# PytorchConnectomics/pytorch_connectomics

Hardware: AMD Instinct MI355X
Metric: voxels/s (train + sliding-window infer), MedNeXt-S 112^3 bf16 (higher is better)
Workload: dtype bf16; 1 GPU; Lucchi++ sliding-window inference (configs[1]): MedNeXt-S k3, 165x1024x768 volume, roi 112^3, overlap 0.5, bump blending, sw_batch_size 8, random-init weights; step = one whole-volume EagerSlidingWindowEngine call (TTA off); value = window-voxels/s; sw_batch_size=8, window_pipeline_streams=3

## Files before the change

include/pytc_hip.h:

```cpp
#ifndef PYTC_HIP_H
#define PYTC_HIP_H

#include <stdint.h>

#ifdef __cplusplus
extern "C" {
#endif

#define PYTC_ABI_VERSION 12

#define PYTC_OK 0
#define PYTC_ERR_INVALID 1
#define PYTC_ERR_HIP 2
#define PYTC_ERR_UNSUPPORTED 3

#define PYTC_F32 0
#define PYTC_BF16 1

#define PYTC_VIEW_FLIP_Z 1
#define PYTC_VIEW_FLIP_Y 2
#define PYTC_VIEW_FLIP_X 4
#define PYTC_VIEW_SWAP_YX 8
#define PYTC_VIEW_SWAP_ZY 16
#define PYTC_VIEW_SWAP_ZX 32

#define PYTC_PAD_CONSTANT 0
#define PYTC_PAD_REFLECT 1
#define PYTC_PAD_REPLICATE 2
#define PYTC_PAD_CIRCULAR 3

#define PYTC_BLEND_PRODUCT 0
#define PYTC_BLEND_MIN 1

#define PYTC_ACT_NONE 0
#define PYTC_ACT_SIGMOID 1
#define PYTC_ACT_TANH 2
#define PYTC_ACT_GELU 3

#define PYTC_RES_NONE 0
#define PYTC_RES_ADD 1
#define PYTC_RES_UPSAMPLE 2
#define PYTC_RES_GELU_BWD 3
#define PYTC_RES_NORM_BWD 4

int pytc_abi_version(void);
const char* pytc_last_error(void);
int pytc_device_info(int device, int* cu_count, int* lds_bytes_per_cu, char* arch, int arch_len);
int pytc_set_tuning(const char* key, int value);


int pytc_gather_windows(const float* vol, int C, int Z, int Y, int X, const int32_t* starts, int B,
                        int rz, int ry, int rx, int view, int pad_mode, float cval, void* out,
                        int out_dtype, void* stream);

int pytc_blend_accumulate(const void* pred, int pred_dtype, int B, const int32_t* starts, int rz,
                          int ry, int rx, int C, int view, const float* wz, const float* wy,
                          const float* wx, int combine, float floor_w, const int32_t* border ,
                          float* value, float* weight, int Z, int Y, int X, void* stream);

int pytc_blend_accumulate_mapped(const void* pred, int pred_dtype, int B, const int32_t* starts, int rz, int ry,
                                 int rx, int C, int view, const float* wz, const float* wy, const float* wx,
                                 int combine, float floor_w, const int32_t* border, const int32_t* chan_src,
                                 const int32_t* chan_shift, float* value, float* weight, int Z, int Y, int X,
                                 void* stream);
int pytc_blend_weight_shifted(int B, const int32_t* starts, int rz, int ry, int rx, const float* wz, const float* wy,
                              const float* wx, int combine, float floor_w, const int32_t* border,
                              const int32_t* shift, float* weight, int Z, int Y, int X, void* stream);
int pytc_normalize_covered(float* value, const float* weight, int64_t n, void* stream);
int pytc_ensemble_update_masked(float* stat, float* count, const float* x, const float* cover, int64_t n, int mode,
                                void* stream);
int pytc_ensemble_finalize_masked(const float* stat, const float* count, float* out, int64_t n, int mode, void* stream);

int pytc_blend_finalize(float* value, const float* weight, int C, int64_t nvox, float clamp,
                        int act, void* stream);

#define PYTC_ACT_SOFTMAX 4
int pytc_channel_activation(float* value, int C, int64_t nvox, int channels_last, int c0, int c1, int act,
                            float scale, void* stream);

int pytc_ensemble_update(float* acc, const float* x, int64_t n, int mode, int count, void* stream);

#define PYTC_ST_U8 0
#define PYTC_ST_I8 1
#define PYTC_ST_U16 2
#define PYTC_ST_I16 3
#define PYTC_ST_I32 4
#define PYTC_ST_F16 5
#define PYTC_ST_F32 6
int pytc_scale_cast(const float* x, void* y, int64_t n, float scale, int target, void* stream);


#define PYTC_RAW_U8 0
#define PYTC_RAW_I8 1
#define PYTC_RAW_U16 2
#define PYTC_RAW_I16 3
#define PYTC_RAW_U32 4
#define PYTC_RAW_I32 5
#define PYTC_RAW_F32 6
#define PYTC_RAW_F64 7
int pytc_resample_region(const void* raw, int raw_dtype, const int64_t* strides_czyx, int C, const int32_t* tab_i0,
                         const int32_t* tab_i1, const float* tab_f, const int32_t* dims_zyx, float* out, void* stream);

#define PYTC_NORM_NONE 0
#define PYTC_NORM_ZSCORE 1
#define PYTC_NORM_MINMAX 2
#define PYTC_NORM_DIVIDE 3
int64_t pytc_window_normalize_ws_elems(int B, int64_t n);
int pytc_window_normalize(float* x, int B, int64_t n, int mode, int binarize, float threshold, float divide, const float* clip,
                          double* workspace, void* stream);


int pytc_dwconv3d_stat_slots(int N, int D, int H, int W, int C, int K, int stride, int dtype,
                             int transposed);

int pytc_dwconv3d_kernel_variant(int N, int D, int H, int W, int C, int K, int stride, int dtype, int transposed);

int pytc_dwconv3d_fwd(const void* x, void* y, const float* w, const float* bias, float* stats,
                      int N, int D, int H, int W, int C, int K, int stride, int dtype,
                      void* stream);

int pytc_dwconv3d_fwd_wide(const void* x, void* y, const float* w, const float* bias, float* stats, int N, int D, int H,
                           int W, int C, int K, int stride, int dtype, void* stream);

int pytc_dwconv3d_res_supported(int D, int H, int W, int C, int K, int stride, int dtype);

int pytc_dwmix_supported(int D, int H, int W, int C, int C_hid, int C_out, int dtype);
int pytc_dwmix_fwd(const void* x, const float* taps, const float* dw_bias, const void* w2n, const float* b2n, const void* w3_f16,
                   const float* b3, int residual, void* y, const void* head_w, const float* head_b, float* head_y, int n_head, int N,
                   int D, int H, int W, int C, int C_hid, int C_out, int dtype, void* stream);
int pytc_dwconv3d_fwd_res(const void* x, const void* res, void* y, const float* w, const float* bias, int N, int D, int H,
                          int W, int C, int K, int stride, int dtype, void* stream);

int pytc_dwconvT3d_fwd(const void* x, void* y, const float* w, const float* bias, float* stats,
                       int N, int D, int H, int W, int C, int K, int dtype, void* stream);

int pytc_groupnorm_finalize(const float* stats, int slots, float count, const float* gamma,
                            const float* beta, float eps, float* ab, int N, int C, void* stream);


int64_t pytc_pw_packed_elems(int C_out, int C_in, int dtype);
int pytc_pw_pack_weight(const float* w, int C_out, int C_in, int transposed, void* packed,
                        int dtype, void* stream);

typedef struct {
  const void* x;
  const void* w_packed;
  const float* bias;
  const float* ab;
  const void* res;
  void* y;
  int N;
  int64_t rows_per_sample;
  int C_in, C_out;
  int in_dtype, out_dtype, w_dtype;
  int act;
  int res_mode;
  int gather;
  int Di, Hi, Wi;
  const void* res_low;
  const float* res_bias;
  int pre_act;
  int w_paired;
} pytc_pw_args;

int pytc_pw_conv_fwd(const pytc_pw_args* a, void* stream);
int pytc_pw_conv_paired_supported(const pytc_pw_args* a);
int pytc_pw_conv_rowmajor_supported(const pytc_pw_args* a);

typedef struct {
  const void* t;
  const float* ab;
  const void* w2_packed;
  const float* b2;
  const void* w3_packed;
  const float* b3;
  const void* res;
  const void* res_low;
  const float* res_bias;
  void* y;
  int N;
  int64_t rows_per_sample;
  int C_in, C_hid, C_out;
  int res_mode;
  int Di, Hi, Wi;
  int w3_format;
  int per_sample;
} pytc_mlp_args;
#define PYTC_W3_BF16 0
#define PYTC_W3_F16 1

int pytc_pw_gemm_supported(int C_in, int C_out);
int pytc_pw_gemm_fwd(const void* x, const void* w, const float* bias, const float* ab, void* y, int N, int64_t rows_per_sample,
                     int C_in, int C_out, int in_f16, int gelu_out, const void* res, const void* res_low, const float* res_bias,
                     int res_mode, int Di, int Hi, int Wi, void* stream);
int pytc_pw_mlp_supported(int C_in, int C_hid, int C_out);
int pytc_pw_pack_weight_paired(const float* w, int C_out, int C_in, int transposed, void* packed_bf16,
                               void* stream);
int pytc_pack_multi(const int64_t* table_dev, int n_items, int64_t total_elems, void* stream);
int pytc_pw_pack_weight_paired_f16(const float* w, int C_out, int C_in, int transposed, void* packed_f16,
                                   void* stream);
int pytc_pw_mlp_fwd(const pytc_mlp_args* a, void* stream);

int pytc_pw_mlp_lds_supported(int C_in, int C_hid, int C_out);
int pytc_pw_mlp_lds_fwd(const pytc_mlp_args* a, void* stream);
int pytc_pw_mlp_dma_applies(const pytc_mlp_args* a, int ignore_res_mode);
int pytc_pw_mlp_proj_supported(int C_in, int C_hid, int C_out, int C_proj);
int pytc_pw_mlp_proj_fwd(const pytc_mlp_args* a, const void* proj_w, const float* proj_b, void* z, int store_y, void* stream);
int pytc_pw_mlp_chunk_supported(int C_in, int C_hid, int C_out);
int pytc_pw_mlp_chunk_fwd(const pytc_mlp_args* a, void* stream);
int pytc_groupnorm_fold_mlp(const float* stats, int slots, float count, const float* gamma, const float* beta, float eps,
                            const float* w2, const float* b2, void* w2n, float* b2n, float* ab_out, int N, int C, int C_hid,
                            void* stream);
int pytc_pw_mlp_train_fwd(const pytc_mlp_args* a, void* hidden_pre, void* stream);
int pytc_pw_mlp_train_fwd_nostore(const pytc_mlp_args* a, void* stream);
int pytc_pw_mlp_bwd(const pytc_mlp_args* a, const void* hidden_pre, void* d_hidden, void* stream);
int pytc_pw_mlp_up_supported(int C_in, int C_hid, int C_out);
int pytc_pw_mlp_up_fwd(const pytc_mlp_args* a, const float* taps, const float* dw_bias, void* stream);
int pytc_pw_mlp_head_supported(int C_in, int C_hid, int C_out);
int pytc_pw_mlp_stemres_fwd(const pytc_mlp_args* a, const float* stem_x, const float* stem_w, const float* stem_b,
                            void* stream);
int pytc_stem_dwconv3d_stat_slots(int D, int H, int W);
int pytc_stem_dwconv3d_supported(int C_in, int C, int K);
int pytc_stem_dwconv3d_mfma_image_bytes(void);
int pytc_stem_dwconv3d_pack_mfma(const float* wx, const float* wb, const float* cst, void* image, void* stream);
int pytc_stem_dwconv3d_fwd(const float* x, const float* wx, const float* wb, const float* cst, const void* mfma_image, void* y,
                           float* stats, int N, int D, int H, int W, int C, void* stream);
int pytc_pw_mlp_head_fwd(const pytc_mlp_args* a, const void* head_w, const float* head_b, float* head_y, int n_head,
                         int store_y, void* stream);


#define PYTC_ACT_RELU 5
#define PYTC_ACT_LEAKY 6
#define PYTC_ACT_ELU 7

typedef struct {
  const void* x;
  const void* w_packed;
  const float* bias;
  const float* ab;
  const void* res;
  void* y;
  int N, D, H, W, C_in, C_out;
  int kd, kh, kw;
  int act_in;
  float act_param;
  int res_mode;
  int dtype;
} pytc_conv3d_args;

int64_t pytc_conv3d_packed_elems(int C_out, int C_in, int kd, int kh, int kw, int dtype);
int pytc_conv3d_pack_weight(const float* w, int C_out, int C_in, int kd, int kh, int kw, void* packed, int dtype,
                            void* stream);
int pytc_conv3d_fwd(const pytc_conv3d_args* a, void* stream);

int pytc_channel_stats_slots(int64_t rows);
int pytc_channel_stats(const void* x, float* stats, int N, int64_t rows, int C, int dtype, void* stream);
int pytc_norm_finalize_groups(const float* stats, int slots, float count, const float* gamma, const float* beta,
                              float eps, int groups, float* ab, int N, int C, void* stream);
int pytc_affine_act(const void* x, void* y, const float* ab, int N, int64_t rows, int C, int act, float prm,
                    int dtype, void* stream);
int pytc_maxpool3d_fwd(const void* x, void* y, int N, int D, int H, int W, int C, int fz, int fy, int fx, int dtype,
                       void* stream);
int pytc_dwconvT3d_generic_fwd(const void* x, void* y, const float* w, int N, int D, int H, int W, int C,
                               const int32_t* kernel, const int32_t* stride, const int32_t* pad, int dtype,
                               void* stream);


int pytc_groupnorm_finalize_mr(const float* stats, int slots, float count, const float* gamma, const float* beta,
                               float eps, float* ab, float* mean_rstd, int N, int C, void* stream);
int pytc_gelu(const void* x, const void* dy, void* out, int64_t n, int dtype, void* stream);
int pytc_add_inplace(void* y, const void* x, int64_t n, int dtype, void* stream);
int pytc_pw_wgrad_slots(int64_t rows_total);
int pytc_pw_wgrad(const void* x, const float* ab, const void* dy, float* dW, float* db, float* workspace, int N,
                  int64_t rows_per_sample, int C_in, int C_out, int dtype, int x_act , void* stream);
int pytc_dw_wgrad_slots(int N, const int32_t* gdims, const int32_t* xdims, int C, int K, int stride, int dtype);
int pytc_dw_wgrad(const void* g, const void* x, float* dW, float* db, float* workspace, int N, const int32_t* gdims,
                  const int32_t* xdims, int C, int K, int stride, int dtype, void* stream);

int pytc_pw_wgrad_partial(const void* x, const float* ab, const void* dy, float* workspace, int want_db, int N,
                          int64_t rows_per_sample, int C_in, int C_out, int dtype, int x_act, int* slots_out, void* stream);
int pytc_pw_wgrad_dgrad_supported(int C_in, int C_out, int dtype);
int pytc_pw_wgrad_dgrad_partial(const void* x, const void* dy, const void* w_t_paired, void* dx, float* workspace, int want_db, int N,
                                int64_t rows_per_sample, int C_in, int C_out, int dtype, int* slots_out, void* stream);
int pytc_mixer_bwd_rc_supported(int C, int C_hid, int C_out, int dtype);
int pytc_mixer_bwd_rc_sps(int N, int64_t rows_per_sample, int C_hid);
int64_t pytc_mixer_bwd_rc_ws_elems(int N, int64_t rows_per_sample, int C_hid, int gn);
int pytc_mixer_bwd_rc(const void* t, const float* ab, const float* mean_rstd, const void* dy, const void* w2_paired, const float* b2,
                      const void* w3t_paired, const float* W2, const float* gamma, float count, void* dhp, float* workspace,
                      float* s_out, float* coef, int want_db3, int gn, int N, int64_t rows_per_sample, int C, int C_hid, int C_out,
                      int dtype, int* slots_out, void* stream);
int pytc_dw_wgrad_partial(const void* g, const void* x, float* workspace, int want_db, int N, const int32_t* gdims,
                          const int32_t* xdims, int C, int K, int stride, int dtype, int* slots_out, void* stream);
int pytc_copy_zero_front(const void* src, void* dst, int N, const int32_t* dims, int C, int dtype, void* stream);
typedef struct {
  const float* part;
  float* out;
  int64_t n;
  int32_t slots;
  int32_t out_t;
} pytc_reduce_item;
int pytc_reduce_slots_multi(const pytc_reduce_item* items, int n_items, void* stream);
int pytc_norm_bwd_ws_elems(int N, int64_t rows, int C);
int pytc_norm_bwd(const void* dtn, const void* t, const float* mean_rstd, const float* gamma, float* stats_ws,
                  float* s_out, void* dt, int N, int64_t rows, float count , int C,
                  int dtype, void* stream);
int pytc_pw_wgrad_groupnorm_supported(int C, int C_hid, int dtype);
int pytc_pw_wgrad_groupnorm_sps(int N, int64_t rows_per_sample, int C, int C_hid);
int64_t pytc_pw_wgrad_groupnorm_ws_elems(int N, int64_t rows_per_sample, int C, int C_hid);
int pytc_pw_wgrad_groupnorm(const void* t, const float* mean_rstd, const float* ab, const void* dhp, const float* W2,
                            const float* gamma, float count, float* s_out, float* coef, float* workspace, int N,
                            int64_t rows_per_sample, int C, int C_hid, int dtype, void* stream);
int pytc_norm_bwd_apply(const void* dtn, const void* t, const float* mean_rstd, const float* gamma, const float* s_in,
                        int s_parts, void* dt, int N, int64_t rows, int C, float count, int dtype, const int32_t* crop_grid,
                        void* stream);
int pytc_dwconv3d_bwd_data(const void* dy, const float* w, void* dx, int N, const int32_t* xdims,
                           const int32_t* ydims, int C, int K, int stride, int dtype, void* stream);
int pytc_dwconv3d_bwd_data_add(const void* dy, const float* w, const void* addend, void* dx, int N, const int32_t* xdims,
                               const int32_t* ydims, int C, int K, int stride, int dtype, void* stream);

int pytc_conv3d_pack_weight_dgrad(const float* w, int C_out, int C_in, int kd, int kh, int kw, void* packed, int dtype,
                                  void* stream);
int pytc_conv3d_pack_plan(int C_out, int C_in, int kd, int kh, int kw, int dtype, int direct, int64_t* out);
int pytc_conv3d_pack_multi(const int64_t* table_dev, int n_items, int64_t total_blocks, void* stream);
int pytc_conv3d_launch_plan(int N, int D, int H, int W, int C_in, int C_out, int kd, int kh, int kw, int dtype, int has_pre,
                            int has_res, int phase, int64_t* out);
int pytc_norm_bwd_means(const float* s, const float* gamma, float* M, float* dgamma, float* dbeta, int N, int C, int groups,
                        float rows, void* stream);
int pytc_bn_train_finalize_cpad(const float* stats, int slots_total, float count, const float* gamma, const float* beta, float eps,
                                float momentum, float* running_mean, float* running_var, int64_t* num_batches_tracked, float* ab,
                                float* mean_rstd, int N, int C, int C_real, void* stream);
int pytc_norm_finalize_groups_cpg(const float* stats, int slots, float count, const float* gamma, const float* beta, float eps,
                                  int groups, int cpg, float* ab, float* mr, int N, int C, void* stream);
int pytc_norm_bwd_means_cpg(const float* s, const float* gamma, float* M, float* dgamma, float* dbeta, int N, int C, int groups,
                            int cpg, float rows, void* stream);
int pytc_bn_train_finalize(const float* stats, int slots_total, float count, const float* gamma, const float* beta, float eps,
                           float momentum, float* running_mean, float* running_var, int64_t* num_batches_tracked, float* ab,
                           float* mean_rstd, int N, int C, void* stream);
int pytc_bn_update_running(const float* mean_rstd, float* running_mean, float* running_var, int C, float count, float eps,
                           float momentum, void* stream);
int64_t pytc_conv3d_wgrad_ws_elems(int N, int D, int H, int W, int C_in, int C_out, const int32_t* kernel, int dtype);
int pytc_conv3d_wgrad(const void* a, const void* dy, float* dW, float* workspace, int N, int D, int H, int W, int C_in,
                      int C_out, const int32_t* kernel, int dtype, void* stream);
int pytc_act_bwd(const void* da, const void* x, const float* ab, void* dt, void* dp, int N, int64_t rows, int C, int act,
                 float prm, int dtype, void* stream);
int pytc_norm_finalize_groups_mr(const float* stats, int slots, float count, const float* gamma, const float* beta,
                                 float eps, int groups, float* ab, float* mr, int N, int C, void* stream);
int pytc_norm_bwd_stats(const void* dtn, const void* t, const float* mean_rstd, float* stats_ws, float* s_out, int N,
                        int64_t rows, int C, int dtype, void* stream);
int pytc_norm_bwd_apply_general(const void* d, const void* x, const float* mean_rstd, const float* gamma, const float* M,
                                void* dx, int N, int64_t rows, int C, int dtype, void* stream);
int pytc_act_norm_bwd_stats(const void* da, const void* x, const float* ab, const float* mean_rstd, float* stats_ws, float* s_out,
                            float* p_ws, float* p_out, int N, int64_t rows, int C, int act, float prm, int dtype, void* stream);
int pytc_act_norm_bwd_apply(const void* da, const void* x, const float* ab, const float* mean_rstd, const float* gamma,
                            const float* M, void* dx, int N, int64_t rows, int C, int act, float prm, int dtype, void* stream);
// ... 178 lines not shown
```

pytorch_connectomics_amd/csrc/pw_common.h:

```cpp
#pragma once
#include "pytc_common.h"

namespace pytc {

template <typename TW>
struct Mma;

template <>
struct Mma<bf16_t> {
  static constexpr int EPL = 8;
  static constexpr int KSTEP = 32;
  typedef bf16x8_t frag_t;
  static __device__ __forceinline__ f32x4_t mma(frag_t a, frag_t b, f32x4_t c) {
    return __builtin_amdgcn_mfma_f32_16x16x32_bf16(a, b, c, 0, 0, 0);
  }
  static __device__ __forceinline__ frag_t from_floats(const float (&v)[8]) {
    f32x8_t f;
#pragma unroll
    for (int i = 0; i < 8; ++i) f[i] = v[i];
    return __builtin_convertvector(f, frag_t);
  }
};

template <>
struct Mma<float> {
  static constexpr int EPL = 4;
  static constexpr int KSTEP = 16;
  typedef f32x4_t frag_t;
  static __device__ __forceinline__ f32x4_t mma(frag_t a, frag_t b, f32x4_t c) {
#pragma unroll
    for (int s = 0; s < 4; ++s) c = __builtin_amdgcn_mfma_f32_16x16x4f32(a[s], b[s], c, 0, 0, 0);
    return c;
  }
  static __device__ __forceinline__ frag_t from_floats(const float (&v)[4]) {
    frag_t f;
#pragma unroll
    for (int i = 0; i < 4; ++i) f[i] = v[i];
    return f;
  }
};

__host__ __device__ __forceinline__ int paired_row(int T, int m) {
  return (T >> 1) * 32 + (m >> 2) * 8 + (T & 1) * 4 + (m & 3);
}

struct EpiParams {
  const void* res;
  const void* res_low;
  const float* res_bias;
  void* y;
  long rps_out;
  int C_out;
  int res_mode;
  int Go_d, Go_h, Go_w;
  int Gl_d, Gl_h, Gl_w;
  int nt;
};

typedef unsigned int pytc_u32x4_t __attribute__((ext_vector_type(4)));
template <typename V>
__device__ __forceinline__ V ld_stream(const V* ptr, int nt) {
  static_assert(sizeof(V) == 16, "16-byte row pieces");
  if (nt) return __builtin_bit_cast(V, __builtin_nontemporal_load(reinterpret_cast<const pytc_u32x4_t*>(ptr)));
  return *ptr;
}

template <typename TO, int NCH, bool GELU_BWD = false, int COUT = 0>
__device__ __forceinline__ void finish_and_store(float (&v)[NCH], const EpiParams& e, int n, long orow, int o0,
                                                 const float* pre = nullptr, const int* pos = nullptr) {
  const int C_out = COUT > 0 ? COUT : e.C_out;
  TO* yn = reinterpret_cast<TO*>(e.y) + (long)n * e.rps_out * C_out;
  const TO* resn = e.res ? reinterpret_cast<const TO*>(e.res) + (long)n * e.rps_out * C_out : nullptr;
  const long off = orow * C_out + o0;
  const bool full = (C_out % NCH) == 0 && (o0 + NCH <= C_out);
  if (e.res_mode == PYTC_RES_ADD) {
    float rv[NCH];
    if (pre) {
#pragma unroll
      for (int i = 0; i < NCH; ++i) rv[i] = pre[i];
    } else if (full) VecIO<TO, NCH>::load(resn + off, rv);
    else {
#pragma unroll
      for (int i = 0; i < NCH; ++i) rv[i] = (o0 + i < C_out) ? to_f32<TO>(resn[off + i]) : 0.f;
    }
#pragma unroll
    for (int i = 0; i < NCH; ++i) v[i] += rv[i];
  } else if (GELU_BWD && e.res_mode == PYTC_RES_GELU_BWD) {
    float rv[NCH];
    if (pre) {
#pragma unroll
      for (int i = 0; i < NCH; ++i) rv[i] = pre[i];
    } else if (full) VecIO<TO, NCH>::load(resn + off, rv);
    else {
#pragma unroll
      for (int i = 0; i < NCH; ++i) rv[i] = (o0 + i < C_out) ? to_f32<TO>(resn[off + i]) : 0.f;
    }
#pragma unroll
    for (int i = 0; i < NCH; ++i) v[i] *= gelu_erf_grad(rv[i]);
  } else if (GELU_BWD && e.res_mode == PYTC_RES_NORM_BWD) {
    float rv[NCH];
    if (pre) {
#pragma unroll
      for (int i = 0; i < NCH; ++i) rv[i] = pre[i];
    } else if (full) VecIO<TO, NCH>::load(resn + off, rv);
    else {
#pragma unroll
      for (int i = 0; i < NCH; ++i) rv[i] = (o0 + i < C_out) ? to_f32<TO>(resn[off + i]) : 0.f;
    }
    const float* cf = e.res_bias + (long)n * 3 * C_out + o0;
#pragma unroll
    for (int i = 0; i < NCH; ++i)
      if (o0 + i < C_out) v[i] = fmaf(cf[i], v[i], fmaf(cf[C_out + i], rv[i], cf[2 * C_out + i]));
    if (e.Go_w > 0) {
      const unsigned ur = (unsigned)orow, gw = (unsigned)e.Go_w, gh = (unsigned)e.Go_h;
      const unsigned tq = ur / gw;
      const int px = (int)(ur - tq * gw), pz = (int)(tq / gh), py = (int)(tq - (unsigned)pz * gh);
      if (px == 0 || py == 0 || pz == 0) return;
      const long crow = ((long)(pz - 1) * (e.Go_h - 1) + (py - 1)) * (e.Go_w - 1) + (px - 1);
      TO* yc = reinterpret_cast<TO*>(e.y) + ((long)n * (e.Go_d - 1) * (e.Go_h - 1) * (e.Go_w - 1) + crow) * C_out + o0;
      if (full) VecIO<TO, NCH>::store(yc, v);
      else {
#pragma unroll
        for (int i = 0; i < NCH; ++i)
          if (o0 + i < C_out) yc[i] = from_f32<TO>(v[i]);
      }
      return;
    }
  } else if (e.res_mode == PYTC_RES_UPSAMPLE) {
    int px, py, pz;
    if (pos) { pz = pos[0]; py = pos[1]; px = pos[2]; }
    else {
      const unsigned ur = (unsigned)orow, gw = (unsigned)e.Go_w, gh = (unsigned)e.Go_h;
      const unsigned t = ur / gw;
      px = (int)(ur - t * gw);
      pz = (int)(t / gh);
      py = (int)(t - (unsigned)pz * gh);
    }
    float sk[NCH];
    if (pre) {
#pragma unroll
      for (int i = 0; i < NCH; ++i) sk[i] = pre[i];
    } else if (full) VecIO<TO, NCH>::load(resn + off, sk);
    else {
#pragma unroll
      for (int i = 0; i < NCH; ++i) sk[i] = (o0 + i < C_out) ? to_f32<TO>(resn[off + i]) : 0.f;
    }
    if (px == 0 || py == 0 || pz == 0) {
#pragma unroll
      for (int i = 0; i < NCH; ++i) v[i] = sk[i];
    } else {
      const int oz = pz - 1, oy = py - 1, ox = px - 1;
      float rl[NCH];
      if (e.res_low && !((oz | oy | ox) & 1)) {
        const TO* rp = reinterpret_cast<const TO*>(e.res_low) +
                       ((((long)n * e.Gl_d + (oz >> 1)) * e.Gl_h + (oy >> 1)) * e.Gl_w + (ox >> 1)) * C_out + o0;
        if (full) VecIO<TO, NCH>::load(rp, rl);
        else {
#pragma unroll
          for (int i = 0; i < NCH; ++i) rl[i] = (o0 + i < C_out) ? to_f32<TO>(rp[i]) : 0.f;
        }
      } else {
#pragma unroll
        for (int i = 0; i < NCH; ++i) rl[i] = (e.res_bias && o0 + i < C_out) ? e.res_bias[o0 + i] : 0.f;
      }
#pragma unroll
      for (int i = 0; i < NCH; ++i) v[i] = v[i] + rl[i] + sk[i];
    }
  }
  if (full) {
    if constexpr (sizeof(TO) == 2 && NCH == 8) {
      if (e.nt) {
        f32x8_t f;
#pragma unroll
        for (int i = 0; i < 8; ++i) f[i] = v[i];
        __builtin_nontemporal_store(__builtin_convertvector(f, bf16x8_t), reinterpret_cast<bf16x8_t*>(yn + off));
        return;
      }
    }
    VecIO<TO, NCH>::store(yn + off, v);
  } else {
#pragma unroll
    for (int i = 0; i < NCH; ++i)
      if (o0 + i < C_out) yn[off + i] = from_f32<TO>(v[i]);
  }
}

template <typename TI, int EPL>
__device__ __forceinline__ void load_row_frag(const TI* __restrict__ row, int k0, int C_in, bool vec_ok,
                                              float (&v)[EPL]) {
  if (vec_ok && k0 + EPL <= C_in) {
    if constexpr (sizeof(TI) == 4 && EPL == 8) {
      float t0[4], t1[4];
      VecIO<float, 4>::load(reinterpret_cast<const float*>(row) + k0, t0);
      VecIO<float, 4>::load(reinterpret_cast<const float*>(row) + k0 + 4, t1);
#pragma unroll
      for (int i = 0; i < 4; ++i) { v[i] = t0[i]; v[4 + i] = t1[i]; }
    } else {
      VecIO<TI, EPL>::load(row + k0, v);
    }
  } else {
#pragma unroll
    for (int j = 0; j < EPL; ++j) v[j] = (k0 + j < C_in) ? to_f32<TI>(row[k0 + j]) : 0.f;
  }
}

template <int PER>
struct WarmRegs { unsigned int r[2 * PER]; };
template <int PER>
__device__ __forceinline__ void warm_l2(const void* base, long bytes, WarmRegs<PER>& w, int first) {
  const long lines = (bytes + 127) >> 7;
  const long lin = (long)blockIdx.z * gridDim.y * gridDim.x + (long)blockIdx.y * gridDim.x + blockIdx.x;
  const long total = (long)gridDim.x * gridDim.y * gridDim.z;
  const long per_xcd = (total + 7) >> 3;
  const long stride = per_xcd * blockDim.x;
  long l = (lin >> 3) * blockDim.x + threadIdx.x;
#pragma unroll
  for (int it = 0; it < PER; ++it, l += stride) {
    const long lc = l < lines ? l : lines - 1;
    const char* ptr = reinterpret_cast<const char*>(base) + (lc << 7);
    asm volatile("global_load_dword %0, %1, off" : "=v"(w.r[first + it]) : "v"(ptr) : "memory");
  }
}
template <int PER>
__device__ __forceinline__ void warm_l2_done(WarmRegs<PER>& w) {
  asm volatile("s_waitcnt vmcnt(0)" : : : "memory");
#pragma unroll
  for (int i = 0; i < 2 * PER; ++i) asm volatile("" : : "v"(w.r[i]) : "memory");
}

__device__ __forceinline__ float apply_act(float t, int act) {
  if (act == PYTC_ACT_GELU) return gelu_erf(t);
  if (act == PYTC_ACT_SIGMOID) return 1.f / (1.f + __expf(-t));
  if (act == PYTC_ACT_TANH) return tanhf(t);
  return t;
}

}
```

pytorch_connectomics_amd/csrc/pw_mlp_chunk_kernels.hip:

```cpp
#include "pw_common.h"

namespace pytc {

struct MlpChunkParams {
  const bf16_t* t;
  const float* ab;
  const bf16x8_t* w2;
  const float* b2;
  const h8_t* w3;
  const float* b3;
  EpiParams e;
  long rps;
  int N, C_in, C_hid, C_out, HC;
  long w2_stride;
};

__device__ __forceinline__ void chunk_glds16(const void* gsrc, unsigned lds_dst) {
  unsigned keep;
  asm volatile("s_mov_b32 %0, m0\n\ts_mov_b32 m0, %2\n\ts_nop 0\n\tglobal_load_lds_dwordx4 %1, off\n\ts_mov_b32 m0, %0"
               : "=&s"(keep) : "v"(gsrc), "s"(lds_dst) : "memory");
}

template <int KS_IN, int MO, int NW, int WPS>
__global__ void __launch_bounds__(NW * 64, WPS)
// ... 47 lines not shown
    for (int ks = 0; ks < KS_IN; ++ks) raw[ks][nt] = ld_stream(reinterpret_cast<const uint4*>(tn + rr * CIN + ks * 32 + kb * 8), p.e.nt);
  }
  {
    const float* b2 = p.b2 + (folded ? (long)n * p.C_hid : 0L);
    for (int i = tid; i < p.C_hid; i += NW * 64) lb2[i] = b2[i];
    if (tid < COUT) lb3[tid] = p.b3[tid];
  }
  request(0);
  if (p.HC > 1) request(1);
  const float* an = folded ? nullptr : p.ab + (long)n * 2 * CIN;
#pragma unroll
  for (int ks = 0; ks < KS_IN; ++ks) {
    if (folded) {
#pragma unroll
      for (int nt = 0; nt < NT; ++nt) bact[ks][nt] = __builtin_bit_cast(bf16x8_t, raw[ks][nt]);
    } else {
      const int k0 = ks * 32 + kb * 8;
      float av[8], bv[8];
      VecIO<float, 4>::load(an + k0, reinterpret_cast<float(&)[4]>(av[0]));
      VecIO<float, 4>::load(an + k0 + 4, reinterpret_cast<float(&)[4]>(av[4]));
      VecIO<float, 4>::load(an + CIN + k0, reinterpret_cast<float(&)[4]>(bv[0]));
      VecIO<float, 4>::load(an + CIN + k0 + 4, reinterpret_cast<float(&)[4]>(bv[4]));
#pragma unroll
      for (int nt = 0; nt < NT; ++nt) {
        float v[8];
        VecIO<bf16_t, 8>::load(reinterpret_cast<const bf16_t*>(&raw[ks][nt]), v);
#pragma unroll
        for (int j = 0; j < 8; ++j) v[j] = fmaf(v[j], av[j], bv[j]);
        bact[ks][nt] = Mma<bf16_t>::from_floats(v);
      }
    }
  }
#pragma unroll
  for (int ks = 0; ks < KS_IN; ++ks)
#pragma unroll
    for (int nt = 0; nt < NT; ++nt) asm volatile("" : "+v"(bact[ks][nt]));
  __syncthreads();
  f32x4_t acc2[MO][NT];
#pragma unroll
  for (int pr = 0; pr < MO / 2; ++pr) {
    const f32x4_t lo = *reinterpret_cast<const f32x4_t*>(lb3 + pr * 32 + kb * 8), hi = *reinterpret_cast<const f32x4_t*>(lb3 + pr * 32 + kb * 8 + 4);
#pragma unroll
    for (int nt = 0; nt < NT; ++nt) { acc2[2 * pr][nt] = lo; acc2[2 * pr + 1][nt] = hi; }
  }

  for (int hc = 0; hc < p.HC; ++hc) {
    if (hc + 1 < p.HC) {
      if (mine == 2) asm volatile("s_waitcnt vmcnt(2)" ::: "memory");
      else if (mine == 1) asm volatile("s_waitcnt vmcnt(1)" ::: "memory");
      else if (mine == 3) asm volatile("s_waitcnt vmcnt(3)" ::: "memory");
      else asm volatile("s_waitcnt vmcnt(0)" ::: "memory");
    } else {
      asm volatile("s_waitcnt vmcnt(0)" ::: "memory");
    }
    __syncthreads();
    if (hc + 2 < p.HC) request(hc + 2);
    const uint4* cb = ring + (size_t)(hc % NBUF) * PIECES * 64;
    const f32x4_t b2lo = *reinterpret_cast<const f32x4_t*>(lb2 + hc * 32 + kb * 8);
    const f32x4_t b2hi = *reinterpret_cast<const f32x4_t*>(lb2 + hc * 32 + kb * 8 + 4);
    f32x4_t acc1[2][NT];
#pragma unroll
    for (int nt = 0; nt < NT; ++nt) { acc1[0][nt] = b2lo; acc1[1][nt] = b2hi; }
#pragma unroll
    for (int mt = 0; mt < 2; ++mt) {
#pragma unroll
      for (int ks = 0; ks < KS_IN; ++ks) {
        const bf16x8_t a = __builtin_bit_cast(bf16x8_t, cb[(mt * KS_IN + ks) * 64 + lane]);
#pragma unroll
        for (int nt = 0; nt < NT; ++nt) acc1[mt][nt] = Mma<bf16_t>::mma(a, bact[ks][nt], acc1[mt][nt]);
      }
    }
    h8_t bhh[NT];
#pragma unroll
    for (int nt = 0; nt < NT; ++nt) {
      float gg[8];
#pragma unroll
      for (int j = 0; j < 4; ++j) { gg[j] = acc1[0][nt][j]; gg[4 + j] = acc1[1][nt][j]; }
      bhh[nt] = gelu_h8_from_f32(gg);
    }
#pragma unroll
    for (int mo = 0; mo < MO; ++mo) {
      const h8_t a = __builtin_bit_cast(h8_t, cb[(2 * KS_IN + mo) * 64 + lane]);
#pragma unroll
      for (int nt = 0; nt < NT; ++nt) acc2[mo][nt] = __builtin_amdgcn_mfma_f32_16x16x32_f16(a, bhh[nt], acc2[mo][nt], 0, 0, 0);
    }
  }

  if (row0 >= p.rps) return;
  int upos[NT][3];
  if (ups) {
    const unsigned ur = (unsigned)row0, gw = (unsigned)p.e.Go_w, gh = (unsigned)p.e.Go_h;
    const unsigned t0 = ur / gw;
    const int bx = (int)(ur - t0 * gw);
    const int bz = (int)(t0 / gh);
    const int by = (int)(t0 - (unsigned)bz * gh);
#pragma unroll
    for (int nt = 0; nt < NT; ++nt) {
      int px = bx + nt * 16 + r, py = by, pz = bz;
      while (px >= p.e.Go_w) { px -= p.e.Go_w; ++py; }
      while (py >= p.e.Go_h) { py -= p.e.Go_h; ++pz; }
      upos[nt][0] = pz; upos[nt][1] = py; upos[nt][2] = px;
    }
  }
#pragma unroll
  for (int pr = 0; pr < MO / 2; ++pr) {
#pragma unroll
    for (int nt = 0; nt < NT; ++nt) {
      if (orow[nt] >= p.rps) continue;
      float v[8];
#pragma unroll
      for (int j = 0; j < 4; ++j) { v[j] = acc2[2 * pr][nt][j]; v[4 + j] = acc2[2 * pr + 1][nt][j]; }
      finish_and_store<bf16_t, 8, false, COUT>(v, p.e, n, orow[nt], pr * 32 + kb * 8, nullptr, (with_res && ups) ? upos[nt] : nullptr);
    }
  }
}

template <int KS_IN, int MO, int NW, int WPS>
static void launch_mlp_chunk_v(const MlpChunkParams& p, hipStream_t s) {
  auto kern = &pw_mlp_chunk_kernel<KS_IN, MO, NW, WPS>;
  const size_t lds = (size_t)3 * (2 * KS_IN + MO) * 1024 + (size_t)(p.C_hid + MO * 16) * 4;
  if (!ensure_dynamic_lds(reinterpret_cast<const void*>(kern), 160 * 1024, "pw_mlp_chunk")) return;
  const long wg_rows = (long)NW * 32;
  dim3 grid((unsigned)((p.rps + wg_rows - 1) / wg_rows), (unsigned)p.N), block(NW * 64);
  hipLaunchKernelGGL(kern, grid, block, lds, s, p);
}

template <int KS_IN, int MO>
static void launch_mlp_chunk(const MlpChunkParams& p, int variant, hipStream_t s) {
  if (variant == 0) variant = (KS_IN == 8) ? 1 : 3;
  switch (variant) {
    case 2: launch_mlp_chunk_v<KS_IN, MO, 12, 3>(p, s); break;
    case 3: launch_mlp_chunk_v<KS_IN, MO, 8, 4>(p, s); break;
    case 4: launch_mlp_chunk_v<KS_IN, MO, 16, 4>(p, s); break;
    default: launch_mlp_chunk_v<KS_IN, MO, 8, 2>(p, s); break;
  }
}

}

using namespace pytc;

extern "C" int pytc_pw_mlp_chunk_supported(int C_in, int C_hid, int C_out) {
  if (C_in % 32 || C_hid % 32 || C_out % 32) return 0;
  const int ks = C_in / 32, mo = C_out / 16;
  const bool shape = (ks == 2 && (mo == 2 || mo == 4 || mo == 8)) || (ks == 4 && mo == 4) || (ks == 4 && mo == 8) || (ks == 8 && mo == 8);
  return (shape && C_hid >= 64 && C_hid <= 8192) ? 1 : 0;
}

extern "C" int pytc_pw_mlp_chunk_fwd(const pytc_mlp_args* a, void* stream) {
  PYTC_REQUIRE(a && a->t && (a->ab || a->per_sample) && a->w2_packed && a->w3_packed && a->b2 && a->b3 && a->y, "pw_mlp_chunk: null pointer");
  PYTC_REQUIRE(!(a->ab && a->per_sample), "pw_mlp_chunk: per-sample (norm-folded) expand operands come without an affine");
  PYTC_REQUIRE(a->w3_format == PYTC_W3_F16, "pw_mlp_chunk: the projection image must be fp16 (pytc_pw_pack_weight_paired_f16)");
  PYTC_REQUIRE(a->N >= 1 && a->rows_per_sample >= 1, "pw_mlp_chunk: bad shape");
  if (!pytc_pw_mlp_chunk_supported(a->C_in, a->C_hid, a->C_out)) {
    set_error("pw_mlp_chunk: no chunk-streamed kernel for C_in=%d C_hid=%d C_out=%d", a->C_in, a->C_hid, a->C_out);
    return PYTC_ERR_UNSUPPORTED;
  }
  PYTC_REQUIRE(a->res_mode == PYTC_RES_NONE || a->res, "pw_mlp_chunk: residual mode without residual pointer");
  PYTC_REQUIRE(a->res_mode == PYTC_RES_NONE || a->res_mode == PYTC_RES_ADD || a->res_mode == PYTC_RES_UPSAMPLE, "pw_mlp_chunk: residual mode");
  MlpChunkParams p{};
  p.t = (const bf16_t*)a->t; p.ab = a->ab; p.w2 = (const bf16x8_t*)a->w2_packed; p.b2 = a->b2;
  p.w3 = (const h8_t*)a->w3_packed; p.b3 = a->b3;
  p.rps = a->rows_per_sample; p.N = a->N; p.C_in = a->C_in; p.C_hid = a->C_hid; p.C_out = a->C_out; p.HC = a->C_hid / 32;
  p.w2_stride = (long)(a->C_hid / 16) * (a->C_in / 32) * 64;
  p.e.res = a->res; p.e.res_low = a->res_low; p.e.res_bias = a->res_bias; p.e.y = a->y;
  p.e.rps_out = a->rows_per_sample; p.e.C_out = a->C_out; p.e.res_mode = a->res_mode;
  p.e.nt = 0;
  p.e.Go_d = p.e.Go_h = p.e.Go_w = p.e.Gl_d = p.e.Gl_h = p.e.Gl_w = 0;
  if (a->res_mode == PYTC_RES_UPSAMPLE) {
    PYTC_REQUIRE((long)a->Di * a->Hi * a->Wi == a->rows_per_sample && !(a->Di & 1) && !(a->Hi & 1) && !(a->Wi & 1) &&
                 a->rows_per_sample < (1L << 31), "pw_mlp_chunk: RES_UPSAMPLE needs the (even) output grid");
    p.e.Go_d = a->Di; p.e.Go_h = a->Hi; p.e.Go_w = a->Wi;
    p.e.Gl_d = a->Di / 2; p.e.Gl_h = a->Hi / 2; p.e.Gl_w = a->Wi / 2;
  }
  hipStream_t s = (hipStream_t)stream;
  const int ks = a->C_in / 32, mo = a->C_out / 16;
  const int variant = tuning_get(K_mlp_chunk_variant);
  if (ks == 2 && mo == 2) launch_mlp_chunk<2, 2>(p, variant, s);
  else if (ks == 2 && mo == 4) launch_mlp_chunk<2, 4>(p, variant, s);
  else if (ks == 2 && mo == 8) launch_mlp_chunk<2, 8>(p, variant, s);
  else if (ks == 4 && mo == 4) launch_mlp_chunk<4, 4>(p, variant, s);
  else if (ks == 4 && mo == 8) launch_mlp_chunk<4, 8>(p, variant, s);
  else launch_mlp_chunk<8, 8>(p, variant, s);
  PYTC_LAUNCH_CHECK("pw_mlp_chunk");
  return PYTC_OK;
}
```

pytorch_connectomics_amd/csrc/pw_mlp_kernels.hip:

```cpp
#include <cmath>
#include "pw_common.h"

namespace pytc {

struct MlpParams {
  const bf16_t* t;
  const float* ab;
  const bf16x8_t* w2;
  const float* b2;
  const bf16x8_t* w3;
  const float* b3;
  EpiParams e;
  long rps;
  int C_in, C_hid, C_out, HC;
  int w3_f16;
  long w2_stride;
  const bf16x8_t* head_w;
  const float* head_b;
  float* head_y;
  int n_head, store_y;
  bf16_t* proj_y;
  const float* stem_x;
  const float* stem_w;
  const float* stem_b;
  bf16_t* hp;
  int round_h;
  const bf16_t* hp_in;
};

constexpr int mlp_waves_per_simd(int ks, int mo, int nt) {
  if (ks >= 8 && nt == 1) return 1;
  const int regs = ks * nt * 4 + mo * nt * 4 + 2 * nt * 4;
  return regs <= 64 ? 4 : (regs <= 112 ? 3 : (regs <= 200 ? 2 : 1));
}

template <int KS_IN, int MO, int NT, int GELU_MODE, bool HEAD = false, bool STEMRES = false, bool STOREH = false, bool BWD = false>
__global__ void __launch_bounds__(256, mlp_waves_per_simd(KS_IN, MO, NT))
pw_mlp_kernel(MlpParams p) {
  constexpr int CIN = KS_IN * 32, COUT = MO * 16;
  static_assert(MO % 2 == 0, "C_out must be a multiple of 32");
  static_assert(!STEMRES || (MO == 2 && (MO / 2) * NT <= 4), "the stem-recomputing residual covers C_out = 32");
  static_assert(!HEAD || MO == 2, "the fused head covers C_out = 32");
  static_assert(GELU_MODE == 1 || GELU_MODE == 3, "sigmoid-form or packed-fp16 GELU");
  constexpr bool PREFETCH_RES = (MO / 2) * NT <= 4;
  const int wave = threadIdx.x >> 6, lane = threadIdx.x & 63;
  const int n = blockIdx.y;
  constexpr bool WARM = KS_IN * MO >= 32;
  constexpr int WPER = KS_IN * MO >= 512 ? 6 : 2;
  WarmRegs<WPER> warm;
  const bool folded = p.ab == nullptr;
  const bf16x8_t* w2 = p.w2 + (folded ? (long)n * p.w2_stride : 0L);
  const float* b2 = p.b2 + (folded ? (long)n * p.C_hid : 0L);
  if (WARM) {
    warm_l2(w2, (long)p.C_hid * CIN * 2, warm, 0);
    warm_l2(p.w3, (long)COUT * p.C_hid * 2, warm, WPER);
  }
  const long row0 = ((long)blockIdx.x * 4 + wave) * (NT * 16);
  if (row0 >= p.rps) {
    if (WARM) asm volatile("s_waitcnt vmcnt(0)" : : : "memory");
    return;
  }
  const int r = lane & 15, kb = lane >> 4;

  long orow[NT];
#pragma unroll
  for (int nt = 0; nt < NT; ++nt) orow[nt] = row0 + nt * 16 + r;

  bf16x8_t bact[KS_IN][NT];
  const bf16_t* tn = p.t + (long)n * p.rps * CIN;
  if (folded) {
#pragma unroll
    for (int ks = 0; ks < KS_IN; ++ks)
#pragma unroll
      for (int nt = 0; nt < NT; ++nt) {
        const long rr = orow[nt] < p.rps ? orow[nt] : p.rps - 1;
        bact[ks][nt] = ld_stream(reinterpret_cast<const bf16x8_t*>(tn + rr * CIN + ks * 32 + kb * 8), p.e.nt);
      }
  }
  const float* an = p.ab + (long)n * 2 * CIN;
#pragma unroll
  for (int ks = 0; ks < KS_IN; ++ks) {
    if (folded) break;
    const int k0 = ks * 32 + kb * 8;
    float av[8], bv[8];
    VecIO<float, 4>::load(an + k0, reinterpret_cast<float(&)[4]>(av[0]));
    VecIO<float, 4>::load(an + k0 + 4, reinterpret_cast<float(&)[4]>(av[4]));
    VecIO<float, 4>::load(an + CIN + k0, reinterpret_cast<float(&)[4]>(bv[0]));
    VecIO<float, 4>::load(an + CIN + k0 + 4, reinterpret_cast<float(&)[4]>(bv[4]));
#pragma unroll
    for (int nt = 0; nt < NT; ++nt) {
      const long rr = orow[nt] < p.rps ? orow[nt] : p.rps - 1;
      float v[8];
      VecIO<bf16_t, 8>::load(tn + rr * CIN + k0, v);
#pragma unroll
      for (int j = 0; j < 8; ++j) v[j] = fmaf(v[j], av[j], bv[j]);
      bact[ks][nt] = Mma<bf16_t>::from_floats(v);
    }
  }

  if (WARM) warm_l2_done(warm);

  uint4 rpre[PREFETCH_RES ? MO / 2 : 1][PREFETCH_RES ? NT : 1];
  const bool use_pre = PREFETCH_RES && p.e.res_mode != PYTC_RES_NONE;
  if constexpr (STEMRES) {
    const float* sx = p.stem_x + (long)n * p.rps;
    float sw[8], sb[8];
    VecIO<float, 4>::load(p.stem_w + kb * 8, reinterpret_cast<float(&)[4]>(sw[0]));
    VecIO<float, 4>::load(p.stem_w + kb * 8 + 4, reinterpret_cast<float(&)[4]>(sw[4]));
    VecIO<float, 4>::load(p.stem_b + kb * 8, reinterpret_cast<float(&)[4]>(sb[0]));
    VecIO<float, 4>::load(p.stem_b + kb * 8 + 4, reinterpret_cast<float(&)[4]>(sb[4]));
#pragma unroll
    for (int nt = 0; nt < NT; ++nt) {
      const float xv = sx[orow[nt] < p.rps ? orow[nt] : p.rps - 1];
      float rv[8];
#pragma unroll
      for (int j = 0; j < 8; ++j) rv[j] = fmaf(sw[j], xv, sb[j]);
      rpre[0][nt] = __builtin_bit_cast(uint4, Mma<bf16_t>::from_floats(rv));
    }
  } else if (use_pre) {
    const bf16_t* resn = reinterpret_cast<const bf16_t*>(p.e.res) + (long)n * p.rps * COUT;
#pragma unroll
    for (int pr = 0; pr < (PREFETCH_RES ? MO / 2 : 1); ++pr)
#pragma unroll
      for (int nt = 0; nt < (PREFETCH_RES ? NT : 1); ++nt) {
        const long rr = orow[nt] < p.rps ? orow[nt] : p.rps - 1;
        rpre[pr][nt] = ld_stream(reinterpret_cast<const uint4*>(resn + rr * COUT + pr * 32 + kb * 8), p.e.nt);
      }
  }

  f32x4_t acc2[MO][NT];
#pragma unroll
  for (int pr = 0; pr < MO / 2; ++pr) {
    float b[8];
    VecIO<float, 4>::load(p.b3 + pr * 32 + kb * 8, reinterpret_cast<float(&)[4]>(b[0]));
    VecIO<float, 4>::load(p.b3 + pr * 32 + kb * 8 + 4, reinterpret_cast<float(&)[4]>(b[4]));
#pragma unroll
    for (int nt = 0; nt < NT; ++nt) {
      acc2[2 * pr][nt] = f32x4_t{b[0], b[1], b[2], b[3]};
      acc2[2 * pr + 1][nt] = f32x4_t{b[4], b[5], b[6], b[7]};
    }
  }

  for (int hc = 0; hc < p.HC; ++hc) {
    float b2v[8];
    VecIO<float, 4>::load(b2 + hc * 32 + kb * 8, reinterpret_cast<float(&)[4]>(b2v[0]));
    VecIO<float, 4>::load(b2 + hc * 32 + kb * 8 + 4, reinterpret_cast<float(&)[4]>(b2v[4]));
    f32x4_t acc1[2][NT];
#pragma unroll
    for (int nt = 0; nt < NT; ++nt) {
      acc1[0][nt] = f32x4_t{b2v[0], b2v[1], b2v[2], b2v[3]};
      acc1[1][nt] = f32x4_t{b2v[4], b2v[5], b2v[6], b2v[7]};
    }
#pragma unroll
    for (int mt = 0; mt < 2; ++mt) {
#pragma unroll
      for (int ks = 0; ks < KS_IN; ++ks) {
        const bf16x8_t a = w2[((long)(hc * 2 + mt) * KS_IN + ks) * 64 + lane];
#pragma unroll
        for (int nt = 0; nt < NT; ++nt) acc1[mt][nt] = Mma<bf16_t>::mma(a, bact[ks][nt], acc1[mt][nt]);
      }
    }
    bf16x8_t bh[NT];
    h8_t bhh[GELU_MODE == 3 ? NT : 1];
#pragma unroll
    for (int nt = 0; nt < NT; ++nt) {
      float g[8];
      if constexpr (BWD) {
        const long rr = orow[nt] < p.rps ? orow[nt] : p.rps - 1;
        float hv[8];
        VecIO<bf16_t, 8>::load(p.hp_in + ((long)n * p.rps + rr) * p.C_hid + hc * 32 + kb * 8, hv);
#pragma unroll
        for (int j = 0; j < 4; ++j) {
          g[j] = acc1[0][nt][j] * gelu_erf_grad(hv[j]);
          g[4 + j] = acc1[1][nt][j] * gelu_erf_grad(hv[4 + j]);
        }
        bh[nt] = Mma<bf16_t>::from_floats(g);
        if (orow[nt] < p.rps)
          *reinterpret_cast<bf16x8_t*>(p.hp + ((long)n * p.rps + orow[nt]) * p.C_hid + hc * 32 + kb * 8) = bh[nt];
        continue;
      }
      if constexpr (STOREH) {
        float pre[8];
#pragma unroll
        for (int j = 0; j < 4; ++j) { pre[j] = acc1[0][nt][j]; pre[4 + j] = acc1[1][nt][j]; }
        const bf16x8_t hb = Mma<bf16_t>::from_floats(pre);
        if (p.hp && orow[nt] < p.rps)
          *reinterpret_cast<bf16x8_t*>(p.hp + ((long)n * p.rps + orow[nt]) * p.C_hid + hc * 32 + kb * 8) = hb;
        const f32x8_t hr = __builtin_convertvector(hb, f32x8_t);
#pragma unroll
        for (int j = 0; j < 4; ++j) { acc1[0][nt][j] = hr[j]; acc1[1][nt][j] = hr[4 + j]; }
      }
      if constexpr (GELU_MODE == 3) {
#pragma unroll
        for (int j = 0; j < 4; ++j) { g[j] = acc1[0][nt][j]; g[4 + j] = acc1[1][nt][j]; }
        bhh[nt] = gelu_h8_from_f32(g);
        continue;
      }
#pragma unroll
      for (int j = 0; j < 4; ++j) {
        g[j] = gelu_fast(acc1[0][nt][j]);
        g[4 + j] = gelu_fast(acc1[1][nt][j]);
      }
      bh[nt] = Mma<bf16_t>::from_floats(g);
    }
#pragma unroll
    for (int mo = 0; mo < MO; ++mo) {
      if constexpr (GELU_MODE == 3) {
        const h8_t a = reinterpret_cast<const h8_t*>(p.w3)[((long)mo * p.HC + hc) * 64 + lane];
#pragma unroll
        for (int nt = 0; nt < NT; ++nt) acc2[mo][nt] = __builtin_amdgcn_mfma_f32_16x16x32_f16(a, bhh[nt], acc2[mo][nt], 0, 0, 0);
      } else {
        const bf16x8_t a = p.w3[((long)mo * p.HC + hc) * 64 + lane];
#pragma unroll
        for (int nt = 0; nt < NT; ++nt) acc2[mo][nt] = Mma<bf16_t>::mma(a, bh[nt], acc2[mo][nt]);
      }
    }
  }

  if constexpr (HEAD) {
    bf16_t* yn = reinterpret_cast<bf16_t*>(p.e.y) + (long)n * p.rps * 32;
    const bf16_t* resn = p.e.res ? reinterpret_cast<const bf16_t*>(p.e.res) + (long)n * p.rps * 32 : nullptr;
    float* hy = p.head_y + (long)n * p.rps * p.n_head;
    const bf16x8_t ah = p.head_w[lane];
    float hb[4];
#pragma unroll
    for (int i = 0; i < 4; ++i) hb[i] = (p.head_b && kb * 4 + i < p.n_head) ? p.head_b[kb * 4 + i] : 0.f;
#pragma unroll
    for (int nt = 0; nt < NT; ++nt) {
      float v[8];
#pragma unroll
      for (int j = 0; j < 4; ++j) { v[j] = acc2[0][nt][j]; v[4 + j] = acc2[1][nt][j]; }
      const bool live = orow[nt] < p.rps;
      if (p.e.res_mode == PYTC_RES_ADD) {
        float rv[8];
        if (use_pre) VecIO<bf16_t, 8>::load(reinterpret_cast<const bf16_t*>(&rpre[0][PREFETCH_RES ? nt : 0]), rv);
        else VecIO<bf16_t, 8>::load(resn + (live ? orow[nt] : p.rps - 1) * 32 + kb * 8, rv);
#pragma unroll
        for (int j = 0; j < 8; ++j) v[j] += rv[j];
      }
      const bf16x8_t ob = Mma<bf16_t>::from_floats(v);
      if (p.store_y && live) *reinterpret_cast<bf16x8_t*>(yn + orow[nt] * 32 + kb * 8) = ob;
      const f32x4_t h = Mma<bf16_t>::mma(ah, ob, f32x4_t{0.f, 0.f, 0.f, 0.f});
      if (live) {
#pragma unroll
        for (int i = 0; i < 4; ++i)
          if (kb * 4 + i < p.n_head) hy[orow[nt] * p.n_head + kb * 4 + i] = h[i] + hb[i];
      }
    }
    return;
  }
  int upos[NT][3];
  const bool ups = p.e.res_mode == PYTC_RES_UPSAMPLE;
  if (ups) {
    const unsigned ur = (unsigned)row0, gw = (unsigned)p.e.Go_w, gh = (unsigned)p.e.Go_h;
    const unsigned t0 = ur / gw;
    const int bx = (int)(ur - t0 * gw);
    const int bz = (int)(t0 / gh);
    const int by = (int)(t0 - (unsigned)bz * gh);
#pragma unroll
    for (int nt = 0; nt < NT; ++nt) {
      int px = bx + nt * 16 + r, py = by, pz = bz;
      while (px >= p.e.Go_w) { px -= p.e.Go_w; ++py; }
      while (py >= p.e.Go_h) { py -= p.e.Go_h; ++pz; }
      upos[nt][0] = pz; upos[nt][1] = py; upos[nt][2] = px;
    }
  }
#pragma unroll
  for (int pr = 0; pr < MO / 2; ++pr) {
#pragma unroll
    for (int nt = 0; nt < NT; ++nt) {
      if (orow[nt] >= p.rps) continue;
      float v[8];
#pragma unroll
      for (int j = 0; j < 4; ++j) {
        v[j] = acc2[2 * pr][nt][j];
        v[4 + j] = acc2[2 * pr + 1][nt][j];
      }
      if (use_pre) {
        float pre[8];
        VecIO<bf16_t, 8>::load(reinterpret_cast<const bf16_t*>(&rpre[PREFETCH_RES ? pr : 0][PREFETCH_RES ? nt : 0]), pre);
        finish_and_store<bf16_t, 8, false, COUT>(v, p.e, n, orow[nt], pr * 32 + kb * 8, pre, ups ? upos[nt] : nullptr);
      } else {
        finish_and_store<bf16_t, 8, false, COUT>(v, p.e, n, orow[nt], pr * 32 + kb * 8, nullptr, ups ? upos[nt] : nullptr);
      }
    }
  }
}


__device__ __forceinline__ void glds16(const void* gsrc, unsigned lds_dst) {
  unsigned keep;
  asm volatile("s_mov_b32 %0, m0\n\ts_mov_b32 m0, %2\n\ts_nop 0\n\tglobal_load_lds_dwordx4 %1, off\n\ts_mov_b32 m0, %0"
               : "=&s"(keep) : "v"(gsrc), "s"(lds_dst) : "memory");
}
__device__ __forceinline__ void glds4(const void* gsrc, unsigned lds_dst) {
  unsigned keep;
  asm volatile("s_mov_b32 %0, m0\n\ts_mov_b32 m0, %2\n\ts_nop 0\n\tglobal_load_lds_dword %1, off\n\ts_mov_b32 m0, %0"
               : "=&s"(keep) : "v"(gsrc), "s"(lds_dst) : "memory");
}

template <int HCT, int KIND>
__global__ void __launch_bounds__(256, 3)
pw_mlp_dma_kernel(MlpParams p, int waves_per_sample) {
  constexpr int NT = 4, CIN = 32, COUT = 32;
  constexpr bool STEM = KIND == 1, HEAD = KIND == 2, PROJ = KIND == 3;
  __shared__ __attribute__((aligned(16))) uint4 land[4][2][NT * 64];
  __shared__ __attribute__((aligned(16))) uint4 w2s[HCT * 2 * 64], w3s[2 * HCT * 64];
  __shared__ __attribute__((aligned(16))) float b2s[HCT * 32], b3s[32];
  __shared__ __attribute__((aligned(16))) float auxa[STEM ? 32 : (HEAD ? 256 : (PROJ ? 512 : 4))], auxb[(STEM || PROJ) ? 32 : (HEAD ? 16 : 4)];
  const int wave = threadIdx.x >> 6, lane = threadIdx.x & 63;
  const int n = blockIdx.y;
  const int r = lane & 15, kb = lane >> 4;
  const long tiles = (p.rps + NT * 16 - 1) / (NT * 16);
  const bool with_res = STEM || p.e.res_mode == PYTC_RES_ADD;
  const bf16_t* tn = p.t + (long)n * p.rps * CIN;
  const bf16_t* resn = (!STEM && with_res) ? reinterpret_cast<const bf16_t*>(p.e.res) + (long)n * p.rps * COUT : nullptr;
  const float* sx = STEM ? p.stem_x + (long)n * p.rps : nullptr;
  bf16_t* yn = reinterpret_cast<bf16_t*>(p.e.y) + (long)n * p.rps * COUT;
  float* hy = HEAD ? p.head_y + (long)n * p.rps * p.n_head : nullptr;
  bf16_t* zn = PROJ ? p.proj_y + (long)n * p.rps * 32 : nullptr;
  {
    const uint4* w2 = reinterpret_cast<const uint4*>(p.w2 + (long)n * p.w2_stride);
    const uint4* w3 = reinterpret_cast<const uint4*>(p.w3);
    for (int i = threadIdx.x; i < HCT * 2 * 64; i += 256) { w2s[i] = w2[i]; w3s[i] = w3[i]; }
    if (threadIdx.x < HCT * 32) b2s[threadIdx.x] = p.b2[(long)n * p.C_hid + threadIdx.x];
    if (threadIdx.x < 32) b3s[threadIdx.x] = p.b3[threadIdx.x];
    if constexpr (STEM) {
      if (threadIdx.x < 32) { auxa[threadIdx.x] = p.stem_w[threadIdx.x]; auxb[threadIdx.x] = p.stem_b[threadIdx.x]; }
    }
    if constexpr (HEAD) {
      reinterpret_cast<float*>(auxa)[threadIdx.x] = reinterpret_cast<const float*>(p.head_w)[threadIdx.x];
      if (threadIdx.x < 16) auxb[threadIdx.x] = (p.head_b && (int)threadIdx.x < p.n_head) ? p.head_b[threadIdx.x] : 0.f;
    }
    if constexpr (PROJ) {
      auxa[threadIdx.x] = reinterpret_cast<const float*>(p.head_w)[threadIdx.x];
      auxa[threadIdx.x + 256] = reinterpret_cast<const float*>(p.head_w)[threadIdx.x + 256];
      if (threadIdx.x < 32) auxb[threadIdx.x] = p.head_b ? p.head_b[threadIdx.x] : 0.f;
    }
  }
  __syncthreads();
  asm volatile("s_waitcnt vmcnt(0)" ::: "memory");

  const unsigned lbase = __builtin_amdgcn_readfirstlane((unsigned)(size_t)(__attribute__((address_space(3))) void*)&land[wave][0][0]);
  auto request = [&](long tile) {
#pragma unroll
    for (int nt = 0; nt < NT; ++nt) {
      long row = tile * (NT * 16) + nt * 16 + r;
      row = row < p.rps ? row : p.rps - 1;
      glds16(tn + row * CIN + kb * 8, lbase + (unsigned)(nt * 64) * 16);
      if constexpr (STEM) glds4(sx + row, lbase + (unsigned)(NT * 64) * 16 + (unsigned)(nt * 64) * 4);
      else if (with_res) glds16(resn + row * COUT + kb * 8, lbase + (unsigned)((NT + nt) * 64) * 16);
    }
  };
  bf16x8_t out[NT];
  f32x4_t hout[HEAD ? NT : 1];
  bf16x8_t zout[PROJ ? NT : 1];
  auto store = [&](long tile) {
#pragma unroll
    for (int nt = 0; nt < NT; ++nt) {
      const long row = tile * (NT * 16) + nt * 16 + r;
      if (row >= p.rps) continue;
      if (!(HEAD || PROJ) || p.store_y) *reinterpret_cast<bf16x8_t*>(yn + row * COUT + kb * 8) = out[nt];
      if constexpr (PROJ) *reinterpret_cast<bf16x8_t*>(zn + row * 32 + kb * 8) = zout[nt];
      if constexpr (HEAD) {
#pragma unroll
        for (int i = 0; i < 4; ++i)
          if (kb * 4 + i < p.n_head) hy[row * p.n_head + kb * 4 + i] = hout[nt][i];
      }
    }
  };
  const long gw = (long)blockIdx.x * 4 + wave;
  long tile = gw;
  if (tile >= tiles) return;
  request(tile);
  long out_tile = -1;
  for (; tile < tiles; tile += waves_per_sample) {
    asm volatile("s_waitcnt vmcnt(0)" ::: "memory");
    __builtin_amdgcn_wave_barrier();
    if (out_tile >= 0) store(out_tile);
    bf16x8_t bact[NT];
    uint4 rpre[STEM ? 1 : NT];
    float xin[STEM ? NT : 1];
#pragma unroll
    for (int nt = 0; nt < NT; ++nt) {
      bact[nt] = __builtin_bit_cast(bf16x8_t, land[wave][0][nt * 64 + lane]);
      if constexpr (STEM) xin[nt] = reinterpret_cast<const float*>(&land[wave][1][0])[nt * 64 + lane];
      else if (with_res) rpre[nt] = land[wave][1][nt * 64 + lane];
    }
    asm volatile("s_waitcnt lgkmcnt(0)" ::: "memory");
    __builtin_amdgcn_wave_barrier();
    if (tile + waves_per_sample < tiles) request(tile + waves_per_sample);
    f32x4_t acc2[2][NT];
    {
      const f32x4_t lo = *reinterpret_cast<const f32x4_t*>(&b3s[kb * 8]), hi = *reinterpret_cast<const f32x4_t*>(&b3s[kb * 8 + 4]);
#pragma unroll
      for (int nt = 0; nt < NT; ++nt) { acc2[0][nt] = lo; acc2[1][nt] = hi; }
    }
#pragma unroll
    for (int hc = 0; hc < HCT; ++hc) {
      f32x4_t acc1[2][NT];
      {
        const f32x4_t lo = *reinterpret_cast<const f32x4_t*>(&b2s[hc * 32 + kb * 8]), hi = *reinterpret_cast<const f32x4_t*>(&b2s[hc * 32 + kb * 8 + 4]);
#pragma unroll
        for (int nt = 0; nt < NT; ++nt) { acc1[0][nt] = lo; acc1[1][nt] = hi; }
      }
#pragma unroll
      for (int mt = 0; mt < 2; ++mt) {
        const bf16x8_t a2 = __builtin_bit_cast(bf16x8_t, w2s[(hc * 2 + mt) * 64 + lane]);
#pragma unroll
        for (int nt = 0; nt < NT; ++nt) acc1[mt][nt] = Mma<bf16_t>::mma(a2, bact[nt], acc1[mt][nt]);
      }
      h8_t bhh[NT];
#pragma unroll
      for (int nt = 0; nt < NT; ++nt) {
        float g[8];
#pragma unroll
        for (int j = 0; j < 4; ++j) { g[j] = acc1[0][nt][j]; g[4 + j] = acc1[1][nt][j]; }
        bhh[nt] = gelu_h8_from_f32(g);
      }
#pragma unroll
      for (int mo = 0; mo < 2; ++mo) {
        const h8_t a3 = __builtin_bit_cast(h8_t, w3s[(mo * HCT + hc) * 64 + lane]);
#pragma unroll
        for (int nt = 0; nt < NT; ++nt) acc2[mo][nt] = __builtin_amdgcn_mfma_f32_16x16x32_f16(a3, bhh[nt], acc2[mo][nt], 0, 0, 0);
      }
    }
    float sw[STEM ? 8 : 1], sb[STEM ? 8 : 1];
    if constexpr (STEM) {
#pragma unroll
// ... 96 lines not shown
  __syncthreads();
  if (i >= total) return;
  int lo = s_lo;
  while (lo + 1 < n_items && table[(lo + 1) * 8 + 6] <= i) ++lo;
  const long* it = table + lo * 8;
  const float* w = reinterpret_cast<const float*>(it[0]);
  const int kind = (int)it[2], C_out = (int)it[3], C_in = (int)it[4], aux = (int)it[5];
  const long e = i - it[6];
  if (kind >= 6) {
    const int o = (int)(e / C_in), k = (int)(e % C_in);
    reinterpret_cast<bf16_t*>(it[1])[e] = from_f32<bf16_t>(kind == 7 ? w[(long)k * C_out + o] : w[e]);
    return;
  }
  if (kind >= 4) {
    const int K3 = aux, C = C_out;
    const int k = (int)(e / C), c = (int)(e % C);
    reinterpret_cast<float*>(it[1])[e] = w[(long)c * K3 + (kind == 5 ? K3 - 1 - k : k)];
    return;
  }
  const int KG = aux, transposed = kind & 1;
  const int j = (int)(e % 8);
  long t = e / 8;
  const int lane = (int)(t % 64);
  t /= 64;
  const int kg = (int)(t % KG);
  const int T = (int)(t / KG);
  const int o = paired_row(T, lane & 15);
  const int k = kg * 32 + (lane >> 4) * 8 + j;
  float v = 0.f;
  if (o < C_out && k < C_in) v = transposed ? w[(long)k * C_out + o] : w[(long)o * C_in + k];
  if (kind >= 2) reinterpret_cast<_Float16*>(it[1])[e] = (_Float16)v;
  else reinterpret_cast<bf16_t*>(it[1])[e] = from_f32<bf16_t>(v);
}

__global__ void __launch_bounds__(1024)
groupnorm_fold_mlp_kernel(const float* __restrict__ stats, int slots, float count, const float* __restrict__ gamma,
                          const float* __restrict__ beta, float eps, const float* __restrict__ w2, const float* __restrict__ b2,
                          bf16_t* __restrict__ w2n, float* __restrict__ b2n, float* __restrict__ ab_out, int C, int C_hid) {
  __shared__ __attribute__((aligned(16))) float red[1024 * 4];
  __shared__ float part[8][2 * 128];
  __shared__ float sa[128], sb[128], smean[128], sbeta[128];
  const int n = blockIdx.x, tid = threadIdx.x;
  const int Q = C / 2;
  const int col = tid % Q, sl = tid / Q, SL = 1024 / Q;
  const float* base = stats + (long)n * slots * 2 * C + col * 4;
  const int KG = C / 32;
  const long total = (long)C_hid * C;
  constexpr int PRE = 2;
  f32x4_t wpre[PRE][2];
#pragma unroll
  for (int i = 0; i < PRE; ++i) {
    const long e8 = tid + (long)i * 1024;
    if (e8 < total / 8) {
      long t = e8;
      const int lane = (int)(t % 64);
      t /= 64;
      const int kg = (int)(t % KG);
      const int o = paired_row((int)(t / KG), lane & 15);
      const float* src = w2 + (long)o * C + kg * 32 + (lane >> 4) * 8;
      wpre[i][0] = *reinterpret_cast<const f32x4_t*>(src);
      wpre[i][1] = *reinterpret_cast<const f32x4_t*>(src + 4);
    }
  }
  f32x4_t a = {0.f, 0.f, 0.f, 0.f};
  constexpr int INFL = 20;
  for (int s0 = sl; s0 < slots; s0 += SL * INFL) {
    f32x4_t v[INFL];
#pragma unroll
    for (int i = 0; i < INFL; ++i) {
      const int s = s0 + i * SL;
      v[i] = s < slots ? *reinterpret_cast<const f32x4_t*>(base + (long)s * 2 * C) : f32x4_t{0.f, 0.f, 0.f, 0.f};
    }
#pragma unroll
    for (int i = 0; i < INFL; ++i)
      if (s0 + i * SL < slots) a += v[i];
  }
  *reinterpret_cast<f32x4_t*>(&red[tid * 4]) = a;
  __syncthreads();
  {
    const int e = tid % (2 * C), pg = tid / (2 * C);
    const int groups = 1024 / (2 * C) < 8 ? 1024 / (2 * C) : 8;
    if (pg < groups) {
      float t = 0.f;
      for (int s = pg; s < SL; s += groups) t += red[s * 2 * C + e];
      part[pg][e] = t;
    }
    __syncthreads();
    if (tid < C) {
      float t1 = 0.f, t2 = 0.f;
      for (int g = 0; g < groups; ++g) { t1 += part[g][tid]; t2 += part[g][C + tid]; }
      const float mean = t1 / count;
      const float var = fmaxf(t2 / count - mean * mean, 0.f);
      float rstd = rsqrtf(var + eps);
      rstd = rstd * (1.5f - 0.5f * (var + eps) * rstd * rstd);
      const float av = (gamma ? gamma[tid] : 1.f) * rstd;
      const float bv = (beta ? beta[tid] : 0.f) - mean * av;
      sa[tid] = av;
      sb[tid] = bv;
      smean[tid] = mean;
      sbeta[tid] = beta ? beta[tid] : 0.f;
      if (ab_out) {
        ab_out[((long)n * 2 + 0) * C + tid] = av;
        ab_out[((long)n * 2 + 1) * C + tid] = bv;
      }
    }
  }
  __syncthreads();
  bf16_t* img = w2n + (long)n * total;
  for (long e8 = tid, i = 0; e8 < total / 8; e8 += 1024, ++i) {
    long t = e8;
    const int lane = (int)(t % 64);
    t /= 64;
    const int kg = (int)(t % KG);
    const int T = (int)(t / KG);
    const int o = paired_row(T, lane & 15);
    const int k = kg * 32 + (lane >> 4) * 8;
    float v[8];
    if (i < PRE) {
#pragma unroll
      for (int q = 0; q < PRE; ++q)
        if (q == i) {
#pragma unroll
          for (int j = 0; j < 4; ++j) { v[j] = wpre[q][0][j]; v[4 + j] = wpre[q][1][j]; }
        }
    } else {
      VecIO<float, 4>::load(w2 + (long)o * C + k, reinterpret_cast<float(&)[4]>(v[0]));
      VecIO<float, 4>::load(w2 + (long)o * C + k + 4, reinterpret_cast<float(&)[4]>(v[4]));
    }
#pragma unroll
    for (int j = 0; j < 8; ++j) v[j] *= sa[k + j];
    *reinterpret_cast<bf16x8_t*>(img + e8 * 8) = Mma<bf16_t>::from_floats(v);
  }
  for (int o = tid; o < C_hid; o += 1024) {
    float acc = b2 ? b2[o] : 0.f;
    const float* wr = w2 + (long)o * C;
    for (int k = 0; k < C; k += 8) {
      const f32x4_t w0 = *reinterpret_cast<const f32x4_t*>(wr + k), w1 = *reinterpret_cast<const f32x4_t*>(wr + k + 4);
      float v[8], wn[8];
#pragma unroll
      for (int j = 0; j < 4; ++j) { v[j] = w0[j] * sa[k + j]; v[4 + j] = w1[j] * sa[k + 4 + j]; }
      const bf16x8_t rounded = Mma<bf16_t>::from_floats(v);
      VecIO<bf16_t, 8>::load(reinterpret_cast<const bf16_t*>(&rounded), wn);
#pragma unroll
      for (int j = 0; j < 8; ++j) {
        const float wj = j < 4 ? w0[j] : w1[j - 4];
        acc = fmaf(wj, sbeta[k + j], acc);
        acc = fmaf(-wn[j], smean[k + j], acc);
      }
    }
    b2n[(long)n * C_hid + o] = acc;
  }
}

template <int KS_IN, int MO, int NT>
static void launch_mlp(const MlpParams& p, int N, hipStream_t s) {
  long rows_per_block = 4L * NT * 16;
  dim3 grid((unsigned)((p.rps + rows_per_block - 1) / rows_per_block), (unsigned)N), block(256);
  if (p.hp_in) {
    hipLaunchKernelGGL((pw_mlp_kernel<KS_IN, MO, NT, 1, false, false, false, true>), grid, block, 0, s, p);
    return;
  }
  if (p.hp || p.round_h) {
    if (p.w3_f16) hipLaunchKernelGGL((pw_mlp_kernel<KS_IN, MO, NT, 3, false, false, true>), grid, block, 0, s, p);
    else hipLaunchKernelGGL((pw_mlp_kernel<KS_IN, MO, NT, 1, false, false, true>), grid, block, 0, s, p);
    return;
  }
  if (p.w3_f16) hipLaunchKernelGGL((pw_mlp_kernel<KS_IN, MO, NT, 3>), grid, block, 0, s, p);
  else hipLaunchKernelGGL((pw_mlp_kernel<KS_IN, MO, NT, 1>), grid, block, 0, s, p);
}

static bool dispatch_mlp(const MlpParams& p, int N, hipStream_t s) {
  const int ks = p.C_in / 32, mo = p.C_out / 16;
#define PYTC_MLP_CASE(KS, MOO, NTT) \
  if (ks == KS && mo == MOO) { launch_mlp<KS, MOO, NTT>(p, N, s); return true; }
  PYTC_MLP_CASE(1, 2, 4)
  PYTC_MLP_CASE(1, 4, 4)
  PYTC_MLP_CASE(2, 2, 4)
  PYTC_MLP_CASE(2, 4, 2)
  PYTC_MLP_CASE(2, 8, 2)
  PYTC_MLP_CASE(4, 4, 2)
  PYTC_MLP_CASE(4, 8, 2)
  PYTC_MLP_CASE(4, 16, 1)
  PYTC_MLP_CASE(8, 8, 2)
  PYTC_MLP_CASE(8, 16, 1)
  PYTC_MLP_CASE(8, 32, 1)
  PYTC_MLP_CASE(16, 16, 1)
  PYTC_MLP_CASE(16, 32, 1)
#undef PYTC_MLP_CASE
  return false;
}

static bool mlp_shape_ok(int C_in, int C_hid, int C_out) {
  if (C_in % 32 || C_hid % 32 || C_out % 32 || C_in < 32 || C_out < 32 || C_hid < 32) return false;
  const int ks = C_in / 32, mo = C_out / 16;
  static const int ok[][2] = {{1, 2}, {1, 4}, {2, 2}, {2, 4}, {2, 8}, {4, 4}, {4, 8}, {4, 16}, {8, 8},
                              {8, 16}, {8, 32}, {16, 16}, {16, 32}};
  for (auto& c : ok)
    if (c[0] == ks && c[1] == mo) return true;
  return false;
}

}

using namespace pytc;

extern "C" int pytc_pw_mlp_supported(int C_in, int C_hid, int C_out) { return mlp_shape_ok(C_in, C_hid, C_out) ? 1 : 0; }

extern "C" int pytc_groupnorm_fold_mlp(const float* stats, int slots, float count, const float* gamma, const float* beta,
                                       float eps, const float* w2, const float* b2, void* w2n, float* b2n, float* ab_out, int N,
                                       int C, int C_hid, void* stream) {
  PYTC_REQUIRE(stats && w2 && w2n && b2n && slots >= 1 && count > 0 && N >= 1, "groupnorm_fold_mlp: bad arguments");
  PYTC_REQUIRE(C == 32 || C == 64 || C == 128, "groupnorm_fold_mlp: C=%d (32, 64 or 128)", C);
  PYTC_REQUIRE(C_hid % 32 == 0 && C_hid >= 32 && C_hid <= 512, "groupnorm_fold_mlp: C_hid=%d", C_hid);
  hipLaunchKernelGGL(groupnorm_fold_mlp_kernel, dim3(N), dim3(1024), 0, (hipStream_t)stream, stats, slots, count, gamma, beta,
                     eps, w2, b2, (bf16_t*)w2n, b2n, ab_out, C, C_hid);
  PYTC_LAUNCH_CHECK("groupnorm_fold_mlp");
  return PYTC_OK;
}

extern "C" int pytc_pw_mlp_head_supported(int C_in, int C_hid, int C_out) {
  return (C_out == 32 && (C_in == 32 || C_in == 64) && C_hid % 32 == 0 && C_hid >= 32) ? 1 : 0;
}

extern "C" int pytc_pw_pack_weight_paired(const float* w, int C_out, int C_in, int transposed, void* packed,
                                          void* stream) {
  PYTC_REQUIRE(w && packed && C_out >= 1 && C_in >= 1, "pw_pack_weight_paired: bad arguments");
  PYTC_REQUIRE(C_out % 32 == 0, "pw_pack_weight_paired: C_out=%d must be a multiple of 32", C_out);
  long total = pytc_pw_packed_elems(C_out, C_in, PYTC_BF16);
  int KG = (C_in + 31) / 32;
  hipLaunchKernelGGL(pw_pack_paired_kernel<bf16_t>, dim3(ceil_div(total, 256)), dim3(256), 0, (hipStream_t)stream, w, C_out,
                     C_in, transposed, (bf16_t*)packed, KG, total);
  PYTC_LAUNCH_CHECK("pw_pack_weight_paired");
  return PYTC_OK;
}

extern "C" int pytc_pw_pack_weight_paired_f16(const float* w, int C_out, int C_in, int transposed, void* packed,
                                              void* stream) {
  PYTC_REQUIRE(w && packed && C_out >= 1 && C_in >= 1, "pw_pack_weight_paired_f16: bad arguments");
  PYTC_REQUIRE(C_out % 32 == 0, "pw_pack_weight_paired_f16: C_out=%d must be a multiple of 32", C_out);
  long total = pytc_pw_packed_elems(C_out, C_in, PYTC_BF16);
  int KG = (C_in + 31) / 32;
  hipLaunchKernelGGL(pw_pack_paired_kernel<_Float16>, dim3(ceil_div(total, 256)), dim3(256), 0, (hipStream_t)stream, w,
                     C_out, C_in, transposed, (_Float16*)packed, KG, total);
  PYTC_LAUNCH_CHECK("pw_pack_weight_paired_f16");
  return PYTC_OK;
}

extern "C" int pytc_pack_multi(const int64_t* table_dev, int n_items, int64_t total_elems, void* stream) {
  PYTC_REQUIRE(table_dev && n_items >= 1 && total_elems >= 1, "pack_multi: bad arguments");
  hipLaunchKernelGGL(pack_multi_kernel, dim3(ceil_div(total_elems, 256)), dim3(256), 0, (hipStream_t)stream,
                     reinterpret_cast<const long*>(table_dev), n_items, (long)total_elems);
  PYTC_LAUNCH_CHECK("pack_multi");
  return PYTC_OK;
}

extern "C" int pytc_pw_mlp_head_fwd(const pytc_mlp_args* a, const void* head_w, const float* head_b, float* head_y,
                                    int n_head, int store_y, void* stream) {
  PYTC_REQUIRE(a && a->t && (a->ab || a->per_sample) && a->w2_packed && a->w3_packed && a->b2 && a->b3 && head_w && head_y, "pw_mlp_head: null pointer");
  PYTC_REQUIRE(!(a->ab && a->per_sample), "pw_mlp_head: per-sample (norm-folded) expand operands come without an affine");
  PYTC_REQUIRE(!store_y || a->y, "pw_mlp_head: store_y without an output buffer");
  PYTC_REQUIRE(a->N >= 1 && a->rows_per_sample >= 1 && n_head >= 1 && n_head <= 16, "pw_mlp_head: bad shape");
  if (!pytc_pw_mlp_head_supported(a->C_in, a->C_hid, a->C_out)) {
    set_error("pw_mlp_head: no fused kernel for C_in=%d C_hid=%d C_out=%d", a->C_in, a->C_hid, a->C_out);
    return PYTC_ERR_UNSUPPORTED;
  }
  PYTC_REQUIRE(a->res_mode == PYTC_RES_NONE || (a->res_mode == PYTC_RES_ADD && a->res), "pw_mlp_head: residual add or none");
  MlpParams p;
  p.t = (const bf16_t*)a->t; p.ab = a->ab; p.w2 = (const bf16x8_t*)a->w2_packed; p.b2 = a->b2;
  p.w3 = (const bf16x8_t*)a->w3_packed; p.b3 = a->b3;
  p.rps = a->rows_per_sample; p.C_in = a->C_in; p.C_hid = a->C_hid; p.C_out = a->C_out; p.HC = a->C_hid / 32;
  p.w2_stride = (long)(a->C_hid / 16) * (a->C_in / 32) * 64;
  p.e.res = a->res; p.e.res_low = nullptr; p.e.res_bias = nullptr; p.e.y = a->y;
  p.e.rps_out = a->rows_per_sample; p.e.C_out = a->C_out; p.e.res_mode = a->res_mode;
  p.e.nt = 0;
  p.e.Go_d = p.e.Go_h = p.e.Go_w = p.e.Gl_d = p.e.Gl_h = p.e.Gl_w = 0;
  p.head_w = (const bf16x8_t*)head_w; p.head_b = head_b; p.head_y = head_y; p.n_head = n_head; p.store_y = store_y;
  p.w3_f16 = a->w3_format == PYTC_W3_F16 ? 1 : 0;
  dim3 grid((unsigned)((p.rps + 4L * 4 * 16 - 1) / (4L * 4 * 16)), (unsigned)a->N), block(256);
  hipStream_t s = (hipStream_t)stream;
  if (mlp_dma_applies(a, p)) {
    mlp_dma_launch<2>(a, p, s);
    PYTC_LAUNCH_CHECK("pw_mlp_head_dma");
    return PYTC_OK;
  }
  if (p.w3_f16) {
    if (a->C_in == 32) hipLaunchKernelGGL((pw_mlp_kernel<1, 2, 4, 3, true>), grid, block, 0, s, p);
    else hipLaunchKernelGGL((pw_mlp_kernel<2, 2, 4, 3, true>), grid, block, 0, s, p);
  } else if (a->C_in == 32) {
    hipLaunchKernelGGL((pw_mlp_kernel<1, 2, 4, 1, true>), grid, block, 0, s, p);
  } else {
    hipLaunchKernelGGL((pw_mlp_kernel<2, 2, 4, 1, true>), grid, block, 0, s, p);
  }
  PYTC_LAUNCH_CHECK("pw_mlp_head");
  return PYTC_OK;
}

extern "C" int pytc_pw_mlp_stemres_fwd(const pytc_mlp_args* a, const float* stem_x, const float* stem_w, const float* stem_b,
                                       void* stream) {
  PYTC_REQUIRE(a && a->t && (a->ab || a->per_sample) && a->w2_packed && a->w3_packed && a->b2 && a->b3 && a->y && stem_x && stem_w && stem_b,
               "pw_mlp_stemres: null pointer");
  PYTC_REQUIRE(!(a->ab && a->per_sample), "pw_mlp_stemres: per-sample (norm-folded) expand operands come without an affine");
  PYTC_REQUIRE(a->N >= 1 && a->rows_per_sample >= 1, "pw_mlp_stemres: bad shape");
  if (!(a->C_in == 32 && a->C_out == 32 && a->C_hid % 32 == 0 && a->C_hid >= 32)) {
    set_error("pw_mlp_stemres: no fused kernel for C_in=%d C_hid=%d C_out=%d", a->C_in, a->C_hid, a->C_out);
    return PYTC_ERR_UNSUPPORTED;
  }
  MlpParams p{};
  p.t = (const bf16_t*)a->t; p.ab = a->ab; p.w2 = (const bf16x8_t*)a->w2_packed; p.b2 = a->b2;
  p.w3 = (const bf16x8_t*)a->w3_packed; p.b3 = a->b3;
  p.rps = a->rows_per_sample; p.C_in = a->C_in; p.C_hid = a->C_hid; p.C_out = a->C_out; p.HC = a->C_hid / 32;
  p.w2_stride = (long)(a->C_hid / 16) * (a->C_in / 32) * 64;
  p.e.res = a->y;
  p.e.y = a->y;
  p.e.rps_out = a->rows_per_sample; p.e.C_out = a->C_out; p.e.res_mode = PYTC_RES_ADD;
  p.e.nt = 0;
  p.stem_x = stem_x; p.stem_w = stem_w; p.stem_b = stem_b;
  p.w3_f16 = a->w3_format == PYTC_W3_F16 ? 1 : 0;
  dim3 grid((unsigned)((p.rps + 4L * 4 * 16 - 1) / (4L * 4 * 16)), (unsigned)a->N), block(256);
  hipStream_t s = (hipStream_t)stream;
  pytc_mlp_args shape = *a;
  shape.res_mode = PYTC_RES_NONE;
  if (mlp_dma_applies(&shape, p)) {
    mlp_dma_launch<1>(a, p, s);
    PYTC_LAUNCH_CHECK("pw_mlp_stemres_dma");
    return PYTC_OK;
  }
  if (p.w3_f16) hipLaunchKernelGGL((pw_mlp_kernel<1, 2, 4, 3, false, true>), grid, block, 0, s, p);
  else hipLaunchKernelGGL((pw_mlp_kernel<1, 2, 4, 1, false, true>), grid, block, 0, s, p);
  PYTC_LAUNCH_CHECK("pw_mlp_stemres");
  return PYTC_OK;
}

extern "C" int pytc_pw_mlp_dma_applies(const pytc_mlp_args* a, int ignore_res_mode) {
  if (!a) return 0;
  MlpParams p{};
  p.HC = a->C_hid / 32;
  p.w3_f16 = a->w3_format == PYTC_W3_F16 ? 1 : 0;
  pytc_mlp_args shape = *a;
  if (ignore_res_mode) shape.res_mode = PYTC_RES_NONE;
  return mlp_dma_applies(&shape, p) ? 1 : 0;
}

extern "C" int pytc_pw_mlp_proj_supported(int C_in, int C_hid, int C_out, int C_proj) {
  return (C_in == 32 && C_out == 32 && C_proj == 32 && (C_hid == 64 || C_hid == 96 || C_hid == 128)) ? 1 : 0;
}
extern "C" int pytc_pw_mlp_proj_fwd(const pytc_mlp_args* a, const void* proj_w, const float* proj_b, void* z, int store_y, void* stream) {
  PYTC_REQUIRE(a && a->t && a->w2_packed && a->w3_packed && a->b2 && a->b3 && proj_w && z, "pw_mlp_proj: null pointer");
  PYTC_REQUIRE(a->per_sample && !a->ab, "pw_mlp_proj: takes the per-sample (norm-folded) expand operands");
  PYTC_REQUIRE(a->w3_format == PYTC_W3_F16, "pw_mlp_proj: the mixer's projection image must be fp16 (pytc_pw_pack_weight_paired_f16)");
  PYTC_REQUIRE(!store_y || a->y, "pw_mlp_proj: store_y without an output buffer");
  PYTC_REQUIRE(a->N >= 1 && a->rows_per_sample >= 1, "pw_mlp_proj: bad shape");
  if (!pytc_pw_mlp_proj_supported(a->C_in, a->C_hid, a->C_out, 32)) {
    set_error("pw_mlp_proj: no fused kernel for C_in=%d C_hid=%d C_out=%d", a->C_in, a->C_hid, a->C_out);
    return PYTC_ERR_UNSUPPORTED;
  }
  PYTC_REQUIRE(a->res_mode == PYTC_RES_NONE || (a->res_mode == PYTC_RES_ADD && a->res), "pw_mlp_proj: residual add or none");
  MlpParams p{};
  p.t = (const bf16_t*)a->t; p.ab = nullptr; p.w2 = (const bf16x8_t*)a->w2_packed; p.b2 = a->b2;
  p.w3 = (const bf16x8_t*)a->w3_packed; p.b3 = a->b3;
  p.rps = a->rows_per_sample; p.C_in = a->C_in; p.C_hid = a->C_hid; p.C_out = a->C_out; p.HC = a->C_hid / 32;
  p.w2_stride = (long)(a->C_hid / 16) * (a->C_in / 32) * 64;
  p.e.res = a->res; p.e.y = a->y; p.e.rps_out = a->rows_per_sample; p.e.C_out = a->C_out; p.e.res_mode = a->res_mode;
  p.head_w = (const bf16x8_t*)proj_w; p.head_b = proj_b; p.proj_y = (bf16_t*)z; p.store_y = store_y;
  p.w3_f16 = 1;
  mlp_dma_launch<3>(a, p, (hipStream_t)stream);
  PYTC_LAUNCH_CHECK("pw_mlp_proj");
  return PYTC_OK;
}

static int mlp_fwd_impl(const pytc_mlp_args* a, void* hp, void* stream, const void* hp_in = nullptr, bool round_h = false);

extern "C" int pytc_pw_mlp_bwd(const pytc_mlp_args* a, const void* hidden_pre, void* d_hidden, void* stream) {
  PYTC_REQUIRE(hidden_pre && d_hidden, "pw_mlp_bwd: null hidden buffers");
  PYTC_REQUIRE(a && a->res_mode == PYTC_RES_NONE, "pw_mlp_bwd: no residual in the backward mixer");
  return mlp_fwd_impl(a, d_hidden, stream, hidden_pre);
}

extern "C" int pytc_pw_mlp_train_fwd(const pytc_mlp_args* a, void* hidden_pre, void* stream) {
  PYTC_REQUIRE(hidden_pre, "pw_mlp_train: null hidden buffer");
  return mlp_fwd_impl(a, hidden_pre, stream);
}

extern "C" int pytc_pw_mlp_train_fwd_nostore(const pytc_mlp_args* a, void* stream) {
  return mlp_fwd_impl(a, nullptr, stream, nullptr, true);
}

extern "C" int pytc_pw_mlp_fwd(const pytc_mlp_args* a, void* stream) { return mlp_fwd_impl(a, nullptr, stream); }

static int mlp_fwd_impl(const pytc_mlp_args* a, void* hp, void* stream, const void* hp_in, bool round_h) {
  PYTC_REQUIRE(a && a->t && (a->ab || a->per_sample) && a->w2_packed && a->w3_packed && a->b2 && a->b3 && a->y, "pw_mlp: null pointer");
  PYTC_REQUIRE(!(a->ab && a->per_sample), "pw_mlp: per-sample (norm-folded) expand operands come without an affine");
  PYTC_REQUIRE(!(a->per_sample && (hp || hp_in || round_h)), "pw_mlp: the training kernels take the shared expand image and the affine");
  PYTC_REQUIRE(a->N >= 1 && a->rows_per_sample >= 1, "pw_mlp: bad shape");
  if (!mlp_shape_ok(a->C_in, a->C_hid, a->C_out)) {
    set_error("pw_mlp: no fused kernel for C_in=%d C_hid=%d C_out=%d", a->C_in, a->C_hid, a->C_out);
    return PYTC_ERR_UNSUPPORTED;
  }
  PYTC_REQUIRE(a->res_mode == PYTC_RES_NONE || a->res, "pw_mlp: residual mode without residual pointer");
  PYTC_REQUIRE(a->res_mode == PYTC_RES_NONE || a->res_mode == PYTC_RES_ADD || a->res_mode == PYTC_RES_UPSAMPLE,
               "pw_mlp: unsupported res_mode %d", a->res_mode);
  MlpParams p{};
  p.t = (const bf16_t*)a->t; p.ab = a->ab; p.w2 = (const bf16x8_t*)a->w2_packed; p.b2 = a->b2;
  p.w3 = (const bf16x8_t*)a->w3_packed; p.b3 = a->b3;
  p.rps = a->rows_per_sample; p.C_in = a->C_in; p.C_hid = a->C_hid; p.C_out = a->C_out; p.HC = a->C_hid / 32;
  p.w2_stride = (long)(a->C_hid / 16) * (a->C_in / 32) * 64;
  p.e.res = a->res; p.e.res_low = a->res_low; p.e.res_bias = a->res_bias; p.e.y = a->y;
  p.e.rps_out = a->rows_per_sample; p.e.C_out = a->C_out; p.e.res_mode = a->res_mode;
  p.e.nt = 0;
  p.e.Go_d = p.e.Go_h = p.e.Go_w = p.e.Gl_d = p.e.Gl_h = p.e.Gl_w = 0;
  p.hp = (bf16_t*)hp;
  p.hp_in = (const bf16_t*)hp_in;
  p.round_h = round_h ? 1 : 0;
  p.w3_f16 = a->w3_format == PYTC_W3_F16 ? 1 : 0;
  PYTC_REQUIRE(!(p.w3_f16 && hp_in), "pw_mlp_bwd: the backward mixer takes bf16 weight images");
  if (a->res_mode == PYTC_RES_UPSAMPLE) {
    PYTC_REQUIRE((long)a->Di * a->Hi * a->Wi == a->rows_per_sample && !(a->Di & 1) && !(a->Hi & 1) && !(a->Wi & 1),
                 "pw_mlp: RES_UPSAMPLE needs the (even) output grid");
    PYTC_REQUIRE(a->rows_per_sample < (1L << 31), "pw_mlp: RES_UPSAMPLE positions are 32-bit (rows per sample < 2^31)");
    p.e.Go_d = a->Di; p.e.Go_h = a->Hi; p.e.Go_w = a->Wi;
    p.e.Gl_d = a->Di / 2; p.e.Gl_h = a->Hi / 2; p.e.Gl_w = a->Wi / 2;
  }
  if (!hp && !hp_in && !round_h && mlp_dma_applies(a, p)) {
    mlp_dma_launch<0>(a, p, (hipStream_t)stream);
    PYTC_LAUNCH_CHECK("pw_mlp_dma");
    return PYTC_OK;
  }
  if (!dispatch_mlp(p, a->N, (hipStream_t)stream)) {
    set_error("pw_mlp: dispatch failed");
    return PYTC_ERR_UNSUPPORTED;
  }
  PYTC_LAUNCH_CHECK("pw_mlp");
  return PYTC_OK;
}
```

pytorch_connectomics_amd/csrc/pw_mlp_lds_kernels.hip:

```cpp
#include <mutex>

#include "pw_common.h"

namespace pytc {

struct MlpLdsParams {
  const bf16_t* t;
  const float* ab;
  const bf16x8_t* w2;
  const float* b2;
  const h8_t* w3;
  const float* b3;
  EpiParams e;
  long rps;
  int N, C_in, C_hid, C_out, HC;
  long w2_stride;
};

template <int KS_IN, int MO, int NT>
struct LdsTile {
  uint4 raw[KS_IN][NT];
  uint4 res[MO / 2][NT];
};

template <int KS_IN, int MO, int NT>
__device__ __forceinline__ void lds_tile_load(LdsTile<KS_IN, MO, NT>& T, const MlpLdsParams& p, int n, long row0, int r, int kb,
                                              bool with_res) {
  const bf16_t* tn = p.t + (long)n * p.rps * (KS_IN * 32);
#pragma unroll
  for (int nt = 0; nt < NT; ++nt) {
    const long o = row0 + nt * 16 + r;
    const long rr = o < p.rps ? o : p.rps - 1;
#pragma unroll
    for (int ks = 0; ks < KS_IN; ++ks) T.raw[ks][nt] = ld_stream(reinterpret_cast<const uint4*>(tn + rr * (KS_IN * 32) + ks * 32 + kb * 8), p.e.nt);
  }
  if (with_res) {
    const bf16_t* resn = reinterpret_cast<const bf16_t*>(p.e.res) + (long)n * p.rps * (MO * 16);
#pragma unroll
    for (int nt = 0; nt < NT; ++nt) {
      const long o = row0 + nt * 16 + r;
      const long rr = o < p.rps ? o : p.rps - 1;
#pragma unroll
      for (int pr = 0; pr < MO / 2; ++pr) T.res[pr][nt] = ld_stream(reinterpret_cast<const uint4*>(resn + rr * (MO * 16) + pr * 32 + kb * 8), p.e.nt);
    }
  }
}

template <int KS_IN, int MO, int NT, int NWAVES, int WPS>
__global__ void __launch_bounds__(NWAVES * 64, WPS)
pw_mlp_lds_kernel(MlpLdsParams p) {
  constexpr int CIN = KS_IN * 32, COUT = MO * 16;
  extern __shared__ __attribute__((aligned(16))) unsigned char lds_raw[];
  bf16x8_t* lw2 = reinterpret_cast<bf16x8_t*>(lds_raw);
  h8_t* lw3 = reinterpret_cast<h8_t*>(lds_raw + (size_t)p.C_hid * CIN * 2);
  float* lb2 = reinterpret_cast<float*>(lds_raw + (size_t)p.C_hid * (CIN + COUT) * 2);
  const int tid = threadIdx.x, wave = tid >> 6, lane = tid & 63;
  const int r = lane & 15, kb = lane >> 4;
  const bool folded = p.ab == nullptr;
  const int n_w2 = p.C_hid * CIN / 8, n_w3 = COUT * p.C_hid / 8;
  for (int i = tid; i < n_w3; i += NWAVES * 64) lw3[i] = p.w3[i];
  const long Ts = (p.rps + NT * 16 - 1) / (NT * 16);
  const long G = Ts * p.N;
  const long g_end = G * (blockIdx.x + 1) / gridDim.x;
  long g = G * blockIdx.x / gridDim.x;
  const bool with_res = p.e.res_mode != PYTC_RES_NONE;
  const bool ups = p.e.res_mode == PYTC_RES_UPSAMPLE;
  int staged = -1;

  while (g < g_end) {
    const int n = (int)(g / Ts);
    const long seg_end = min(g_end, (long)(n + 1) * Ts);
    if (staged < 0 || folded) {
      __syncthreads();
      const bf16x8_t* src = p.w2 + (folded ? (long)n * p.w2_stride : 0L);
      for (int i = tid; i < n_w2; i += NWAVES * 64) lw2[i] = src[i];
      const float* b2 = p.b2 + (folded ? (long)n * p.C_hid : 0L);
      for (int i = tid; i < p.C_hid; i += NWAVES * 64) lb2[i] = b2[i];
      staged = n;
      __syncthreads();
    }
    const float* an = folded ? nullptr : p.ab + (long)n * 2 * CIN;
    const long t_base = (long)n * Ts;

    for (long gt = g + wave; gt < seg_end; gt += NWAVES) {
      const long row0 = (gt - t_base) * (NT * 16);
      LdsTile<KS_IN, MO, NT> cur;
      lds_tile_load(cur, p, n, row0, r, kb, with_res);
      long orow[NT];
#pragma unroll
      for (int nt = 0; nt < NT; ++nt) orow[nt] = row0 + nt * 16 + r;

      bf16x8_t bact[KS_IN][NT];
#pragma unroll
      for (int ks = 0; ks < KS_IN; ++ks) {
        if (folded) {
#pragma unroll
          for (int nt = 0; nt < NT; ++nt) bact[ks][nt] = __builtin_bit_cast(bf16x8_t, cur.raw[ks][nt]);
        } else {
          const int k0 = ks * 32 + kb * 8;
          float av[8], bv[8];
          VecIO<float, 4>::load(an + k0, reinterpret_cast<float(&)[4]>(av[0]));
          VecIO<float, 4>::load(an + k0 + 4, reinterpret_cast<float(&)[4]>(av[4]));
          VecIO<float, 4>::load(an + CIN + k0, reinterpret_cast<float(&)[4]>(bv[0]));
          VecIO<float, 4>::load(an + CIN + k0 + 4, reinterpret_cast<float(&)[4]>(bv[4]));
#pragma unroll
          for (int nt = 0; nt < NT; ++nt) {
            float v[8];
            VecIO<bf16_t, 8>::load(reinterpret_cast<const bf16_t*>(&cur.raw[ks][nt]), v);
#pragma unroll
            for (int j = 0; j < 8; ++j) v[j] = fmaf(v[j], av[j], bv[j]);
            bact[ks][nt] = Mma<bf16_t>::from_floats(v);
          }
        }
      }
      f32x4_t acc2[MO][NT];
#pragma unroll
      for (int pr = 0; pr < MO / 2; ++pr) {
        float b[8];
        VecIO<float, 4>::load(p.b3 + pr * 32 + kb * 8, reinterpret_cast<float(&)[4]>(b[0]));
        VecIO<float, 4>::load(p.b3 + pr * 32 + kb * 8 + 4, reinterpret_cast<float(&)[4]>(b[4]));
#pragma unroll
        for (int nt = 0; nt < NT; ++nt) {
          acc2[2 * pr][nt] = f32x4_t{b[0], b[1], b[2], b[3]};
          acc2[2 * pr + 1][nt] = f32x4_t{b[4], b[5], b[6], b[7]};
        }
      }
      for (int hc = 0; hc < p.HC; ++hc) {
        const f32x4_t b2lo = *reinterpret_cast<const f32x4_t*>(lb2 + hc * 32 + kb * 8);
        const f32x4_t b2hi = *reinterpret_cast<const f32x4_t*>(lb2 + hc * 32 + kb * 8 + 4);
        f32x4_t acc1[2][NT];
#pragma unroll
        for (int nt = 0; nt < NT; ++nt) { acc1[0][nt] = b2lo; acc1[1][nt] = b2hi; }
#pragma unroll
        for (int mt = 0; mt < 2; ++mt) {
#pragma unroll
          for (int ks = 0; ks < KS_IN; ++ks) {
            const bf16x8_t a = lw2[((hc * 2 + mt) * KS_IN + ks) * 64 + lane];
#pragma unroll
            for (int nt = 0; nt < NT; ++nt) acc1[mt][nt] = Mma<bf16_t>::mma(a, bact[ks][nt], acc1[mt][nt]);
          }
        }
        h8_t bhh[NT];
#pragma unroll
        for (int nt = 0; nt < NT; ++nt) {
          float gg[8];
#pragma unroll
          for (int j = 0; j < 4; ++j) { gg[j] = acc1[0][nt][j]; gg[4 + j] = acc1[1][nt][j]; }
          bhh[nt] = gelu_h8_from_f32(gg);
        }
#pragma unroll
        for (int mo = 0; mo < MO; ++mo) {
          const h8_t a = lw3[(mo * p.HC + hc) * 64 + lane];
#pragma unroll
          for (int nt = 0; nt < NT; ++nt) acc2[mo][nt] = __builtin_amdgcn_mfma_f32_16x16x32_f16(a, bhh[nt], acc2[mo][nt], 0, 0, 0);
        }
      }
      int upos[NT][3];
      if (ups) {
        const unsigned ur = (unsigned)row0, gw = (unsigned)p.e.Go_w, gh = (unsigned)p.e.Go_h;
        const unsigned t0 = ur / gw;
        const int bx = (int)(ur - t0 * gw);
        const int bz = (int)(t0 / gh);
        const int by = (int)(t0 - (unsigned)bz * gh);
#pragma unroll
        for (int nt = 0; nt < NT; ++nt) {
          int px = bx + nt * 16 + r, py = by, pz = bz;
          while (px >= p.e.Go_w) { px -= p.e.Go_w; ++py; }
          while (py >= p.e.Go_h) { py -= p.e.Go_h; ++pz; }
          upos[nt][0] = pz; upos[nt][1] = py; upos[nt][2] = px;
        }
      }
#pragma unroll
      for (int pr = 0; pr < MO / 2; ++pr) {
#pragma unroll
        for (int nt = 0; nt < NT; ++nt) {
          if (orow[nt] >= p.rps) continue;
          float v[8];
#pragma unroll
          for (int j = 0; j < 4; ++j) { v[j] = acc2[2 * pr][nt][j]; v[4 + j] = acc2[2 * pr + 1][nt][j]; }
          if (with_res) {
            float pre[8];
            VecIO<bf16_t, 8>::load(reinterpret_cast<const bf16_t*>(&cur.res[pr][nt]), pre);
            finish_and_store<bf16_t, 8, false, COUT>(v, p.e, n, orow[nt], pr * 32 + kb * 8, pre, ups ? upos[nt] : nullptr);
          } else {
            finish_and_store<bf16_t, 8, false, COUT>(v, p.e, n, orow[nt], pr * 32 + kb * 8, nullptr, nullptr);
          }
        }
      }
    }
    g = seg_end;
  }
}

template <int KS_IN, int MO, int NT, int NWAVES, int WPS>
static void launch_mlp_lds_v(const MlpLdsParams& p, size_t lds, hipStream_t s) {
  auto kern = &pw_mlp_lds_kernel<KS_IN, MO, NT, NWAVES, WPS>;
  if (!ensure_dynamic_lds(reinterpret_cast<const void*>(kern), 160 * 1024, "pw_mlp_lds")) return;
  const long tiles = ((p.rps + NT * 16 - 1) / (NT * 16)) * p.N;
  const int by_lds = (int)((160 * 1024) / lds), by_waves = WPS * 4 / NWAVES;
  const int per_cu = by_lds < by_waves ? (by_lds < 1 ? 1 : by_lds) : by_waves;
  long blocks = 256L * per_cu;
  const long need = (tiles + NWAVES - 1) / NWAVES;
  if (blocks > need) blocks = need;
  hipLaunchKernelGGL(kern, dim3((unsigned)blocks), dim3(NWAVES * 64), lds, s, p);
}

template <int KS_IN, int MO, int NT>
static void launch_mlp_lds(const MlpLdsParams& p, int variant, hipStream_t s) {
  const size_t lds = (size_t)p.C_hid * (p.C_in + p.C_out) * 2 + (size_t)p.C_hid * 4;
  if (variant == 0) variant = (KS_IN == 4 && MO == 8) ? 3 : (MO == 2 ? 2 : 4);
  switch (variant) {
    case 1: launch_mlp_lds_v<KS_IN, MO, NT, 8, 4>(p, lds, s); break;
    case 2: launch_mlp_lds_v<KS_IN, MO, NT, 16, 4>(p, lds, s); break;
    case 3: launch_mlp_lds_v<KS_IN, MO, NT, 8, 2>(p, lds, s); break;
    default: launch_mlp_lds_v<KS_IN, MO, NT, 12, 3>(p, lds, s); break;
  }
}

}

using namespace pytc;

extern "C" int pytc_pw_mlp_lds_supported(int C_in, int C_hid, int C_out) {
  if (C_in % 32 || C_hid % 32 || C_out % 32) return 0;
  const int ks = C_in / 32, mo = C_out / 16;
  const bool shape = (ks == 2 && mo == 2) || (ks == 2 && mo == 4) || (ks == 4 && mo == 4) || (ks == 4 && mo == 8);
  const size_t lds = (size_t)C_hid * (C_in + C_out) * 2 + (size_t)C_hid * 4;
  return (shape && lds <= 160 * 1024) ? 1 : 0;
}

extern "C" int pytc_pw_mlp_lds_fwd(const pytc_mlp_args* a, void* stream) {
  PYTC_REQUIRE(a && a->t && (a->ab || a->per_sample) && a->w2_packed && a->w3_packed && a->b2 && a->b3 && a->y, "pw_mlp_lds: null pointer");
  PYTC_REQUIRE(!(a->ab && a->per_sample), "pw_mlp_lds: per-sample (norm-folded) expand operands come without an affine");
  PYTC_REQUIRE(a->w3_format == PYTC_W3_F16, "pw_mlp_lds: the projection image must be fp16 (pytc_pw_pack_weight_paired_f16)");
  PYTC_REQUIRE(a->N >= 1 && a->rows_per_sample >= 1, "pw_mlp_lds: bad shape");
  if (!pytc_pw_mlp_lds_supported(a->C_in, a->C_hid, a->C_out)) {
    set_error("pw_mlp_lds: no LDS-resident kernel for C_in=%d C_hid=%d C_out=%d", a->C_in, a->C_hid, a->C_out);
    return PYTC_ERR_UNSUPPORTED;
  }
  PYTC_REQUIRE(a->res_mode == PYTC_RES_NONE || a->res, "pw_mlp_lds: residual mode without residual pointer");
  MlpLdsParams p{};
  p.t = (const bf16_t*)a->t; p.ab = a->ab; p.w2 = (const bf16x8_t*)a->w2_packed; p.b2 = a->b2;
  p.w3 = (const h8_t*)a->w3_packed; p.b3 = a->b3;
  p.rps = a->rows_per_sample; p.N = a->N; p.C_in = a->C_in; p.C_hid = a->C_hid; p.C_out = a->C_out; p.HC = a->C_hid / 32;
  p.w2_stride = (long)(a->C_hid / 16) * (a->C_in / 32) * 64;
  p.e.res = a->res; p.e.res_low = a->res_low; p.e.res_bias = a->res_bias; p.e.y = a->y;
  p.e.rps_out = a->rows_per_sample; p.e.C_out = a->C_out; p.e.res_mode = a->res_mode;
  p.e.nt = 0;
  p.e.Go_d = p.e.Go_h = p.e.Go_w = p.e.Gl_d = p.e.Gl_h = p.e.Gl_w = 0;
  if (a->res_mode == PYTC_RES_UPSAMPLE) {
    PYTC_REQUIRE((long)a->Di * a->Hi * a->Wi == a->rows_per_sample && !(a->Di & 1) && !(a->Hi & 1) && !(a->Wi & 1) &&
                 a->rows_per_sample < (1L << 31), "pw_mlp_lds: RES_UPSAMPLE needs the (even) output grid");
    p.e.Go_d = a->Di; p.e.Go_h = a->Hi; p.e.Go_w = a->Wi;
    p.e.Gl_d = a->Di / 2; p.e.Gl_h = a->Hi / 2; p.e.Gl_w = a->Wi / 2;
  }
  hipStream_t s = (hipStream_t)stream;
  const int ks = a->C_in / 32, mo = a->C_out / 16;
  const int variant = tuning_get(K_mlp_lds_variant);
  if (ks == 2 && mo == 2) launch_mlp_lds<2, 2, 2>(p, variant, s);
  else if (ks == 2 && mo == 4) launch_mlp_lds<2, 4, 2>(p, variant, s);
  else if (ks == 4 && mo == 4) launch_mlp_lds<4, 4, 2>(p, variant, s);
  else launch_mlp_lds<4, 8, 2>(p, variant, s);
  PYTC_LAUNCH_CHECK("pw_mlp_lds");
  return PYTC_OK;
}
```

pytorch_connectomics_amd/csrc/pw_mlp_up_kernels.hip:

```cpp
#include "pw_common.h"

namespace pytc {

struct MlpUpParams {
  const bf16_t* xlow;
  const float* taps;
  const float* b1;
  const float* ab;
  const bf16x8_t* w2;
  const float* b2;
  const bf16x8_t* w3;
  const float* b3;
  const bf16_t* skip;
  const bf16_t* res_low;
  const float* res_bias;
  bf16_t* y;
  int N, D, H, W, XS;
  int C_in, C_hid, C_out, HC;
  long tiles;
};

constexpr int up_waves_per_simd(int ks, int mo) {
  const int regs = ks * 4 * 4 + mo * 4 * 4 + 2 * 4 * 4 + 8 * 4 + (mo / 2) * 4 * 4;
  return regs <= 112 ? 3 : (regs <= 200 ? 2 : 1);
// ... 90 lines not shown
      const f32x2_t w0{wa[0], wa[1]}, w1{wa[2], wa[3]}, w2{wb[0], wb[1]}, w3{wb[2], wb[3]};
      asm volatile("v_pk_fma_f32 %0, %1, %2, %0" : "+v"(acc[0]) : "v"(x0), "v"(w0));
      asm volatile("v_pk_fma_f32 %0, %1, %2, %0" : "+v"(acc[1]) : "v"(x1), "v"(w1));
      asm volatile("v_pk_fma_f32 %0, %1, %2, %0" : "+v"(acc[2]) : "v"(x2), "v"(w2));
      asm volatile("v_pk_fma_f32 %0, %1, %2, %0" : "+v"(acc[3]) : "v"(x3), "v"(w3));
      if (u.last) {
        const int nt = u.nt, py = nt >> 1, px = nt & 1;
        const bool face = (Pz == 0) | (2 * my + py == 0) | (2 * mxc + px == 0);
        float t8[8];
#pragma unroll
        for (int j = 0; j < 4; ++j) { t8[2 * j] = face ? 0.f : acc[j][0]; t8[2 * j + 1] = face ? 0.f : acc[j][1]; }
        const f32x8_t tr = __builtin_convertvector(Mma<bf16_t>::from_floats(t8), f32x8_t);
        float v[8];
#pragma unroll
        for (int j = 0; j < 8; ++j) v[j] = fmaf(tr[j], av[j], bv[j]);
        bact[ks][nt] = Mma<bf16_t>::from_floats(v);
      }
    }
    __builtin_amdgcn_sched_barrier(0);
  }

  uint4 sk[MO / 2][NT];
  const bf16_t* skn = p.skip + (long)n * (2L * p.D) * Ho * Wo * p.C_out;
#pragma unroll
  for (int nt = 0; nt < NT; ++nt)
#pragma unroll
    for (int pr = 0; pr < MO / 2; ++pr)
      sk[pr][nt] = *reinterpret_cast<const uint4*>(skn + (long)orow[nt] * p.C_out + pr * 32 + kb * 8);

  f32x4_t acc2[MO][NT];
#pragma unroll
  for (int pr = 0; pr < MO / 2; ++pr) {
    float b[8];
    VecIO<float, 4>::load(p.b3 + pr * 32 + kb * 8, reinterpret_cast<float(&)[4]>(b[0]));
    VecIO<float, 4>::load(p.b3 + pr * 32 + kb * 8 + 4, reinterpret_cast<float(&)[4]>(b[4]));
#pragma unroll
    for (int nt = 0; nt < NT; ++nt) {
      acc2[2 * pr][nt] = f32x4_t{b[0], b[1], b[2], b[3]};
      acc2[2 * pr + 1][nt] = f32x4_t{b[4], b[5], b[6], b[7]};
    }
  }

  for (int hc = 0; hc < p.HC; ++hc) {
    float b2v[8];
    VecIO<float, 4>::load(p.b2 + hc * 32 + kb * 8, reinterpret_cast<float(&)[4]>(b2v[0]));
    VecIO<float, 4>::load(p.b2 + hc * 32 + kb * 8 + 4, reinterpret_cast<float(&)[4]>(b2v[4]));
    f32x4_t acc1[2][NT];
#pragma unroll
    for (int nt = 0; nt < NT; ++nt) {
      acc1[0][nt] = f32x4_t{b2v[0], b2v[1], b2v[2], b2v[3]};
      acc1[1][nt] = f32x4_t{b2v[4], b2v[5], b2v[6], b2v[7]};
    }
#pragma unroll
    for (int mt = 0; mt < 2; ++mt) {
#pragma unroll
      for (int ks = 0; ks < KS_IN; ++ks) {
        const bf16x8_t a = p.w2[((long)(hc * 2 + mt) * KS_IN + ks) * 64 + lane];
#pragma unroll
        for (int nt = 0; nt < NT; ++nt) acc1[mt][nt] = Mma<bf16_t>::mma(a, bact[ks][nt], acc1[mt][nt]);
      }
    }
    bf16x8_t bh[NT];
#pragma unroll
    for (int nt = 0; nt < NT; ++nt) {
      float g[8];
#pragma unroll
      for (int j = 0; j < 4; ++j) {
        g[j] = gelu_fast(acc1[0][nt][j]);
        g[4 + j] = gelu_fast(acc1[1][nt][j]);
      }
      bh[nt] = Mma<bf16_t>::from_floats(g);
    }
#pragma unroll
    for (int mo = 0; mo < MO; ++mo) {
      const bf16x8_t a = p.w3[((long)mo * p.HC + hc) * 64 + lane];
#pragma unroll
      for (int nt = 0; nt < NT; ++nt) acc2[mo][nt] = Mma<bf16_t>::mma(a, bh[nt], acc2[mo][nt]);
    }
  }

  if (!live) return;
  bf16_t* yn = p.y + (long)n * (2L * p.D) * Ho * Wo * p.C_out;
#pragma unroll
  for (int nt = 0; nt < NT; ++nt) {
    const int py = nt >> 1, px = nt & 1;
    const bool face = (Pz == 0) | (2 * my + py == 0) | (2 * mx + px == 0);
    const bool odd = pz & py & px;
#pragma unroll
    for (int pr = 0; pr < MO / 2; ++pr) {
      const int o0 = pr * 32 + kb * 8;
      float v[8], s[8];
#pragma unroll
      for (int j = 0; j < 4; ++j) { v[j] = acc2[2 * pr][nt][j]; v[4 + j] = acc2[2 * pr + 1][nt][j]; }
      VecIO<bf16_t, 8>::load(reinterpret_cast<const bf16_t*>(&sk[pr][nt]), s);
      if (face) {
#pragma unroll
        for (int j = 0; j < 8; ++j) v[j] = s[j];
      } else {
        float rl[8];
        if (p.res_low && odd) {
          VecIO<bf16_t, 8>::load(p.res_low + ((((long)n * p.D + mz) * p.H + my) * p.W + mx) * p.C_out + o0, rl);
        } else {
          VecIO<float, 4>::load(p.res_bias + o0, reinterpret_cast<float(&)[4]>(rl[0]));
          VecIO<float, 4>::load(p.res_bias + o0 + 4, reinterpret_cast<float(&)[4]>(rl[4]));
        }
#pragma unroll
        for (int j = 0; j < 8; ++j) v[j] = v[j] + rl[j] + s[j];
      }
      VecIO<bf16_t, 8>::store(yn + (long)orow[nt] * p.C_out + o0, v);
    }
  }
}

template <int KS_IN, int MO>
__global__ void __launch_bounds__(256, up_waves_per_simd(KS_IN, MO))
pw_mlp_up_kernel(MlpUpParams p) {
  static_assert(MO % 2 == 0, "C_out must be a multiple of 32");
  extern __shared__ __attribute__((aligned(16))) float wl[];
  for (int i = threadIdx.x; i < 27 * p.C_in; i += 256) wl[i] = p.taps[i];
  __syncthreads();
  const int wave = __builtin_amdgcn_readfirstlane(threadIdx.x >> 6), lane = threadIdx.x & 63;
  const int tile = (int)blockIdx.x * 4 + wave;
  if (tile >= (int)p.tiles) return;
  int tq = tile;
  const int xs = tq % p.XS; tq /= p.XS;
  const int my = tq % p.H; tq /= p.H;
  const int pz = tq & 1; tq >>= 1;
  const int mz = tq % p.D;
  const int n = tq / p.D;
  if (pz) up_tile<KS_IN, MO, 1>(p, wl, n, mz, my, xs, lane);
  else up_tile<KS_IN, MO, 0>(p, wl, n, mz, my, xs, lane);
}

template <int KS_IN, int MO>
static void launch_up(const MlpUpParams& p, hipStream_t s) {
  dim3 grid((unsigned)((p.tiles + 3) / 4)), block(256);
  const size_t lds = (size_t)27 * p.C_in * sizeof(float);
  hipLaunchKernelGGL((pw_mlp_up_kernel<KS_IN, MO>), grid, block, lds, s, p);
}

}

using namespace pytc;

extern "C" int pytc_pw_mlp_up_supported(int C_in, int C_hid, int C_out) {
  if (C_hid % 32 || C_hid < 32) return 0;
  return ((C_in == 64 && C_out == 32) || (C_in == 128 && C_out == 64)) ? 1 : 0;
}

extern "C" int pytc_pw_mlp_up_fwd(const pytc_mlp_args* a, const float* taps, const float* dw_bias, void* stream) {
  PYTC_REQUIRE(a && a->t && a->ab && a->w2_packed && a->w3_packed && a->b2 && a->b3 && a->y && a->res && taps && dw_bias &&
               a->res_bias, "pw_mlp_up: null pointer (dw_bias and res_bias are zero vectors when unused)");
  PYTC_REQUIRE(a->N >= 1 && a->Di >= 1 && a->Hi >= 1 && a->Wi >= 1, "pw_mlp_up: bad shape");
  if (!pytc_pw_mlp_up_supported(a->C_in, a->C_hid, a->C_out)) {
    set_error("pw_mlp_up: no fused kernel for C_in=%d C_hid=%d C_out=%d", a->C_in, a->C_hid, a->C_out);
    return PYTC_ERR_UNSUPPORTED;
  }
  MlpUpParams p{};
  p.xlow = (const bf16_t*)a->t; p.taps = taps; p.b1 = dw_bias; p.ab = a->ab;
  p.w2 = (const bf16x8_t*)a->w2_packed; p.b2 = a->b2; p.w3 = (const bf16x8_t*)a->w3_packed; p.b3 = a->b3;
  p.skip = (const bf16_t*)a->res; p.res_low = (const bf16_t*)a->res_low; p.res_bias = a->res_bias; p.y = (bf16_t*)a->y;
  p.N = a->N; p.D = a->Di; p.H = a->Hi; p.W = a->Wi; p.XS = (a->Wi + 15) / 16;
  p.C_in = a->C_in; p.C_hid = a->C_hid; p.C_out = a->C_out; p.HC = a->C_hid / 32;
  p.tiles = (long)a->N * a->Di * 2 * a->Hi * p.XS;
  PYTC_REQUIRE(p.tiles < (1L << 31) - 8, "pw_mlp_up: too many tiles");
  hipStream_t s = (hipStream_t)stream;
  if (a->C_in == 64) launch_up<2, 2>(p, s);
  else launch_up<4, 4>(p, s);
  PYTC_LAUNCH_CHECK("pw_mlp_up");
  return PYTC_OK;
}
```

pytorch_connectomics_amd/csrc/pytc_common.h:

```cpp
#pragma once
#include <hip/hip_runtime.h>
#include <stdint.h>
#include <stdio.h>
#include <string.h>

#include "../../include/pytc_hip.h"

namespace pytc {

typedef __bf16 bf16_t;
typedef __bf16 bf16x2_t __attribute__((ext_vector_type(2)));
typedef __bf16 bf16x4_t __attribute__((ext_vector_type(4)));
typedef __bf16 bf16x8_t __attribute__((ext_vector_type(8)));
typedef float f32x2_t __attribute__((ext_vector_type(2)));
typedef float f32x4_t __attribute__((ext_vector_type(4)));
typedef float f32x8_t __attribute__((ext_vector_type(8)));
typedef float f32x16_t __attribute__((ext_vector_type(16)));
typedef short s16x8_t __attribute__((ext_vector_type(8)));

constexpr int WAVE = 64;

void set_error(const char* fmt, ...);
int hip_fail(hipError_t e, const char* what);
bool ensure_dynamic_lds(const void* kernel, size_t bytes, const char* what);
bool take_launch_failure();

#define PYTC_REQUIRE(cond, ...)                     \
  do {                                              \
    if (!(cond)) {                                  \
      pytc::set_error(__VA_ARGS__);                 \
      return PYTC_ERR_INVALID;                      \
    }                                               \
  } while (0)

#define PYTC_LAUNCH_CHECK(name)                                  \
  do {                                                           \
    if (pytc::take_launch_failure()) return PYTC_ERR_HIP;        \
    hipError_t e_ = hipGetLastError();                           \
    if (e_ != hipSuccess) return pytc::hip_fail(e_, name);       \
  } while (0)

#define PYTC_KNOBS(X)                                                                                                             \
  X(channel_act_flat, 1, "channel activation of contiguous NDHWC tensors as a flat 16-byte stream; 0 = the per-voxel kernel")      \
  X(conv_wgrad_mfma, 1, "dense-conv weight gradient on the matrix cores (bf16); 0 = the VALU kernel")                              \
  X(dw_wgrad_march, 1, "depthwise K = 3 / stride 1 weight gradient as a z-march; 0 = the vector / generic kernels")                \
  X(dw_wgrad_vec, 1, "depthwise K = 3 weight gradient with 16-byte channel vectors; 0 = the generic kernel")                       \
  X(dwconvT_tile, 1, "transposed depthwise conv at C = 64 / 128 (bf16) as one tile of input cells per workgroup; 0 = cell kernel") \
  X(dwconv_march_h16, 1, "VALU z-march depthwise conv: packed-f16 in-plane partial sums; 0 = fp32 taps")                           \
  X(dwconv_mfma, 1, "bf16 stride-1 K = 3 depthwise forward (and the fused block) on the matrix cores; 0 = the VALU z-march")       \
  X(dwconv_mfma_variant, 0, "matrix-core depthwise conv: bit 0 = hi + lo weight halves, bit 1 = two planes in flight, not three")  \
  X(dwconv_s2_march, 1, "stride-2 K = 3 depthwise conv at C = 32 / 64 (bf16) as a z-march over an LDS ring; 0 = gather kernel")    \
  X(elementwise_vec, 1, "16-byte vector forms of the norm-apply / elementwise training kernels; 0 = the scalar kernels")           \
  X(mixer_bwd_rc_slot_div, 1, "recomputing mixer backward: divide the slot count (fewer, longer slots)")                           \
  X(mlp_chunk_variant, 0, "chunked-hidden mixer (pw_mlp_chunk_kernels.hip): tile shape of the launch")                             \
  X(mlp_dma, 1, "level-0 mixer with DMA-prefetched row tiles (pw_mlp_dma_kernel); 0 = one tile per wave")                          \
  X(mlp_dma_rows, 1 << 20, "fewest rows of a launch that takes the DMA mixer")                                                     \
  X(mlp_dma_wgs, 0, "DMA mixer: workgroups per sample; 0 = chosen from the row count")                                             \
  X(mlp_lds_variant, 0, "LDS-resident mixer (pw_mlp_lds_kernels.hip): tile shape of the launch")                                   \
  X(norm_bwd_from_wgrad_flat, 1, "GroupNorm-backward epilogue of the expand weight gradient as one flat kernel; 0 = chunked")      \
  X(pw_gemm_rows, 0, "LDS-tiled 1x1 GEMM: 64 / 128 forces the rows per workgroup; 0 = by problem size")                            \
  X(pw_thin, 1, "plain 1x1 convs with one input / few output channels on the thin kernels; 0 = the generic kernel")                \
  X(wgrad_dgrad_fused, 1, "projecting conv's weight gradient and the GELU-backward data gradient in one kernel; 0 = two launches")  \
  X(wgrad_small_split, 1, "matrix-core 1x1 weight gradient: more, shorter row slots when the launch would leave CUs idle")         \
  X(wgrad_valu, 0, "1: 1x1 weight gradient on the VALU kernel instead of the matrix cores")                                        \
  X(wgrad_whole_rounds, 1, "matrix-core 1x1 weight gradient: round the slot count down to whole rounds of resident workgroups")

enum Knob {
#define PYTC_KNOB_ENUM(name, dflt, doc) K_##name,
  PYTC_KNOBS(PYTC_KNOB_ENUM)
#undef PYTC_KNOB_ENUM
  K_COUNT
};
int tuning_get(Knob k);

template <typename T, int VEC>
struct VecIO;

template <int VEC>
struct VecIO<float, VEC> {
  typedef float vec_t __attribute__((ext_vector_type(VEC)));
  static __device__ __forceinline__ void load(const float* p, float (&v)[VEC]) {
    vec_t t = *reinterpret_cast<const vec_t*>(p);
#pragma unroll
    for (int i = 0; i < VEC; ++i) v[i] = t[i];
  }
  static __device__ __forceinline__ void store(float* p, const float (&v)[VEC]) {
    vec_t t;
#pragma unroll
    for (int i = 0; i < VEC; ++i) t[i] = v[i];
    *reinterpret_cast<vec_t*>(p) = t;
  }
};
template <>
struct VecIO<float, 1> {
  static __device__ __forceinline__ void load(const float* p, float (&v)[1]) { v[0] = *p; }
  static __device__ __forceinline__ void store(float* p, const float (&v)[1]) { *p = v[0]; }
};

template <int VEC>
struct VecIO<bf16_t, VEC> {
  typedef __bf16 vec_t __attribute__((ext_vector_type(VEC)));
  typedef float fvec_t __attribute__((ext_vector_type(VEC)));
  static __device__ __forceinline__ void load(const bf16_t* p, float (&v)[VEC]) {
    vec_t t = *reinterpret_cast<const vec_t*>(p);
    fvec_t f = __builtin_convertvector(t, fvec_t);
#pragma unroll
    for (int i = 0; i < VEC; ++i) v[i] = f[i];
  }
  static __device__ __forceinline__ void store(bf16_t* p, const float (&v)[VEC]) {
    fvec_t f;
#pragma unroll
    for (int i = 0; i < VEC; ++i) f[i] = v[i];
    *reinterpret_cast<vec_t*>(p) = __builtin_convertvector(f, vec_t);
  }
};
template <>
struct VecIO<bf16_t, 1> {
  static __device__ __forceinline__ void load(const bf16_t* p, float (&v)[1]) { v[0] = (float)*p; }
  static __device__ __forceinline__ void store(bf16_t* p, const float (&v)[1]) { *p = (bf16_t)v[0]; }
};

template <typename T>
__device__ __forceinline__ float to_f32(T v) { return (float)v; }
template <typename T>
__device__ __forceinline__ T from_f32(float v) { return (T)v; }

__device__ __forceinline__ float wave_sum(float v) {
#pragma unroll
  for (int o = 32; o > 0; o >>= 1) v += __shfl_xor(v, o, 64);
  return v;
}

template <int THREADS, typename T>
__device__ __forceinline__ T block_sum(T v, T* red) {
  red[threadIdx.x] = v;
  __syncthreads();
  for (int s = THREADS / 2; s > 0; s >>= 1) {
    if ((int)threadIdx.x < s) red[threadIdx.x] += red[threadIdx.x + s];
    __syncthreads();
  }
  const T r = red[0];
  __syncthreads();
  return r;
}

__device__ __forceinline__ float gelu_erf(float x) {
  const float az = fabsf(x) * 0.70710678118654752440f;
  const float t = __builtin_amdgcn_rcpf(fmaf(0.3275911f, az, 1.0f));
  float p = fmaf(t, 1.061405429f, -1.453152027f);
  p = fmaf(t, p, 1.421413741f);
  p = fmaf(t, p, -0.284496736f);
  p = fmaf(t, p, 0.254829592f);
  p *= t;
  const float pe = p * __builtin_amdgcn_exp2f(-az * az * 1.44269504088896340736f);
  const float one_plus_erf = x < 0.f ? pe : 2.0f - pe;
  return 0.5f * x * one_plus_erf;
}

__device__ __forceinline__ float gelu_erf_grad(float x) {
  const float az = fabsf(x) * 0.70710678118654752440f;
  const float t = __builtin_amdgcn_rcpf(fmaf(0.3275911f, az, 1.0f));
  float p = fmaf(t, 1.061405429f, -1.453152027f);
  p = fmaf(t, p, 1.421413741f);
  p = fmaf(t, p, -0.284496736f);
  p = fmaf(t, p, 0.254829592f);
  p *= t;
  const float e = __builtin_amdgcn_exp2f(-az * az * 1.44269504088896340736f);
  const float pe = p * e;
  const float one_plus_erf = x < 0.f ? pe : 2.0f - pe;
  return fmaf(x * 0.3989422804014327f, e, 0.5f * one_plus_erf);
}

__device__ __forceinline__ float gelu_fast(float x) {
  const float x2 = fminf(x * x, 64.0f);
  float p = fmaf(x2, 1.0142630e-3f, -1.0677572e-1f);
  p = fmaf(p, x2, -2.3011213f);
  const float e = __builtin_amdgcn_exp2f(x * p);
  return x * __builtin_amdgcn_rcpf(1.0f + e);
}

__device__ __forceinline__ void gelu_fast_with_grad(float x, float& g, float& gd) {
  const float x2 = fminf(x * x, 64.0f);
  float p = fmaf(x2, 1.0142630e-3f, -1.0677572e-1f);
  p = fmaf(p, x2, -2.3011213f);
  const float e = __builtin_amdgcn_exp2f(x * p);
  const float s = __builtin_amdgcn_rcpf(1.0f + e);
  g = x * s;
  const float q = fmaf(x2, 2.0f * 1.0142630e-3f, -1.0677572e-1f);
  const float du = fmaf(x2 + x2, q, p);
  gd = fmaf(g * (1.0f - s), du * -0.69314718055994530942f, s);
}

typedef _Float16 h2_t __attribute__((ext_vector_type(2)));
typedef _Float16 h8_t __attribute__((ext_vector_type(8)));

__device__ __forceinline__ h2_t gelu_h2(h2_t x) {
  const h2_t U = {(_Float16)3.75f, (_Float16)3.75f};
  const h2_t u = __builtin_elementwise_min(__builtin_elementwise_abs(x), U);
  const h2_t t = u * (h2_t){(_Float16)(2.0f / 3.75f), (_Float16)(2.0f / 3.75f)} + (h2_t){(_Float16)-1.0f, (_Float16)-1.0f};
#define PYTC_H2C(v) ((h2_t){(_Float16)(v), (_Float16)(v)})
  h2_t p = PYTC_H2C(-6.166994737e-02f);
  p = p * t + PYTC_H2C(6.367329291e-02f);
  p = p * t + PYTC_H2C(1.683184914e-01f);
  p = p * t + PYTC_H2C(-3.056981228e-01f);
  p = p * t + PYTC_H2C(7.903670132e-02f);
  p = p * t + PYTC_H2C(1.852329106e-01f);
  p = p * t + PYTC_H2C(-1.855973189e-01f);
  p = p * t + PYTC_H2C(5.694380662e-02f);
#undef PYTC_H2C
  return __builtin_elementwise_max(x, (h2_t){(_Float16)0.0f, (_Float16)0.0f}) - p;
}
// ... 42 lines not shown
```

pytorch_connectomics_amd/hip_ops.py:

```python
from __future__ import annotations

import ctypes as C
from typing import Optional, Sequence

import torch

from . import _native as nat

_DT = {torch.float32: nat.F32, torch.bfloat16: nat.BF16}


def dtype_code(dt: torch.dtype) -> int:
    try:
        return _DT[dt]
    except KeyError:
        raise TypeError(f"pytorch_connectomics_amd kernels support float32/bfloat16, got {dt}") from None


def require_device(device, what: str = "this inference path") -> None:
    if torch.device(device).type != "cuda":
        raise RuntimeError(f"{what} (pytorch_connectomics_amd) needs a CUDA(HIP) device: there is no CPU path")


def _on_device(t: torch.Tensor, name: str) -> torch.Tensor:
# ... 446 lines not shown
    return bool(nat.lib().pytc_pw_conv_paired_supported(C.byref(a)))


def _mlp_symbol(a, plain: str, kind: int) -> str:
    if not PROFILER.enabled:
        return plain
    if nat.lib().pytc_pw_mlp_dma_applies(C.byref(a), 1 if kind == 1 else 0):
        return f"pw_mlp_dma_kernel<{int(a.C_hid) // 32}, {kind}>"
    return plain


def pw_mlp_supported(c_in: int, c_hid: int, c_out: int) -> bool:
    return bool(nat.lib().pytc_pw_mlp_supported(int(c_in), int(c_hid), int(c_out)))


MLP_F16_PROJECT = True


def pw_pack_weight_paired(w: torch.Tensor, *, transposed: bool = False, f16: bool = False) -> torch.Tensor:
    _dev(w, "w")
    if w.dtype != torch.float32 or w.dim() != 2:
        raise ValueError("pointwise weight must be float32 2-D")
    c_out, c_in = (w.shape[1], w.shape[0]) if transposed else (w.shape[0], w.shape[1])
    n = nat.lib().pytc_pw_packed_elems(c_out, c_in, nat.BF16)
    packed = torch.empty((n,), dtype=torch.float16 if f16 else torch.bfloat16, device=w.device)
    fn = nat.lib().pytc_pw_pack_weight_paired_f16 if f16 else nat.lib().pytc_pw_pack_weight_paired
    _run("pw_pack_weight_paired", _nbytes(w, packed), fn, _p(w), c_out, c_in, int(transposed), _p(packed), _stream())
    return packed


PACK_PAIRED, PACK_PAIRED_T, PACK_PAIRED_F16, PACK_PAIRED_F16_T, PACK_TAPS, PACK_TAPS_FLIPPED, PACK_ROWMAJOR, PACK_ROWMAJOR_T = range(8)


class StepPacks:

    def __init__(self):
        self.rows = []
        self.index = {}
        self.table = None
        self.total = 0

    def lookup(self, w: torch.Tensor, kind: int):
        i = self.index.get((w.data_ptr(), kind))
        if i is None:
            return None
        row = self.rows[i]
        return row[1] if row[7] == w._version else None

    def register(self, w: torch.Tensor, kind: int, out: torch.Tensor, c_out: int, c_in: int, aux: int) -> None:
        key = (w.data_ptr(), kind)
        i = self.index.get(key)
        row = [w, out, int(kind), int(c_out), int(c_in), int(aux), int(out.numel()), w._version]
        if i is None:
            self.index[key] = len(self.rows)
            self.rows.append(row)
        else:
            self.rows[i] = row
        self.table = None

    def refresh(self) -> None:
        if not self.rows or all(r[7] == r[0]._version for r in self.rows):
            return
        dev = self.rows[0][1].device
        if self.table is None:
            flat, pos = [], 0
            for src, out, kind, c_out, c_in, aux, n, _ver in self.rows:
                flat += [src.data_ptr(), out.data_ptr(), kind, c_out, c_in, aux, pos, n]
                pos += n
            self.table = torch.tensor(flat, dtype=torch.int64).to(dev)
            self.total = pos
        _run("pack_multi", self.total * 6, nat.lib().pytc_pack_multi, _p(self.table), len(self.rows), self.total, _stream())
        for r in self.rows:
            r[7] = r[0]._version


def packed_paired(w_mat: torch.Tensor, *, transposed: bool = False, f16: bool = False, packs: Optional[StepPacks] = None):
    if packs is None:
        return pw_pack_weight_paired(w_mat, transposed=transposed, f16=f16)
    kind = (PACK_PAIRED_F16 if f16 else PACK_PAIRED) + (1 if transposed else 0)
    hit = packs.lookup(w_mat, kind)
    if hit is not None:
        return hit
    out = pw_pack_weight_paired(w_mat, transposed=transposed, f16=f16)
    c_out, c_in = (w_mat.shape[1], w_mat.shape[0]) if transposed else (w_mat.shape[0], w_mat.shape[1])
    packs.register(w_mat, kind, out, c_out, c_in, (c_in + 31) // 32)
    return out


def packed_rowmajor(w_mat: torch.Tensor, *, transposed: bool = False, packs: Optional[StepPacks] = None) -> torch.Tensor:
    kind = PACK_ROWMAJOR_T if transposed else PACK_ROWMAJOR
    if packs is not None:
        hit = packs.lookup(w_mat, kind)
        if hit is not None:
            return hit
    out = (w_mat.t() if transposed else w_mat).to(torch.bfloat16).contiguous()
    if packs is not None:
        c_out, c_in = (w_mat.shape[1], w_mat.shape[0]) if transposed else (w_mat.shape[0], w_mat.shape[1])
        packs.register(w_mat, kind, out, c_out, c_in, 0)
    return out


def pw_conv_rowmajor_supported(*, c_in: int, c_out: int, in_dtype: torch.dtype, out_dtype: torch.dtype, act: int = nat.ACT_NONE,
                               gather: int = 0) -> bool:
    a = nat.PwArgs()
    a.C_in, a.C_out, a.act, a.gather = int(c_in), int(c_out), int(act), int(gather)
    try:
        a.in_dtype, a.out_dtype, a.w_dtype = dtype_code(in_dtype), dtype_code(out_dtype), dtype_code(torch.bfloat16)
    except Exception:
        return False
    return bool(nat.lib().pytc_pw_conv_rowmajor_supported(C.byref(a)))


def packed_taps(w: torch.Tensor, *, flipped: bool = False, packs: Optional[StepPacks] = None) -> torch.Tensor:
    c, k3 = w.shape[0], w.shape[-1] ** 3
    src = w.detach()
    kind = PACK_TAPS_FLIPPED if flipped else PACK_TAPS
    if packs is not None and src.dtype == torch.float32 and src.is_contiguous():
        hit = packs.lookup(src, kind)
        if hit is not None:
            return hit
    out = src.float().reshape(c, k3).t().contiguous()
    if flipped:
        out = torch.flip(out, dims=[0]).contiguous()
    if packs is not None and src.dtype == torch.float32 and src.is_contiguous():
        packs.register(src, kind, out, c, 1, k3)
    return out


def _check_out(y: torch.Tensor, numel: int, dtype: torch.dtype, what: str) -> None:
    _dev(y, "y")
    if y.dtype != dtype or y.numel() != numel or not y.is_contiguous():
        raise ValueError(f"{what}: output buffer must be a contiguous {dtype} tensor of {numel} elements, got "
                         f"{tuple(y.shape)} {y.dtype} contiguous={y.is_contiguous()}")


def _w3_format(w3p: torch.Tensor) -> int:
    return nat.W3_F16 if w3p.dtype == torch.float16 else nat.W3_BF16


def _folded_operands(ab, w2p: torch.Tensor, b2: torch.Tensor, N: int, c_in: int, c_hid: int) -> int:
    if ab is not None:
        return 0
    if tuple(w2p.shape) != (N, c_hid * c_in) or tuple(b2.shape) != (N, c_hid) or w2p.dtype != torch.bfloat16:
        raise ValueError(f"norm-folded mixer operands must be w2n (N, C_hid*C_in) bf16 and b2n (N, C_hid); got {tuple(w2p.shape)} "
                         f"{w2p.dtype} / {tuple(b2.shape)}")
    return 1


def pw_mlp(t: torch.Tensor, ab: Optional[torch.Tensor], w2p: torch.Tensor, b2: torch.Tensor, w3p: torch.Tensor,
           b3: torch.Tensor, *, N: int, rows_per_sample: int, c_in: int, c_hid: int, c_out: int,
           res: Optional[torch.Tensor] = None, res_mode: int = nat.RES_NONE, grid: Sequence[int] = (0, 0, 0),
           res_low: Optional[torch.Tensor] = None, res_bias: Optional[torch.Tensor] = None,
           y: Optional[torch.Tensor] = None, hidden_pre: Optional[torch.Tensor] = None, lds: bool = False,
           chunked: bool = False, train_nostore: bool = False) -> torch.Tensor:
    _dev(t, "t")
    if t.dtype != torch.bfloat16:
        raise TypeError("pw_mlp runs on bfloat16 activations")
    if y is None:
        y = torch.empty((N, rows_per_sample, c_out), dtype=torch.bfloat16, device=t.device)
    else:
        _check_out(y, N * rows_per_sample * c_out, torch.bfloat16, "pw_mlp")
    a = nat.MlpArgs()
    a.t, a.ab, a.w2_packed, a.b2, a.w3_packed, a.b3 = (t.data_ptr(), None if ab is None else ab.data_ptr(), w2p.data_ptr(),
                                                       b2.data_ptr(), w3p.data_ptr(), b3.data_ptr())
    a.per_sample = _folded_operands(ab, w2p, b2, N, c_in, c_hid)
    a.w3_format = _w3_format(w3p)
    a.res = res.data_ptr() if res is not None else None
    a.res_low = res_low.data_ptr() if res_low is not None else None
    a.res_bias = res_bias.data_ptr() if res_bias is not None else None
    a.y = y.data_ptr()
    a.N, a.rows_per_sample, a.C_in, a.C_hid, a.C_out, a.res_mode = N, rows_per_sample, c_in, c_hid, c_out, res_mode
    a.Di, a.Hi, a.Wi = (int(v) for v in grid)
    nb = N * rows_per_sample * 2 * (c_in + c_out + (c_out if res is not None else 0))
    if hidden_pre is not None:
        _dev(hidden_pre, "hidden_pre")
        _run(f"pw_mlp_train_fwd[{c_in}->{c_hid}->{c_out}]", nb + N * rows_per_sample * 2 * c_hid, nat.lib().pytc_pw_mlp_train_fwd,
             C.byref(a), _p(hidden_pre), _stream())
        return y
    if train_nostore:
        _run(f"pw_mlp_train_fwd_nostore[{c_in}->{c_hid}->{c_out}]", nb, nat.lib().pytc_pw_mlp_train_fwd_nostore, C.byref(a), _stream(),
             symbol=f"pw_mlp_kernel<{c_in // 32}, {c_out // 16}>")
        return y
    if lds:
        _run(f"pw_mlp_fwd[{c_in}->{c_hid}->{c_out}]", nb, nat.lib().pytc_pw_mlp_lds_fwd, C.byref(a), _stream(),
             symbol=f"pw_mlp_lds_kernel<{c_in // 32}, {c_out // 16}>")
        return y
    if chunked:
        _run(f"pw_mlp_fwd[{c_in}->{c_hid}->{c_out}]", nb, nat.lib().pytc_pw_mlp_chunk_fwd, C.byref(a), _stream(),
             symbol=f"pw_mlp_chunk_kernel<{c_in // 32}, {c_out // 16}>")
        return y
    _run(f"pw_mlp_fwd[{c_in}->{c_hid}->{c_out}]", nb, nat.lib().pytc_pw_mlp_fwd, C.byref(a), _stream(),
         symbol=_mlp_symbol(a, f"pw_mlp_kernel<{c_in // 32}, {c_out // 16}>", 0))
    return y


def pw_mlp_lds_supported(c_in: int, c_hid: int, c_out: int) -> bool:
    return bool(nat.lib().pytc_pw_mlp_lds_supported(int(c_in), int(c_hid), int(c_out)))


def pw_mlp_chunk_supported(c_in: int, c_hid: int, c_out: int) -> bool:
    return bool(nat.lib().pytc_pw_mlp_chunk_supported(int(c_in), int(c_hid), int(c_out)))


def pw_gemm_supported(c_in: int, c_out: int) -> bool:
    return bool(nat.lib().pytc_pw_gemm_supported(int(c_in), int(c_out)))


def pw_gemm(x: torch.Tensor, w: torch.Tensor, bias: torch.Tensor, *, N: int, rows_per_sample: int, ab: Optional[torch.Tensor] = None,
            gelu: bool = False, res: Optional[torch.Tensor] = None, res_mode: int = nat.RES_NONE, grid: Sequence[int] = (0, 0, 0),
            res_low: Optional[torch.Tensor] = None, res_bias: Optional[torch.Tensor] = None,
            y: Optional[torch.Tensor] = None) -> torch.Tensor:
    _dev(x, "x"); _dev(w, "w")
    c_out, c_in = int(w.shape[0]), int(w.shape[1])
    if x.dtype not in (torch.bfloat16, torch.float16) or w.dtype != x.dtype or not w.is_contiguous() or int(x.shape[-1]) != c_in:
        raise TypeError(f"pw_gemm: x {tuple(x.shape)} {x.dtype} / w {tuple(w.shape)} {w.dtype}: same 16-bit type, w (C_out, C_in) contiguous")
    out_dt = torch.float16 if gelu else torch.bfloat16
    if y is None:
        y = torch.empty((N, rows_per_sample, c_out), dtype=out_dt, device=x.device)
    else:
        _check_out(y, N * rows_per_sample * c_out, out_dt, "pw_gemm")
    nb = N * rows_per_sample * 2 * (c_in + c_out + (c_out if res is not None else 0)) + 2 * c_in * c_out
    _run(f"pw_gemm[{c_in}->{c_out}]", nb, nat.lib().pytc_pw_gemm_fwd, _p(x), _p(w), _p(bias), _p(ab), _p(y), N, rows_per_sample, c_in,
         c_out, int(x.dtype == torch.float16), int(gelu), _p(res), _p(res_low), _p(res_bias), int(res_mode), *(int(v) for v in grid),
         _stream(), flops=2 * N * rows_per_sample * c_in * c_out, symbol="pw_gemm_lds_kernel")
    return y


def pw_mlp_up_supported(c_in: int, c_hid: int, c_out: int) -> bool:
    return bool(nat.lib().pytc_pw_mlp_up_supported(int(c_in), int(c_hid), int(c_out)))


def pw_mlp_up(x_low: torch.Tensor, taps: torch.Tensor, dw_bias: Optional[torch.Tensor], ab: torch.Tensor, w2p: torch.Tensor,
              b2: torch.Tensor, w3p: torch.Tensor, b3: torch.Tensor, skip: torch.Tensor, *, c_hid: int, c_out: int,
              res_low: Optional[torch.Tensor] = None, res_bias: Optional[torch.Tensor] = None) -> torch.Tensor:
    _dev(x_low, "x_low"); _dev(skip, "skip"); _dev(taps, "taps")
    if x_low.dtype != torch.bfloat16 or skip.dtype != torch.bfloat16:
        raise TypeError("pw_mlp_up runs on bfloat16 activations")
    N, D, H, W, c_in = x_low.shape
    if tuple(skip.shape) != (N, 2 * D, 2 * H, 2 * W, c_out):
        raise ValueError(f"pw_mlp_up: skip shape {tuple(skip.shape)} does not match the up-sampled grid")
    y = torch.empty((N, 2 * D, 2 * H, 2 * W, c_out), dtype=torch.bfloat16, device=x_low.device)
    a = nat.MlpArgs()
    a.t, a.ab, a.w2_packed, a.b2, a.w3_packed, a.b3 = (x_low.data_ptr(), ab.data_ptr(), w2p.data_ptr(), b2.data_ptr(),
                                                       w3p.data_ptr(), b3.data_ptr())
    if w3p.dtype != torch.bfloat16:
        raise TypeError("pw_mlp_up takes the bf16 image of the projection weights")
    a.res = skip.data_ptr()
    if dw_bias is None:
        dw_bias = torch.zeros((c_in,), dtype=torch.float32, device=x_low.device)
    if res_bias is None:
        res_bias = torch.zeros((c_out,), dtype=torch.float32, device=x_low.device)
    a.res_low = res_low.data_ptr() if res_low is not None else None
    a.res_bias = res_bias.data_ptr()
    a.y = y.data_ptr()
    a.N, a.rows_per_sample, a.C_in, a.C_hid, a.C_out, a.res_mode = N, 8 * D * H * W, c_in, c_hid, c_out, nat.RES_UPSAMPLE
    a.Di, a.Hi, a.Wi = D, H, W
    nb = _nbytes(x_low, skip, y) + (_nbytes(res_low) if res_low is not None else 0)
    _run(f"pw_mlp_up_fwd[{c_in}->{c_hid}->{c_out}]", nb, nat.lib().pytc_pw_mlp_up_fwd, C.byref(a), _p(taps), _p(dw_bias),
         _stream())
    return y


def stem_dwconv3d_supported(c_in: int, c: int, K: int) -> bool:
    return bool(nat.lib().pytc_stem_dwconv3d_supported(int(c_in), int(c), int(K)))


def stem_dwconv3d_pack(stem_w: torch.Tensor, stem_b: torch.Tensor, w_taps: torch.Tensor, bias: Optional[torch.Tensor]):
    wx = (w_taps * stem_w.view(1, -1)).contiguous()
    wb = (w_taps * stem_b.view(1, -1)).contiguous()
    cst = (wb.sum(0) + (bias if bias is not None else 0.0)).contiguous()
    image = torch.empty((nat.lib().pytc_stem_dwconv3d_mfma_image_bytes(),), dtype=torch.uint8, device=wx.device)
    _run("stem_dwconv3d_pack_mfma", 0, nat.lib().pytc_stem_dwconv3d_pack_mfma, _p(wx), _p(wb), _p(cst), _p(image), _stream())
    return wx, wb, cst, image


def stem_dwconv3d(x: torch.Tensor, packed):
    wx, wb, cst, image = packed
    _dev(x, "x"); _dev(wx, "wx")
    if x.dtype != torch.float32 or x.shape[-1] != 1:
        raise TypeError("stem_dwconv3d takes the 1-channel fp32 network input")
    N, D, H, W, _ = x.shape
    Cc = wx.shape[1]
    y = torch.empty((N, D, H, W, Cc), dtype=torch.bfloat16, device=x.device)
    slots = nat.lib().pytc_stem_dwconv3d_stat_slots(D, H, W)
    st = torch.empty((N, slots, 2, Cc), dtype=torch.float32, device=x.device)
    _run(f"stem_dwconv3d_fwd[C{Cc}_k3]", _nbytes(x, y), nat.lib().pytc_stem_dwconv3d_fwd, _p(x), _p(wx), _p(wb), _p(cst),
         _p(image), _p(y), _p(st), N, D, H, W, Cc, _stream())
    return y, st


def pw_mlp_stemres(t: torch.Tensor, ab: torch.Tensor, w2p: torch.Tensor, b2: torch.Tensor, w3p: torch.Tensor, b3: torch.Tensor,
                   x0: torch.Tensor, stem_w: torch.Tensor, stem_b: torch.Tensor, *, N: int, rows_per_sample: int, c_in: int,
                   c_hid: int, c_out: int, y: Optional[torch.Tensor] = None) -> torch.Tensor:
    _dev(t, "t"); _dev(x0, "x0")
    if t.dtype != torch.bfloat16 or x0.dtype != torch.float32:
        raise TypeError("pw_mlp_stemres: bf16 activations and the fp32 network input")
    if y is None:
        y = torch.empty((N, rows_per_sample, c_out), dtype=torch.bfloat16, device=t.device)
    else:
        _check_out(y, N * rows_per_sample * c_out, torch.bfloat16, "pw_mlp_stemres")
    a = nat.MlpArgs()
    a.t, a.ab, a.w2_packed, a.b2, a.w3_packed, a.b3 = (t.data_ptr(), None if ab is None else ab.data_ptr(), w2p.data_ptr(),
                                                       b2.data_ptr(), w3p.data_ptr(), b3.data_ptr())
    a.per_sample = _folded_operands(ab, w2p, b2, N, c_in, c_hid)
    a.w3_format = _w3_format(w3p)
    a.res = a.res_low = a.res_bias = None
    a.y = y.data_ptr()
    a.N, a.rows_per_sample, a.C_in, a.C_hid, a.C_out, a.res_mode = N, rows_per_sample, c_in, c_hid, c_out, nat.RES_ADD
    a.Di = a.Hi = a.Wi = 0
    nb = N * rows_per_sample * (2 * (c_in + c_out) + 4)
    _run(f"pw_mlp_fwd[{c_in}->{c_hid}->{c_out}]", nb, nat.lib().pytc_pw_mlp_stemres_fwd, C.byref(a), _p(x0), _p(stem_w),
         _p(stem_b), _stream(), symbol=_mlp_symbol(a, f"pw_mlp_kernel<{c_in // 32}, {c_out // 16}>+stemres", 1))
    return y


_MLP_BWD_CONSTS: dict = {}


def pw_mlp_bwd(dy: torch.Tensor, hidden_pre: torch.Tensor, w3t_p: torch.Tensor, w2t_p: torch.Tensor, *, N: int,
               rows_per_sample: int, c_in: int, c_hid: int, c_out: int):
    _dev(dy, "dy"); _dev(hidden_pre, "hidden_pre")
    if dy.dtype != torch.bfloat16:
        raise TypeError("pw_mlp_bwd runs on bfloat16 activations")
    dev = dy.device
    dx = torch.empty((N, rows_per_sample, c_in), dtype=torch.bfloat16, device=dev)
    dh = torch.empty((N, rows_per_sample, c_hid), dtype=torch.bfloat16, device=dev)
    key = (dev, N, c_in, c_hid, c_out)
    consts = _MLP_BWD_CONSTS.get(key)
    if consts is None:
        consts = (torch.cat([torch.ones((N, 1, c_out), device=dev), torch.zeros((N, 1, c_out), device=dev)], 1).contiguous(),
                  torch.zeros((c_hid,), device=dev), torch.zeros((c_in,), device=dev))
        _MLP_BWD_CONSTS[key] = consts
    ident, zh, zi = consts
    a = nat.MlpArgs()
    a.t, a.ab, a.w2_packed, a.b2, a.w3_packed, a.b3 = (dy.data_ptr(), ident.data_ptr(), w3t_p.data_ptr(), zh.data_ptr(),
                                                       w2t_p.data_ptr(), zi.data_ptr())
    a.w3_format = nat.W3_BF16
    a.res = a.res_low = a.res_bias = None
    a.y = dx.data_ptr()
    a.N, a.rows_per_sample, a.C_in, a.C_hid, a.C_out, a.res_mode = N, rows_per_sample, c_out, c_hid, c_in, nat.RES_NONE
    a.Di = a.Hi = a.Wi = 0
    nb = N * rows_per_sample * 2 * (c_out + 2 * c_hid + c_in)
    _run(f"pw_mlp_bwd[{c_out}->{c_hid}->{c_in}]", nb, nat.lib().pytc_pw_mlp_bwd, C.byref(a), _p(hidden_pre), _p(dh), _stream())
    return dx, dh


# ... 1686 lines not shown
```

pytorch_connectomics_amd/models/architectures/mednext.py:

```python
from __future__ import annotations

import os
from typing import Dict, List, Optional, Sequence, Union

import torch
import torch.nn as nn

from ... import _native as nat
from ... import hip_ops as ops

SMALL_ROWS_TWO_GEMMS = int(os.environ.get("PYTC_MIXER_TWO_GEMM_ROWS", "0"))

L0_SUBBATCH = int(os.environ.get("PYTC_L0_SUBBATCH", "0"))


def _conv_nd(dim: str):
    if dim == "3d":
        return nn.Conv3d, nn.ConvTranspose3d
    if dim == "2d":
        return nn.Conv2d, nn.ConvTranspose2d
    raise ValueError(f"dim must be '2d' or '3d', got {dim!r}")


class _ChannelLayerNorm(nn.Module):
# ... 236 lines not shown
        if kind == "up":
            t, st = ops.dwconv3d(x, taps, b1, K=K, transposed=True, stats=not is_ln)
            count = float((2 * D - 1) * (2 * H - 1) * (2 * W - 1))
        else:
            t, st = ops.dwconv3d(x, taps, b1, K=K, stride=2 if kind == "down" else 1, stats=not is_ln)
            count = float(t.shape[1] * t.shape[2] * t.shape[3])
        gamma, beta = self._vec(m.norm, "weight", m.norm.weight), self._vec(m.norm, "bias", m.norm.bias)
        if is_ln:
            t = ops.layernorm_rows(t, gamma, beta, m.norm.eps)
            ab = None
        else:
            ab = None
        _, Do, Ho, Wo, _ = t.shape
        rows = Do * Ho * Wo
        small = (self.fused and dt == torch.bfloat16 and not m.grn and not is_ln and N * rows < SMALL_ROWS_TWO_GEMMS
                 and ops.pw_conv_paired_supported(c_in=C, c_out=c_hid, in_dtype=dt, out_dtype=dt)
                 and ops.pw_conv_paired_supported(c_in=c_hid, c_out=c_out, in_dtype=dt, out_dtype=dt))
        if (not small and self.fused and dt == torch.bfloat16 and not m.grn and not is_ln and m.conv2.bias is not None
                and m.conv3.bias is not None and head is None and ops.MLP_F16_PROJECT
                and (rows <= self.deep_gemm_rows or (self.deep_gemm_cin and C >= self.deep_gemm_cin))
                and ops.pw_gemm_supported(C, c_hid) and ops.pw_gemm_supported(c_hid, c_out)):
            ab = ops.groupnorm_finalize(st, count, gamma, beta, m.norm.eps)
            return self._block_deep_gemm(m, x, t, ab, skip, (N, D, H, W, C), (Do, Ho, Wo), c_hid, c_out, out)
        if (not small and self.fused and dt == torch.bfloat16 and not m.grn and not is_ln and m.conv2.bias is not None
                and m.conv3.bias is not None and ops.pw_mlp_supported(C, c_hid, c_out)):
            ab, w2x, b2x = self._fold(m, st, count, C, c_hid)
            if (head is not None and kind == "block" and head.weight.shape[1] <= 16
                    and ops.pw_mlp_head_supported(C, c_hid, c_out)):
                _, logits = ops.pw_mlp_head(t, ab, w2x, b2x,
                                            self._pw_paired(m.conv3, project=True), self._vec(m.conv3, "bias", m.conv3.bias),
                                            self._head_w(head), self._vec(head, "bias", head.bias), N=N,
                                            rows_per_sample=rows, c_in=C, c_hid=c_hid, c_out=c_out,
                                            res=x if m.do_res else None, store_y=False)
                return None, logits.view(N, Do, Ho, Wo, -1)
            if (proj is not None and head is None and out is None and kind == "block" and ab is None and ops.MLP_F16_PROJECT
                    and tuple(proj.weight.shape[:2]) == (32, c_out) and ops.pw_mlp_proj_supported(C, c_hid, c_out, 32)):
                _, z = ops.pw_mlp_proj(t, w2x, b2x, self._pw_paired(m.conv3, project=True), self._vec(m.conv3, "bias", m.conv3.bias),
                                       self._pw_paired(proj), self._vec(proj, "bias", proj.bias), N=N, rows_per_sample=rows, c_in=C,
                                       c_hid=c_hid, c_out=c_out, res=x if m.do_res else None, store_y=False)
                return None, z.view(N, Do, Ho, Wo, 32)
            return self._block_fused(m, x, t, ab, skip, (N, D, H, W, C), (Do, Ho, Wo), c_hid, c_out, out, w2x, b2x)
        if not is_ln:
            ab = ops.groupnorm_finalize(st, count, gamma, beta, m.norm.eps)
        G = {}
        if small:
            h = ops.pw_conv(t, self._pw_paired(m.conv2), self._vec(m.conv2, "bias", m.conv2.bias), N=N, rows_per_sample=rows,
                            c_in=C, c_out=c_hid, out_dtype=dt, ab=ab, w_paired=True)
            w3, b3 = self._pw_paired(m.conv3), self._vec(m.conv3, "bias", m.conv3.bias)
            G = dict(pre_act=nat.ACT_GELU, w_paired=True)
        else:
            h = ops.pw_conv(t, self._pw(m.conv2, dt), self._vec(m.conv2, "bias", m.conv2.bias), N=N,
                            rows_per_sample=rows, c_in=C, c_out=c_hid, out_dtype=dt, ab=ab, act=nat.ACT_GELU)
            if m.grn:
                h = self._grn(m, h, N, (Do, Ho, Wo), c_hid, kind)
            w3, b3 = self._pw(m.conv3, dt), self._vec(m.conv3, "bias", m.conv3.bias)
        if kind == "block":
            y = ops.pw_conv(h, w3, b3, N=N, rows_per_sample=rows, c_in=c_hid, c_out=c_out, out_dtype=dt,
                            res=x if m.do_res else None, res_mode=nat.RES_ADD if m.do_res else nat.RES_NONE, **G)
        elif kind == "down":
            res = None
            if m.resample_do_res:
                res = ops.pw_conv(x, self._pw(m.res_conv, dt), self._vec(m.res_conv, "bias", m.res_conv.bias),
                                  N=N, rows_per_sample=rows, c_in=C, c_out=c_out, out_dtype=dt, gather=2,
                                  grid=(D, H, W))
            y = ops.pw_conv(h, w3, b3, N=N, rows_per_sample=rows, c_in=c_hid, c_out=c_out, out_dtype=dt,
                            res=res, res_mode=nat.RES_ADD if res is not None else nat.RES_NONE, **G)
        else:
            if skip is None:
                skip = torch.zeros((N, Do, Ho, Wo, c_out), dtype=dt, device=x.device)
            res_low = res_bias = None
            if m.resample_do_res:
                res_bias = self._vec(m.res_conv, "bias", m.res_conv.bias)
                res_low = ops.pw_conv(x, self._pw(m.res_conv, dt, transposed=True), res_bias, N=N,
                                      rows_per_sample=D * H * W, c_in=C, c_out=c_out, out_dtype=dt)
            y = ops.pw_conv(h, w3, b3, N=N, rows_per_sample=rows, c_in=c_hid, c_out=c_out, out_dtype=dt,
                            res=skip, res_mode=nat.RES_UPSAMPLE, grid=(Do, Ho, Wo), res_low=res_low,
                            res_bias=res_bias, **G)
        return y.view(N, Do, Ho, Wo, c_out)


def _block_dwmix(self, m, x, taps, b1, c_hid, c_out, head=None, out=None):
    N, D, H, W, C = x.shape
    _, st = ops.dwconv3d(x, taps, b1, K=3, store=False)
    w2n, b2n = ops.groupnorm_fold_mlp(st, float(D * H * W), self._vec(m.norm, "weight", m.norm.weight), self._vec(m.norm, "bias", m.norm.bias),
                                      m.norm.eps, self._w2_matrix(m.conv2), self._vec(m.conv2, "bias", m.conv2.bias))
    w3, b3 = self._pw_paired(m.conv3, project=True), self._vec(m.conv3, "bias", m.conv3.bias)
    if head is not None:
        _, logits = ops.dwmix(x, taps, b1, w2n, b2n, w3, b3, c_hid=c_hid, c_out=c_out, residual=bool(m.do_res),
                              head_w=self._head_w(head), head_b=self._vec(head, "bias", head.bias), store_y=False)
        return None, logits
    if out is not None and tuple(out.shape) != (N, D, H, W, c_out):
        raise ValueError(f"block output buffer {tuple(out.shape)} != {(N, D, H, W, c_out)}")
    return ops.dwmix(x, taps, b1, w2n, b2n, w3, b3, c_hid=c_hid, c_out=c_out, residual=bool(m.do_res), y=out)


HipBlockOps._block_dwmix = None


def _stem_block_fused(self, stem: nn.Module, m, x_cl: torch.Tensor, out: Optional[torch.Tensor] = None) -> Optional[torch.Tensor]:
    N, D, H, W, cin = x_cl.shape
    C = stem.weight.shape[0]
    K = m.conv1.weight.shape[-1]
    if (cin != 1 or x_cl.dtype != torch.float32 or stem.bias is None or m.kind != "block" or not m.do_res or m.grn
            or not isinstance(m.norm, nn.GroupNorm) or m.dim != "3d" or m.conv2.bias is None or m.conv3.bias is None
            or m.conv1.weight.shape[0] != C or W % 4 != 0 or not ops.stem_dwconv3d_supported(cin, C, K)):
        return None
    c_hid, c_out = m.conv2.weight.shape[0], m.conv3.weight.shape[0]
    if c_out != C or not ops.pw_mlp_supported(C, c_hid, c_out):
        return None
    sw = self.cache.get(("stemw", id(stem)), [stem.weight], lambda: stem.weight.detach().float().reshape(-1).bfloat16().float().contiguous())
    sb = self._vec(stem, "bias", stem.bias)
    taps, _ = self._taps(m.conv1)
    packed = self.cache.get(("stemdw", id(stem), id(m.conv1)), [stem.weight, stem.bias, m.conv1.weight, m.conv1.bias],
                            lambda: ops.stem_dwconv3d_pack(sw, sb, taps, self._vec(m.conv1, "bias", m.conv1.bias)))
    t, st = ops.stem_dwconv3d(x_cl, packed)
    rows = D * H * W
    ab, w2x, b2x = self._fold(m, st, float(rows), C, c_hid)
    y = ops.pw_mlp_stemres(t, ab, w2x, b2x,
                           self._pw_paired(m.conv3, project=True), self._vec(m.conv3, "bias", m.conv3.bias), x_cl.reshape(N, rows), sw, sb,
                           N=N, rows_per_sample=rows, c_in=C, c_hid=c_hid, c_out=c_out,
                           y=None if out is None else out.view(N, rows, c_out))
    return y.view(N, D, H, W, c_out)


HipBlockOps._stem_block_fused = None


def _block_fused(self, m, x, t, ab, skip, ishape, oshape, c_hid, c_out, out=None, w2=None, b2=None):
    N, D, H, W, C = ishape
    Do, Ho, Wo = oshape
    rows = Do * Ho * Wo
    dt = torch.bfloat16
    if w2 is None:
        w2, b2 = self._pw_paired(m.conv2), self._vec(m.conv2, "bias", m.conv2.bias)
    w3, b3 = self._pw_paired(m.conv3, project=True), self._vec(m.conv3, "bias", m.conv3.bias)
    kw = dict(N=N, rows_per_sample=rows, c_in=C, c_hid=c_hid, c_out=c_out)
    if (self.lds_mixer_rows and N * rows >= self.lds_mixer_rows and w3.dtype == torch.float16
            and ops.pw_mlp_lds_supported(C, c_hid, c_out)):
        kw["lds"] = True
    chunk_ok = (self.chunk_mixer_rows and N * rows >= self.chunk_mixer_rows and w3.dtype == torch.float16
                and ops.pw_mlp_chunk_supported(C, c_hid, c_out))
    if chunk_ok and (c_hid >= self.chunk_mixer_hid or (C, c_out) == (128, 64)):
        kw.pop("lds", None)
        kw["chunked"] = True
    if out is not None:
        if tuple(out.shape) != (N, Do, Ho, Wo, c_out):
            raise ValueError(f"block output buffer {tuple(out.shape)} != {(N, Do, Ho, Wo, c_out)}")
        kw["y"] = out.view(N, rows, c_out)
    if m.kind == "block":
        y = ops.pw_mlp(t, ab, w2, b2, w3, b3, res=x if m.do_res else None,
                       res_mode=nat.RES_ADD if m.do_res else nat.RES_NONE, **kw)
    elif m.kind == "down":
        res = None
        if m.resample_do_res:
            paired = ops.pw_conv_paired_supported(c_in=C, c_out=c_out, in_dtype=dt, out_dtype=dt, gather=2)
            wres = self._pw_paired(m.res_conv) if paired else self._pw(m.res_conv, dt)
            res = ops.pw_conv(x, wres, self._vec(m.res_conv, "bias", m.res_conv.bias), N=N, rows_per_sample=rows,
                              c_in=C, c_out=c_out, out_dtype=dt, gather=2, grid=(D, H, W), w_paired=paired)
        y = ops.pw_mlp(t, ab, w2, b2, w3, b3, res=res, res_mode=nat.RES_ADD if res is not None else nat.RES_NONE, **kw)
    else:
        if skip is None:
            skip = torch.zeros((N, Do, Ho, Wo, c_out), dtype=dt, device=x.device)
        res_low = res_bias = None
        if m.resample_do_res:
            res_bias = self._vec(m.res_conv, "bias", m.res_conv.bias)
            paired = ops.pw_conv_paired_supported(c_in=C, c_out=c_out, in_dtype=dt, out_dtype=dt)
            wres = self._pw_paired(m.res_conv, transposed=True) if paired else self._pw(m.res_conv, dt, transposed=True)
            res_low = ops.pw_conv(x, wres, res_bias, N=N, rows_per_sample=D * H * W, c_in=C, c_out=c_out,
                                  out_dtype=dt, w_paired=paired)
        y = ops.pw_mlp(t, ab, w2, b2, w3, b3, res=skip, res_mode=nat.RES_UPSAMPLE, grid=(Do, Ho, Wo),
                       res_low=res_low, res_bias=res_bias, **kw)
    return y.view(N, Do, Ho, Wo, c_out)


def _block_deep_gemm(self, m, x, t, ab, skip, ishape, oshape, c_hid, c_out, out=None):
    N, D, H, W, C = ishape
    Do, Ho, Wo = oshape
    rows = Do * Ho * Wo
    dt = torch.bfloat16
    w2 = self.cache.get(("gw2", id(m.conv2)), [m.conv2.weight],
                        lambda: m.conv2.weight.detach().float().reshape(c_hid, C).to(torch.bfloat16).contiguous())
    w3 = self.cache.get(("gw3", id(m.conv3)), [m.conv3.weight],
                        lambda: m.conv3.weight.detach().float().reshape(c_out, c_hid).to(torch.float16).contiguous())
    b2, b3 = self._vec(m.conv2, "bias", m.conv2.bias), self._vec(m.conv3, "bias", m.conv3.bias)
    h = ops.pw_gemm(t.view(N, rows, C), w2, b2, N=N, rows_per_sample=rows, ab=ab, gelu=True)
    kw = dict(N=N, rows_per_sample=rows)
    if out is not None:
        kw["y"] = out.view(N, rows, c_out)
    if m.kind == "block":
        y = ops.pw_gemm(h, w3, b3, res=x if m.do_res else None, res_mode=nat.RES_ADD if m.do_res else nat.RES_NONE, **kw)
    elif m.kind == "down":
        res = None
        if m.resample_do_res:
            paired = ops.pw_conv_paired_supported(c_in=C, c_out=c_out, in_dtype=dt, out_dtype=dt, gather=2)
            wres = self._pw_paired(m.res_conv) if paired else self._pw(m.res_conv, dt)
            res = ops.pw_conv(x, wres, self._vec(m.res_conv, "bias", m.res_conv.bias), N=N, rows_per_sample=rows,
                              c_in=C, c_out=c_out, out_dtype=dt, gather=2, grid=(D, H, W), w_paired=paired)
        y = ops.pw_gemm(h, w3, b3, res=res, res_mode=nat.RES_ADD if res is not None else nat.RES_NONE, **kw)
    else:
        if skip is None:
            skip = torch.zeros((N, Do, Ho, Wo, c_out), dtype=dt, device=x.device)
        res_low = res_bias = None
        if m.resample_do_res:
            res_bias = self._vec(m.res_conv, "bias", m.res_conv.bias)
            paired = ops.pw_conv_paired_supported(c_in=C, c_out=c_out, in_dtype=dt, out_dtype=dt)
            wres = self._pw_paired(m.res_conv, transposed=True) if paired else self._pw(m.res_conv, dt, transposed=True)
            res_low = ops.pw_conv(x, wres, res_bias, N=N, rows_per_sample=D * H * W, c_in=C, c_out=c_out, out_dtype=dt, w_paired=paired)
        y = ops.pw_gemm(h, w3, b3, res=skip, res_mode=nat.RES_UPSAMPLE, grid=(Do, Ho, Wo), res_low=res_low, res_bias=res_bias, **kw)
    return y.view(N, Do, Ho, Wo, c_out)


def _up_block_fused(self, m, x, skip, taps, b1, c_hid, c_out):
    N, D, H, W, C = x.shape
    dt = torch.bfloat16
    _, st = ops.dwconv3d(x, taps, b1, K=3, transposed=True, stats=True, store=False)
    ab = ops.groupnorm_finalize(st, float((2 * D - 1) * (2 * H - 1) * (2 * W - 1)), self._vec(m.norm, "weight", m.norm.weight),
                                self._vec(m.norm, "bias", m.norm.bias), m.norm.eps)
    res_low = res_bias = None
    if m.resample_do_res:
        res_bias = self._vec(m.res_conv, "bias", m.res_conv.bias)
        paired = ops.pw_conv_paired_supported(c_in=C, c_out=c_out, in_dtype=dt, out_dtype=dt)
        wres = self._pw_paired(m.res_conv, transposed=True) if paired else self._pw(m.res_conv, dt, transposed=True)
        res_low = ops.pw_conv(x, wres, res_bias, N=N, rows_per_sample=D * H * W, c_in=C, c_out=c_out, out_dtype=dt,
                              w_paired=paired)
    return ops.pw_mlp_up(x, taps, b1, ab, self._pw_paired(m.conv2), self._vec(m.conv2, "bias", m.conv2.bias),
                         self._pw_paired(m.conv3), self._vec(m.conv3, "bias", m.conv3.bias), skip.contiguous(),
                         c_hid=c_hid, c_out=c_out, res_low=res_low, res_bias=res_bias)


HipBlockOps._up_block_fused = _up_block_fused
HipBlockOps._block_deep_gemm = _block_deep_gemm
HipBlockOps._block_fused = _block_fused
HipBlockOps._stem_block_fused = _stem_block_fused
HipBlockOps._block_dwmix = _block_dwmix


def resolve_compute_dtype(module_pref: Optional[torch.dtype]) -> torch.dtype:
    if module_pref is not None:
        return module_pref
    if torch.is_autocast_enabled("cuda"):
        adt = torch.get_autocast_dtype("cuda")
        if adt == torch.bfloat16:
            return torch.bfloat16
        if adt == torch.float16:
            raise RuntimeError("fp16 autocast is not supported by the MI355X engine; use bf16-mixed")
    return torch.float32


def embed_stencil_2d(w: torch.Tensor) -> torch.Tensor:
    k = w.shape[-1]
    out = w.new_zeros((w.shape[0], w.shape[1], k, k, k))
    out[:, :, k // 2] = w
    return out


def to_channels_last(x: torch.Tensor) -> torch.Tensor:
    if x.shape[1] == 1:
        return x.reshape(x.shape[0], *x.shape[2:], 1)
    return x.permute(0, 2, 3, 4, 1).contiguous()


def to_channels_first(y: torch.Tensor) -> torch.Tensor:
    if y.shape[-1] == 1:
        return y.reshape(y.shape[0], 1, *y.shape[1:-1])
    return y.permute(0, 4, 1, 2, 3).contiguous()


class MedNeXt(nn.Module):

    def __init__(self, in_channels: int, n_channels: int, n_classes: int, exp_r: Union[int, Sequence[int]] = 4,
                 kernel_size: int = 7, enc_kernel_size: Optional[int] = None,
                 dec_kernel_size: Optional[int] = None, deep_supervision: bool = False, do_res: bool = False,
                 do_res_up_down: bool = False, checkpoint_style: Optional[str] = None,
                 block_counts: Sequence[int] = (2, 2, 2, 2, 2, 2, 2, 2, 2), norm_type: str = "group",
                 dim: str = "3d", grn: bool = False):
        super().__init__()
        if checkpoint_style not in (None, "outside_block"):
            raise ValueError("checkpoint_style must be None or 'outside_block'")
        if len(block_counts) != 9:
            raise ValueError("block_counts must have exactly 9 elements")
        self.do_ds = deep_supervision
        self.inside_block_checkpointing = False
        self.outside_block_checkpointing = checkpoint_style == "outside_block"
        self.checkpoint_policy = "auto"
        if kernel_size is not None:
            enc_kernel_size = dec_kernel_size = kernel_size
        conv, _ = _conv_nd(dim)
        if isinstance(exp_r, int):
            exp_r = [exp_r] * 9
        exp_r = list(exp_r)
        n = n_channels
        self.dim = dim
        self.stem = conv(in_channels, n, kernel_size=1)

        def blocks(c, r, k, count):
            return nn.Sequential(*[MedNeXtBlock(c, c, r, k, do_res, norm_type, dim=dim, grn=grn)
                                   for _ in range(count)])

        for lvl in range(4):
            setattr(self, f"enc_block_{lvl}", blocks(n << lvl, exp_r[lvl], enc_kernel_size, block_counts[lvl]))
            setattr(self, f"down_{lvl}", MedNeXtDownBlock(n << lvl, n << (lvl + 1), exp_r[lvl + 1], enc_kernel_size,
                                                          do_res=do_res_up_down, norm_type=norm_type, dim=dim, grn=grn))
        self.bottleneck = blocks(n << 4, exp_r[4], dec_kernel_size, block_counts[4])
        for i, lvl in enumerate((3, 2, 1, 0)):
            setattr(self, f"up_{lvl}", MedNeXtUpBlock(n << (lvl + 1), n << lvl, exp_r[5 + i], dec_kernel_size,
                                                      do_res=do_res_up_down, norm_type=norm_type, dim=dim, grn=grn))
            setattr(self, f"dec_block_{lvl}", blocks(n << lvl, exp_r[5 + i], dec_kernel_size, block_counts[5 + i]))
        self.out_0 = OutBlock(n, n_classes, dim)
        self.dummy_tensor = nn.Parameter(torch.tensor([1.0]), requires_grad=True)
        if deep_supervision:
            for h in (1, 2, 3, 4):
                setattr(self, f"out_{h}", OutBlock(n << h, n_classes, dim))
        self.block_counts = list(block_counts)
        self.compute_dtype: Optional[torch.dtype] = None
        self._hip = HipBlockOps()
        self.fuse_head = True
        self.fuse_stem = True
        self.l0_subbatch = L0_SUBBATCH

    def _check_input(self, x: torch.Tensor):
        if not x.is_cuda:
            raise RuntimeError("MedNeXt (pytorch_connectomics_amd) runs only on an MI355X/ROCm device: "
                               "there is no CPU path. Move the model and input to 'cuda'.")
        if self.dim == "2d":
# ... 165 lines not shown
```

Baseline: 1.847 billion voxels/s.

## Fuse residual 1x1 conv into MedNeXt down/up mixer kernels

```diff
diff --git a/include/pytc_hip.h b/include/pytc_hip.h
--- a/include/pytc_hip.h
+++ b/include/pytc_hip.h
@@ -7,7 +7,7 @@
 extern "C" {
 #endif
 
-#define PYTC_ABI_VERSION 12
+#define PYTC_ABI_VERSION 13
 
 #define PYTC_OK 0
 #define PYTC_ERR_INVALID 1
@@ -42,6 +42,7 @@
 #define PYTC_RES_UPSAMPLE 2
 #define PYTC_RES_GELU_BWD 3
 #define PYTC_RES_NORM_BWD 4
+#define PYTC_RES_CONV_GATHER 5
 
 int pytc_abi_version(void);
 const char* pytc_last_error(void);
@@ -200,6 +201,9 @@
 int pytc_pw_pack_weight_paired_f16(const float* w, int C_out, int C_in, int transposed, void* packed_f16,
                                    void* stream);
 int pytc_pw_mlp_fwd(const pytc_mlp_args* a, void* stream);
+int pytc_pw_mlp_res_conv_fwd(const pytc_mlp_args* a, const void* res_x, const void* res_w_packed, const float* res_conv_bias, int Dx, int Hx,
+                             int Wx, int lds, void* stream);
+int pytc_pw_mlp_res_conv_supported(int C_in, int C_hid, int C_out, int res_mode, int lds);
 
 int pytc_pw_mlp_lds_supported(int C_in, int C_hid, int C_out);
 int pytc_pw_mlp_lds_fwd(const pytc_mlp_args* a, void* stream);
diff --git a/pytorch_connectomics_amd/csrc/pw_common.h b/pytorch_connectomics_amd/csrc/pw_common.h
--- a/pytorch_connectomics_amd/csrc/pw_common.h
+++ b/pytorch_connectomics_amd/csrc/pw_common.h
@@ -67,7 +67,7 @@
 
 template <typename TO, int NCH, bool GELU_BWD = false, int COUT = 0>
 __device__ __forceinline__ void finish_and_store(float (&v)[NCH], const EpiParams& e, int n, long orow, int o0,
-                                                 const float* pre = nullptr, const int* pos = nullptr) {
+                                                 const float* pre = nullptr, const int* pos = nullptr, const float* rlow = nullptr) {
   const int C_out = COUT > 0 ? COUT : e.C_out;
   TO* yn = reinterpret_cast<TO*>(e.y) + (long)n * e.rps_out * C_out;
   const TO* resn = e.res ? reinterpret_cast<const TO*>(e.res) + (long)n * e.rps_out * C_out : nullptr;
@@ -151,7 +151,10 @@
     } else {
       const int oz = pz - 1, oy = py - 1, ox = px - 1;
       float rl[NCH];
-      if (e.res_low && !((oz | oy | ox) & 1)) {
+      if (rlow && !((oz | oy | ox) & 1)) {
+#pragma unroll
+        for (int i = 0; i < NCH; ++i) rl[i] = rlow[i];
+      } else if (e.res_low && !((oz | oy | ox) & 1)) {
         const TO* rp = reinterpret_cast<const TO*>(e.res_low) +
                        ((((long)n * e.Gl_d + (oz >> 1)) * e.Gl_h + (oy >> 1)) * e.Gl_w + (ox >> 1)) * C_out + o0;
         if (full) VecIO<TO, NCH>::load(rp, rl);
@@ -184,6 +187,21 @@
       if (o0 + i < C_out) yn[off + i] = from_f32<TO>(v[i]);
   }
 }
+
+struct MlpResConv {
+  const void* x;
+  const void* w_packed;
+  const float* bias;
+  int Dx, Hx, Wx;
+};
+int mlp_lds_fwd(const pytc_mlp_args* a, const MlpResConv* rc, void* stream);
+#define PYTC_REFUSE_RES_CONV(a, name)                                                       \
+  do {                                                                                      \
+    if ((a)->res_mode == PYTC_RES_CONV_GATHER) {                                            \
+      pytc::set_error(name ": PYTC_RES_CONV_GATHER (the residual conv inside the mixer) is not implemented by this entry"); \
+      return PYTC_ERR_UNSUPPORTED;                                                          \
+    }                                                                                       \
+  } while (0)
 
 template <typename TI, int EPL>
 __device__ __forceinline__ void load_row_frag(const TI* __restrict__ row, int k0, int C_in, bool vec_ok,
diff --git a/pytorch_connectomics_amd/csrc/pw_mlp_chunk_kernels.hip b/pytorch_connectomics_amd/csrc/pw_mlp_chunk_kernels.hip
--- a/pytorch_connectomics_amd/csrc/pw_mlp_chunk_kernels.hip
+++ b/pytorch_connectomics_amd/csrc/pw_mlp_chunk_kernels.hip
@@ -223,6 +223,7 @@
   PYTC_REQUIRE(!(a->ab && a->per_sample), "pw_mlp_chunk: per-sample (norm-folded) expand operands come without an affine");
   PYTC_REQUIRE(a->w3_format == PYTC_W3_F16, "pw_mlp_chunk: the projection image must be fp16 (pytc_pw_pack_weight_paired_f16)");
   PYTC_REQUIRE(a->N >= 1 && a->rows_per_sample >= 1, "pw_mlp_chunk: bad shape");
+  PYTC_REFUSE_RES_CONV(a, "pw_mlp_chunk");
   if (!pytc_pw_mlp_chunk_supported(a->C_in, a->C_hid, a->C_out)) {
     set_error("pw_mlp_chunk: no chunk-streamed kernel for C_in=%d C_hid=%d C_out=%d", a->C_in, a->C_hid, a->C_out);
     return PYTC_ERR_UNSUPPORTED;
diff --git a/pytorch_connectomics_amd/csrc/pw_mlp_kernels.hip b/pytorch_connectomics_amd/csrc/pw_mlp_kernels.hip
--- a/pytorch_connectomics_amd/csrc/pw_mlp_kernels.hip
+++ b/pytorch_connectomics_amd/csrc/pw_mlp_kernels.hip
@@ -26,6 +26,11 @@
   bf16_t* hp;
   int round_h;
   const bf16_t* hp_in;
+  const bf16_t* rx;
+  const bf16x8_t* rw;
+  const float* rb;
+  long rps_rx;
+  int Gi_h, Gi_w;
 };
 
 constexpr int mlp_waves_per_simd(int ks, int mo, int nt) {
@@ -34,15 +39,17 @@
   return regs <= 64 ? 4 : (regs <= 112 ? 3 : (regs <= 200 ? 2 : 1));
 }
 
-template <int KS_IN, int MO, int NT, int GELU_MODE, bool HEAD = false, bool STEMRES = false, bool STOREH = false, bool BWD = false>
-__global__ void __launch_bounds__(256, mlp_waves_per_simd(KS_IN, MO, NT))
+template <int KS_IN, int MO, int NT, int GELU_MODE, bool HEAD = false, bool STEMRES = false, bool STOREH = false, bool BWD = false,
+          bool RESCONV = false>
+__global__ void __launch_bounds__(256, mlp_waves_per_simd(KS_IN, MO, NT) + ((RESCONV && KS_IN == 2 && MO == 8) ? 1 : 0))
 pw_mlp_kernel(MlpParams p) {
+  static_assert(!RESCONV || !(HEAD || STEMRES || STOREH || BWD), "the residual conv rides the plain inference mixer");
   constexpr int CIN = KS_IN * 32, COUT = MO * 16;
   static_assert(MO % 2 == 0, "C_out must be a multiple of 32");
   static_assert(!STEMRES || (MO == 2 && (MO / 2) * NT <= 4), "the stem-recomputing residual covers C_out = 32");
   static_assert(!HEAD || MO == 2, "the fused head covers C_out = 32");
   static_assert(GELU_MODE == 1 || GELU_MODE == 3, "sigmoid-form or packed-fp16 GELU");
-  constexpr bool PREFETCH_RES = (MO / 2) * NT <= 4;
+  constexpr bool PREFETCH_RES = !RESCONV && (MO / 2) * NT <= 4;
   const int wave = threadIdx.x >> 6, lane = threadIdx.x & 63;
   const int n = blockIdx.y;
   constexpr bool WARM = KS_IN * MO >= 32;
@@ -128,6 +135,29 @@
       }
   }
 
+  constexpr bool XRES_EARLY = KS_IN == 1;
+  bf16x8_t xres[KS_IN][NT];
+  auto load_xres = [&]() {
+    const bf16_t* rxn = p.rx + (long)n * p.rps_rx * CIN;
+    const unsigned ur = (unsigned)row0, gw = (unsigned)p.e.Go_w, gh = (unsigned)p.e.Go_h;
+    const unsigned t0 = ur / gw;
+    const int bx = (int)(ur - t0 * gw);
+    const int bz = (int)(t0 / gh);
+    const int by = (int)(t0 - (unsigned)bz * gh);
+#pragma unroll
+    for (int nt = 0; nt < NT; ++nt) {
+      int px = bx + nt * 16 + r, py = by, pz = bz;
+      while (px >= p.e.Go_w) { px -= p.e.Go_w; ++py; }
+      while (py >= p.e.Go_h) { py -= p.e.Go_h; ++pz; }
+      if (orow[nt] >= p.rps) { pz = p.e.Go_d - 1; py = p.e.Go_h - 1; px = p.e.Go_w - 1; }
+      const long irow = ((long)(2 * pz) * p.Gi_h + 2 * py) * p.Gi_w + 2 * px;
+#pragma unroll
+      for (int ks = 0; ks < KS_IN; ++ks)
+        xres[ks][nt] = ld_stream(reinterpret_cast<const bf16x8_t*>(rxn + irow * CIN + ks * 32 + kb * 8), p.e.nt);
+    }
+  };
+  if constexpr (RESCONV && XRES_EARLY) load_xres();
+
   f32x4_t acc2[MO][NT];
 #pragma unroll
   for (int pr = 0; pr < MO / 2; ++pr) {
@@ -217,6 +247,8 @@
     }
   }
 
+  if constexpr (RESCONV && !XRES_EARLY) load_xres();
+
   if constexpr (HEAD) {
     bf16_t* yn = reinterpret_cast<bf16_t*>(p.e.y) + (long)n * p.rps * 32;
     const bf16_t* resn = p.e.res ? reinterpret_cast<const bf16_t*>(p.e.res) + (long)n * p.rps * 32 : nullptr;
@@ -267,6 +299,29 @@
   }
 #pragma unroll
   for (int pr = 0; pr < MO / 2; ++pr) {
+    f32x4_t racc[RESCONV ? 2 : 1][RESCONV ? NT : 1];
+    if constexpr (RESCONV) {
+      float b[8];
+#pragma unroll
+      for (int j = 0; j < 8; ++j) b[j] = 0.f;
+      if (p.rb) {
+        VecIO<float, 4>::load(p.rb + pr * 32 + kb * 8, reinterpret_cast<float(&)[4]>(b[0]));
+        VecIO<float, 4>::load(p.rb + pr * 32 + kb * 8 + 4, reinterpret_cast<float(&)[4]>(b[4]));
+      }
+#pragma unroll
+      for (int nt = 0; nt < NT; ++nt) {
+        racc[0][nt] = f32x4_t{b[0], b[1], b[2], b[3]};
+        racc[1][nt] = f32x4_t{b[4], b[5], b[6], b[7]};
+      }
+#pragma unroll
+      for (int mt = 0; mt < 2; ++mt)
+#pragma unroll
+        for (int ks = 0; ks < KS_IN; ++ks) {
+          const bf16x8_t a = p.rw[((long)(pr * 2 + mt) * KS_IN + ks) * 64 + lane];
+#pragma unroll
+          for (int nt = 0; nt < NT; ++nt) racc[mt][nt] = Mma<bf16_t>::mma(a, xres[ks][nt], racc[mt][nt]);
+        }
+    }
 #pragma unroll
     for (int nt = 0; nt < NT; ++nt) {
       if (orow[nt] >= p.rps) continue;
@@ -275,6 +330,15 @@
       for (int j = 0; j < 4; ++j) {
         v[j] = acc2[2 * pr][nt][j];
         v[4 + j] = acc2[2 * pr + 1][nt][j];
+      }
+      if constexpr (RESCONV) {
+        float rv[8], pre[8];
+#pragma unroll
+        for (int j = 0; j < 4; ++j) { rv[j] = racc[0][nt][j]; rv[4 + j] = racc[1][nt][j]; }
+        const bf16x8_t rb16 = Mma<bf16_t>::from_floats(rv);
+        VecIO<bf16_t, 8>::load(reinterpret_cast<const bf16_t*>(&rb16), pre);
+        finish_and_store<bf16_t, 8, false, COUT>(v, p.e, n, orow[nt], pr * 32 + kb * 8, pre, nullptr);
+        continue;
       }
       if (use_pre) {
         float pre[8];
@@ -677,10 +741,19 @@
   }
 }
 
+constexpr bool mlp_res_conv_shape(int ks, int mo) { return (ks == 1 && mo == 4) || (ks == 2 && mo == 8); }
+
 template <int KS_IN, int MO, int NT>
 static void launch_mlp(const MlpParams& p, int N, hipStream_t s) {
   long rows_per_block = 4L * NT * 16;
   dim3 grid((unsigned)((p.rps + rows_per_block - 1) / rows_per_block), (unsigned)N), block(256);
+  if constexpr (mlp_res_conv_shape(KS_IN, MO)) {
+    if (p.rx) {
+      if (p.w3_f16) hipLaunchKernelGGL((pw_mlp_kernel<KS_IN, MO, NT, 3, false, false, false, false, true>), grid, block, 0, s, p);
+      else hipLaunchKernelGGL((pw_mlp_kernel<KS_IN, MO, NT, 1, false, false, false, false, true>), grid, block, 0, s, p);
+      return;
+    }
+  }
   if (p.hp_in) {
     hipLaunchKernelGGL((pw_mlp_kernel<KS_IN, MO, NT, 1, false, false, false, true>), grid, block, 0, s, p);
     return;
@@ -731,6 +804,18 @@
 
 extern "C" int pytc_pw_mlp_supported(int C_in, int C_hid, int C_out) { return mlp_shape_ok(C_in, C_hid, C_out) ? 1 : 0; }
 
+extern "C" int pytc_pw_mlp_res_conv_supported(int C_in, int C_hid, int C_out, int res_mode, int lds) {
+  if (C_in % 32 || C_hid % 32 || C_out % 32 || C_hid < 32) return 0;
+  const int ks = C_in / 32, mo = C_out / 16, bits = tuning_get(K_mlp_res_conv);
+  if (lds) {
+    const int variant = tuning_get(K_mlp_lds_variant);
+    const size_t bytes = (size_t)C_hid * (C_in + C_out) * 2 + (size_t)C_hid * 4 + (size_t)C_out * C_in * 2 + (size_t)C_out * 4;
+    return (res_mode == PYTC_RES_UPSAMPLE && ks == 2 && mo == 2 && (bits & 4) && (variant == 0 || variant == 2) && bytes <= 160 * 1024) ? 1 : 0;
+  }
+  if (res_mode != PYTC_RES_CONV_GATHER || !mlp_res_conv_shape(ks, mo)) return 0;
+  return (bits & (ks == 1 ? 1 : 2)) ? 1 : 0;
+}
+
 extern "C" int pytc_groupnorm_fold_mlp(const float* stats, int slots, float count, const float* gamma, const float* beta,
                                        float eps, const float* w2, const float* b2, void* w2n, float* b2n, float* ab_out, int N,
                                        int C, int C_hid, void* stream) {
@@ -785,6 +870,7 @@
   PYTC_REQUIRE(!(a->ab && a->per_sample), "pw_mlp_head: per-sample (norm-folded) expand operands come without an affine");
   PYTC_REQUIRE(!store_y || a->y, "pw_mlp_head: store_y without an output buffer");
   PYTC_REQUIRE(a->N >= 1 && a->rows_per_sample >= 1 && n_head >= 1 && n_head <= 16, "pw_mlp_head: bad shape");
+  PYTC_REFUSE_RES_CONV(a, "pw_mlp_head");
   if (!pytc_pw_mlp_head_supported(a->C_in, a->C_hid, a->C_out)) {
     set_error("pw_mlp_head: no fused kernel for C_in=%d C_hid=%d C_out=%d", a->C_in, a->C_hid, a->C_out);
     return PYTC_ERR_UNSUPPORTED;
@@ -826,6 +912,7 @@
                "pw_mlp_stemres: null pointer");
   PYTC_REQUIRE(!(a->ab && a->per_sample), "pw_mlp_stemres: per-sample (norm-folded) expand operands come without an affine");
   PYTC_REQUIRE(a->N >= 1 && a->rows_per_sample >= 1, "pw_mlp_stemres: bad shape");
+  PYTC_REFUSE_RES_CONV(a, "pw_mlp_stemres");
   if (!(a->C_in == 32 && a->C_out == 32 && a->C_hid % 32 == 0 && a->C_hid >= 32)) {
     set_error("pw_mlp_stemres: no fused kernel for C_in=%d C_hid=%d C_out=%d", a->C_in, a->C_hid, a->C_out);
     return PYTC_ERR_UNSUPPORTED;
@@ -875,6 +962,7 @@
   PYTC_REQUIRE(a->w3_format == PYTC_W3_F16, "pw_mlp_proj: the mixer's projection image must be fp16 (pytc_pw_pack_weight_paired_f16)");
   PYTC_REQUIRE(!store_y || a->y, "pw_mlp_proj: store_y without an output buffer");
   PYTC_REQUIRE(a->N >= 1 && a->rows_per_sample >= 1, "pw_mlp_proj: bad shape");
+  PYTC_REFUSE_RES_CONV(a, "pw_mlp_proj");
   if (!pytc_pw_mlp_proj_supported(a->C_in, a->C_hid, a->C_out, 32)) {
     set_error("pw_mlp_proj: no fused kernel for C_in=%d C_hid=%d C_out=%d", a->C_in, a->C_hid, a->C_out);
     return PYTC_ERR_UNSUPPORTED;
@@ -893,7 +981,8 @@
   return PYTC_OK;
 }
 
-static int mlp_fwd_impl(const pytc_mlp_args* a, void* hp, void* stream, const void* hp_in = nullptr, bool round_h = false);
+static int mlp_fwd_impl(const pytc_mlp_args* a, void* hp, void* stream, const void* hp_in = nullptr, bool round_h = false,
+                        const MlpResConv* rc = nullptr);
 
 extern "C" int pytc_pw_mlp_bwd(const pytc_mlp_args* a, const void* hidden_pre, void* d_hidden, void* stream) {
   PYTC_REQUIRE(hidden_pre && d_hidden, "pw_mlp_bwd: null hidden buffers");
@@ -912,7 +1001,14 @@
 
 extern "C" int pytc_pw_mlp_fwd(const pytc_mlp_args* a, void* stream) { return mlp_fwd_impl(a, nullptr, stream); }
 
-static int mlp_fwd_impl(const pytc_mlp_args* a, void* hp, void* stream, const void* hp_in, bool round_h) {
+extern "C" int pytc_pw_mlp_res_conv_fwd(const pytc_mlp_args* a, const void* res_x, const void* res_w_packed, const float* res_conv_bias,
+                                        int Dx, int Hx, int Wx, int lds, void* stream) {
+  PYTC_REQUIRE(a && res_x && res_w_packed, "pw_mlp_res_conv: null pointer");
+  const MlpResConv rc{res_x, res_w_packed, res_conv_bias, Dx, Hx, Wx};
+  return lds ? mlp_lds_fwd(a, &rc, stream) : mlp_fwd_impl(a, nullptr, stream, nullptr, false, &rc);
+}
+
+static int mlp_fwd_impl(const pytc_mlp_args* a, void* hp, void* stream, const void* hp_in, bool round_h, const MlpResConv* rc) {
   PYTC_REQUIRE(a && a->t && (a->ab || a->per_sample) && a->w2_packed && a->w3_packed && a->b2 && a->b3 && a->y, "pw_mlp: null pointer");
   PYTC_REQUIRE(!(a->ab && a->per_sample), "pw_mlp: per-sample (norm-folded) expand operands come without an affine");
   PYTC_REQUIRE(!(a->per_sample && (hp || hp_in || round_h)), "pw_mlp: the training kernels take the shared expand image and the affine");
@@ -921,8 +1017,21 @@
     set_error("pw_mlp: no fused kernel for C_in=%d C_hid=%d C_out=%d", a->C_in, a->C_hid, a->C_out);
     return PYTC_ERR_UNSUPPORTED;
   }
-  PYTC_REQUIRE(a->res_mode == PYTC_RES_NONE || a->res, "pw_mlp: residual mode without residual pointer");
-  PYTC_REQUIRE(a->res_mode == PYTC_RES_NONE || a->res_mode == PYTC_RES_ADD || a->res_mode == PYTC_RES_UPSAMPLE,
+  const bool res_conv = a->res_mode == PYTC_RES_CONV_GATHER;
+  if (res_conv || rc) {
+    const bool form = res_conv && rc && !hp && !hp_in && !round_h && mlp_res_conv_shape(a->C_in / 32, a->C_out / 16);
+    if (!form) {
+      set_error("pw_mlp: the residual conv inside the mixer covers PYTC_RES_CONV_GATHER at C_in -> C_out of 32 -> 64 and 64 -> 128, "
+                "through pytc_pw_mlp_res_conv_fwd, inference only; got res_mode %d, %d -> %d", a->res_mode, a->C_in, a->C_out);
+      return PYTC_ERR_UNSUPPORTED;
+    }
+    PYTC_REQUIRE(rc->x && rc->w_packed && !a->res && !a->res_low, "pw_mlp: RES_CONV_GATHER takes res_x and res_w_packed, not res / res_low");
+    const long Do = (rc->Dx - 1) / 2 + 1, Ho = (rc->Hx - 1) / 2 + 1, Wo = (rc->Wx - 1) / 2 + 1;
+    PYTC_REQUIRE(rc->Dx >= 1 && rc->Hx >= 1 && rc->Wx >= 1 && Do * Ho * Wo == a->rows_per_sample && a->rows_per_sample < (1L << 31),
+                 "pw_mlp: RES_CONV_GATHER needs the grid of res_x, (%d, %d, %d), whose stride-2 grid has rows_per_sample rows", rc->Dx, rc->Hx, rc->Wx);
+  }
+  PYTC_REQUIRE(a->res_mode == PYTC_RES_NONE || res_conv || a->res, "pw_mlp: residual mode without residual pointer");
+  PYTC_REQUIRE(a->res_mode == PYTC_RES_NONE || a->res_mode == PYTC_RES_ADD || a->res_mode == PYTC_RES_UPSAMPLE || res_conv,
                "pw_mlp: unsupported res_mode %d", a->res_mode);
   MlpParams p{};
   p.t = (const bf16_t*)a->t; p.ab = a->ab; p.w2 = (const bf16x8_t*)a->w2_packed; p.b2 = a->b2;
@@ -945,6 +1054,12 @@
     p.e.Go_d = a->Di; p.e.Go_h = a->Hi; p.e.Go_w = a->Wi;
     p.e.Gl_d = a->Di / 2; p.e.Gl_h = a->Hi / 2; p.e.Gl_w = a->Wi / 2;
   }
+  if (res_conv) {
+    p.e.res_mode = PYTC_RES_ADD;
+    p.rx = (const bf16_t*)rc->x; p.rw = (const bf16x8_t*)rc->w_packed; p.rb = rc->bias;
+    p.rps_rx = (long)rc->Dx * rc->Hx * rc->Wx; p.Gi_h = rc->Hx; p.Gi_w = rc->Wx;
+    p.e.Go_d = (rc->Dx - 1) / 2 + 1; p.e.Go_h = (rc->Hx - 1) / 2 + 1; p.e.Go_w = (rc->Wx - 1) / 2 + 1;
+  }
   if (!hp && !hp_in && !round_h && mlp_dma_applies(a, p)) {
     mlp_dma_launch<0>(a, p, (hipStream_t)stream);
     PYTC_LAUNCH_CHECK("pw_mlp_dma");
diff --git a/pytorch_connectomics_amd/csrc/pw_mlp_lds_kernels.hip b/pytorch_connectomics_amd/csrc/pw_mlp_lds_kernels.hip
--- a/pytorch_connectomics_amd/csrc/pw_mlp_lds_kernels.hip
+++ b/pytorch_connectomics_amd/csrc/pw_mlp_lds_kernels.hip
@@ -15,6 +15,9 @@
   long rps;
   int N, C_in, C_hid, C_out, HC;
   long w2_stride;
+  const bf16_t* rx;
+  const bf16x8_t* rw;
+  const float* rb;
 };
 
 template <int KS_IN, int MO, int NT>
@@ -46,7 +49,7 @@
   }
 }
 
-template <int KS_IN, int MO, int NT, int NWAVES, int WPS>
+template <int KS_IN, int MO, int NT, int NWAVES, int WPS, bool RESCONV = false>
 __global__ void __launch_bounds__(NWAVES * 64, WPS)
 pw_mlp_lds_kernel(MlpLdsParams p) {
   constexpr int CIN = KS_IN * 32, COUT = MO * 16;
@@ -54,11 +57,17 @@
   bf16x8_t* lw2 = reinterpret_cast<bf16x8_t*>(lds_raw);
   h8_t* lw3 = reinterpret_cast<h8_t*>(lds_raw + (size_t)p.C_hid * CIN * 2);
   float* lb2 = reinterpret_cast<float*>(lds_raw + (size_t)p.C_hid * (CIN + COUT) * 2);
+  bf16x8_t* lrw = reinterpret_cast<bf16x8_t*>(lds_raw + (size_t)p.C_hid * (CIN + COUT) * 2 + (size_t)p.C_hid * 4);
+  float* lrb = reinterpret_cast<float*>(lrw + MO * KS_IN * 64);
   const int tid = threadIdx.x, wave = tid >> 6, lane = tid & 63;
   const int r = lane & 15, kb = lane >> 4;
   const bool folded = p.ab == nullptr;
   const int n_w2 = p.C_hid * CIN / 8, n_w3 = COUT * p.C_hid / 8;
   for (int i = tid; i < n_w3; i += NWAVES * 64) lw3[i] = p.w3[i];
+  if constexpr (RESCONV) {
+    for (int i = tid; i < MO * KS_IN * 64; i += NWAVES * 64) lrw[i] = p.rw[i];
+    for (int i = tid; i < COUT; i += NWAVES * 64) lrb[i] = p.rb ? p.rb[i] : 0.f;
+  }
   const long Ts = (p.rps + NT * 16 - 1) / (NT * 16);
   const long G = Ts * p.N;
   const long g_end = G * (blockIdx.x + 1) / gridDim.x;
@@ -170,6 +179,54 @@
           upos[nt][0] = pz; upos[nt][1] = py; upos[nt][2] = px;
         }
       }
+      bf16x8_t rl16[RESCONV ? MO / 2 : 1][RESCONV ? NT : 1];
+      if constexpr (RESCONV) {
+#pragma unroll
+        for (int pr = 0; pr < MO / 2; ++pr)
+#pragma unroll
+          for (int nt = 0; nt < NT; ++nt) rl16[pr][nt] = __builtin_bit_cast(bf16x8_t, uint4{0u, 0u, 0u, 0u});
+        long lrow[NT];
+        bool any = false;
+#pragma unroll
+        for (int nt = 0; nt < NT; ++nt) {
+          const int oz = upos[nt][0] - 1, oy = upos[nt][1] - 1, ox = upos[nt][2] - 1;
+          const bool need = orow[nt] < p.rps && oz >= 0 && oy >= 0 && ox >= 0 && !((oz | oy | ox) & 1);
+          lrow[nt] = need ? ((long)(oz >> 1) * p.e.Gl_h + (oy >> 1)) * p.e.Gl_w + (ox >> 1) : 0L;
+          any = any || need;
+        }
+        if (__ballot(any) != 0) {
+          const bf16_t* rxn = p.rx + (long)n * ((long)p.e.Gl_d * p.e.Gl_h * p.e.Gl_w) * CIN;
+          bf16x8_t xl[KS_IN][NT];
+#pragma unroll
+          for (int nt = 0; nt < NT; ++nt)
+#pragma unroll
+            for (int ks = 0; ks < KS_IN; ++ks)
+              xl[ks][nt] = *reinterpret_cast<const bf16x8_t*>(rxn + lrow[nt] * CIN + ks * 32 + kb * 8);
+#pragma unroll
+          for (int pr = 0; pr < MO / 2; ++pr) {
+            const f32x4_t blo = *reinterpret_cast<const f32x4_t*>(lrb + pr * 32 + kb * 8);
+            const f32x4_t bhi = *reinterpret_cast<const f32x4_t*>(lrb + pr * 32 + kb * 8 + 4);
+            f32x4_t racc[2][NT];
+#pragma unroll
+            for (int nt = 0; nt < NT; ++nt) { racc[0][nt] = blo; racc[1][nt] = bhi; }
+#pragma unroll
+            for (int mt = 0; mt < 2; ++mt)
+#pragma unroll
+              for (int ks = 0; ks < KS_IN; ++ks) {
+                const bf16x8_t a = lrw[((pr * 2 + mt) * KS_IN + ks) * 64 + lane];
+#pragma unroll
+                for (int nt = 0; nt < NT; ++nt) racc[mt][nt] = Mma<bf16_t>::mma(a, xl[ks][nt], racc[mt][nt]);
+              }
+#pragma unroll
+            for (int nt = 0; nt < NT; ++nt) {
+              float rv[8];
+#pragma unroll
+              for (int j = 0; j < 4; ++j) { rv[j] = racc[0][nt][j]; rv[4 + j] = racc[1][nt][j]; }
+              rl16[pr][nt] = Mma<bf16_t>::from_floats(rv);
+            }
+          }
+        }
+      }
 #pragma unroll
       for (int pr = 0; pr < MO / 2; ++pr) {
 #pragma unroll
@@ -178,6 +235,13 @@
           float v[8];
 #pragma unroll
           for (int j = 0; j < 4; ++j) { v[j] = acc2[2 * pr][nt][j]; v[4 + j] = acc2[2 * pr + 1][nt][j]; }
+          if constexpr (RESCONV) {
+            float pre[8], rl[8];
+            VecIO<bf16_t, 8>::load(reinterpret_cast<const bf16_t*>(&cur.res[pr][nt]), pre);
+            VecIO<bf16_t, 8>::load(reinterpret_cast<const bf16_t*>(&rl16[pr][nt]), rl);
+            finish_and_store<bf16_t, 8, false, COUT>(v, p.e, n, orow[nt], pr * 32 + kb * 8, pre, upos[nt], rl);
+            continue;
+          }
           if (with_res) {
             float pre[8];
             VecIO<bf16_t, 8>::load(reinterpret_cast<const bf16_t*>(&cur.res[pr][nt]), pre);
@@ -192,9 +256,9 @@
   }
 }
 
-template <int KS_IN, int MO, int NT, int NWAVES, int WPS>
+template <int KS_IN, int MO, int NT, int NWAVES, int WPS, bool RESCONV = false>
 static void launch_mlp_lds_v(const MlpLdsParams& p, size_t lds, hipStream_t s) {
-  auto kern = &pw_mlp_lds_kernel<KS_IN, MO, NT, NWAVES, WPS>;
+  auto kern = &pw_mlp_lds_kernel<KS_IN, MO, NT, NWAVES, WPS, RESCONV>;
   if (!ensure_dynamic_lds(reinterpret_cast<const void*>(kern), 160 * 1024, "pw_mlp_lds")) return;
   const long tiles = ((p.rps + NT * 16 - 1) / (NT * 16)) * p.N;
   const int by_lds = (int)((160 * 1024) / lds), by_waves = WPS * 4 / NWAVES;
@@ -229,7 +293,9 @@
   return (shape && lds <= 160 * 1024) ? 1 : 0;
 }
 
-extern "C" int pytc_pw_mlp_lds_fwd(const pytc_mlp_args* a, void* stream) {
+extern "C" int pytc_pw_mlp_lds_fwd(const pytc_mlp_args* a, void* stream) { return mlp_lds_fwd(a, nullptr, stream); }
+
+int pytc::mlp_lds_fwd(const pytc_mlp_args* a, const MlpResConv* rc, void* stream) {
   PYTC_REQUIRE(a && a->t && (a->ab || a->per_sample) && a->w2_packed && a->w3_packed && a->b2 && a->b3 && a->y, "pw_mlp_lds: null pointer");
   PYTC_REQUIRE(!(a->ab && a->per_sample), "pw_mlp_lds: per-sample (norm-folded) expand operands come without an affine");
   PYTC_REQUIRE(a->w3_format == PYTC_W3_F16, "pw_mlp_lds: the projection image must be fp16 (pytc_pw_pack_weight_paired_f16)");
@@ -237,6 +303,17 @@
   if (!pytc_pw_mlp_lds_supported(a->C_in, a->C_hid, a->C_out)) {
     set_error("pw_mlp_lds: no LDS-resident kernel for C_in=%d C_hid=%d C_out=%d", a->C_in, a->C_hid, a->C_out);
     return PYTC_ERR_UNSUPPORTED;
+  }
+  const bool res_conv = rc != nullptr || a->res_mode == PYTC_RES_CONV_GATHER;
+  if (res_conv) {
+    const int variant = tuning_get(K_mlp_lds_variant);
+    const size_t lds = (size_t)a->C_hid * (a->C_in + a->C_out) * 2 + (size_t)a->C_hid * 4 + (size_t)a->C_out * a->C_in * 2 + (size_t)a->C_out * 4;
+    if (!(rc && a->res_mode == PYTC_RES_UPSAMPLE && a->C_in == 64 && a->C_out == 32 && (variant == 0 || variant == 2) && lds <= 160 * 1024)) {
+      set_error("pw_mlp_lds: the residual conv inside the mixer (pytc_pw_mlp_res_conv_fwd) covers PYTC_RES_UPSAMPLE at 64 -> 32 on the default launch shape; "
+                "got res_mode %d, %d -> %d, mlp_lds_variant %d", a->res_mode, a->C_in, a->C_out, variant);
+      return PYTC_ERR_UNSUPPORTED;
+    }
+    PYTC_REQUIRE(rc->x && rc->w_packed && !a->res_low, "pw_mlp_lds: res_x comes with res_w_packed and takes the place of res_low");
   }
   PYTC_REQUIRE(a->res_mode == PYTC_RES_NONE || a->res, "pw_mlp_lds: residual mode without residual pointer");
   MlpLdsParams p{};
@@ -257,7 +334,11 @@
   hipStream_t s = (hipStream_t)stream;
   const int ks = a->C_in / 32, mo = a->C_out / 16;
   const int variant = tuning_get(K_mlp_lds_variant);
-  if (ks == 2 && mo == 2) launch_mlp_lds<2, 2, 2>(p, variant, s);
+  if (res_conv) {
+    p.rx = (const bf16_t*)rc->x; p.rw = (const bf16x8_t*)rc->w_packed; p.rb = rc->bias;
+    const size_t lds = (size_t)p.C_hid * (p.C_in + p.C_out) * 2 + (size_t)p.C_hid * 4 + (size_t)p.C_out * p.C_in * 2 + (size_t)p.C_out * 4;
+    launch_mlp_lds_v<2, 2, 2, 16, 4, true>(p, lds, s);
+  } else if (ks == 2 && mo == 2) launch_mlp_lds<2, 2, 2>(p, variant, s);
   else if (ks == 2 && mo == 4) launch_mlp_lds<2, 4, 2>(p, variant, s);
   else if (ks == 4 && mo == 4) launch_mlp_lds<4, 4, 2>(p, variant, s);
   else launch_mlp_lds<4, 8, 2>(p, variant, s);
diff --git a/pytorch_connectomics_amd/csrc/pw_mlp_up_kernels.hip b/pytorch_connectomics_amd/csrc/pw_mlp_up_kernels.hip
--- a/pytorch_connectomics_amd/csrc/pw_mlp_up_kernels.hip
+++ b/pytorch_connectomics_amd/csrc/pw_mlp_up_kernels.hip
@@ -266,6 +266,7 @@
   PYTC_REQUIRE(a && a->t && a->ab && a->w2_packed && a->w3_packed && a->b2 && a->b3 && a->y && a->res && taps && dw_bias &&
                a->res_bias, "pw_mlp_up: null pointer (dw_bias and res_bias are zero vectors when unused)");
   PYTC_REQUIRE(a->N >= 1 && a->Di >= 1 && a->Hi >= 1 && a->Wi >= 1, "pw_mlp_up: bad shape");
+  PYTC_REFUSE_RES_CONV(a, "pw_mlp_up");
   if (!pytc_pw_mlp_up_supported(a->C_in, a->C_hid, a->C_out)) {
     set_error("pw_mlp_up: no fused kernel for C_in=%d C_hid=%d C_out=%d", a->C_in, a->C_hid, a->C_out);
     return PYTC_ERR_UNSUPPORTED;
diff --git a/pytorch_connectomics_amd/csrc/pytc_common.h b/pytorch_connectomics_amd/csrc/pytc_common.h
--- a/pytorch_connectomics_amd/csrc/pytc_common.h
+++ b/pytorch_connectomics_amd/csrc/pytc_common.h
@@ -57,6 +57,7 @@
   X(mlp_dma_rows, 1 << 20, "fewest rows of a launch that takes the DMA mixer")                                                     \
   X(mlp_dma_wgs, 0, "DMA mixer: workgroups per sample; 0 = chosen from the row count")                                             \
   X(mlp_lds_variant, 0, "LDS-resident mixer (pw_mlp_lds_kernels.hip): tile shape of the launch")                                   \
+  X(mlp_res_conv, 7, "residual 1x1 conv inside the mixer: bit 0 = down 32->64, bit 1 = down 64->128, bit 2 = up 64->32; 0 = own launch") \
   X(norm_bwd_from_wgrad_flat, 1, "GroupNorm-backward epilogue of the expand weight gradient as one flat kernel; 0 = chunked")      \
   X(pw_gemm_rows, 0, "LDS-tiled 1x1 GEMM: 64 / 128 forces the rows per workgroup; 0 = by problem size")                            \
   X(pw_thin, 1, "plain 1x1 convs with one input / few output channels on the thin kernels; 0 = the generic kernel")                \
diff --git a/pytorch_connectomics_amd/hip_ops.py b/pytorch_connectomics_amd/hip_ops.py
--- a/pytorch_connectomics_amd/hip_ops.py
+++ b/pytorch_connectomics_amd/hip_ops.py
@@ -622,10 +622,20 @@
            res: Optional[torch.Tensor] = None, res_mode: int = nat.RES_NONE, grid: Sequence[int] = (0, 0, 0),
            res_low: Optional[torch.Tensor] = None, res_bias: Optional[torch.Tensor] = None,
            y: Optional[torch.Tensor] = None, hidden_pre: Optional[torch.Tensor] = None, lds: bool = False,
-           chunked: bool = False, train_nostore: bool = False) -> torch.Tensor:
+           chunked: bool = False, train_nostore: bool = False, res_x: Optional[torch.Tensor] = None,
+           res_w: Optional[torch.Tensor] = None, res_conv_bias: Optional[torch.Tensor] = None,
+           res_grid: Sequence[int] = (0, 0, 0)) -> torch.Tensor:
     _dev(t, "t")
     if t.dtype != torch.bfloat16:
         raise TypeError("pw_mlp runs on bfloat16 activations")
+    if res_x is not None:
+        _dev(res_x, "res_x"); _dev(res_w, "res_w")
+        if res_x.dtype != torch.bfloat16 or res_w.dtype != torch.bfloat16 or not res_x.is_contiguous() or res_x.shape[-1] != c_in \
+                or res_w.numel() != c_in * c_out:
+            raise TypeError(f"pw_mlp: res_x must be contiguous bf16 (..., {c_in}) and res_w the paired bf16 image of a {c_in} -> {c_out} conv")
+        want = N * rows_per_sample // 8 if res_mode == nat.RES_UPSAMPLE else N * int(res_grid[0]) * int(res_grid[1]) * int(res_grid[2])
+        if res_x.numel() != want * c_in:
+            raise ValueError(f"pw_mlp: res_x has {res_x.numel() // c_in} rows, the grid says {want}")
     if y is None:
         y = torch.empty((N, rows_per_sample, c_out), dtype=torch.bfloat16, device=t.device)
     else:
@@ -642,6 +652,14 @@
     a.N, a.rows_per_sample, a.C_in, a.C_hid, a.C_out, a.res_mode = N, rows_per_sample, c_in, c_hid, c_out, res_mode
     a.Di, a.Hi, a.Wi = (int(v) for v in grid)
     nb = N * rows_per_sample * 2 * (c_in + c_out + (c_out if res is not None else 0))
+    if res_x is not None:
+        nb += (N * rows_per_sample if res_mode != nat.RES_UPSAMPLE else res_x.numel() // c_in) * 2 * c_in
+        if hidden_pre is not None or train_nostore or chunked:
+            raise ValueError("pw_mlp: res_x goes with the streaming (inference) and the LDS-resident mixers only")
+        kernel = "pw_mlp_lds_kernel" if lds else "pw_mlp_kernel"
+        _run(f"pw_mlp_fwd[{c_in}->{c_hid}->{c_out}]", nb, nat.lib().pytc_pw_mlp_res_conv_fwd, C.byref(a), _p(res_x), _p(res_w), _p(res_conv_bias),
+             *(int(v) for v in res_grid), int(bool(lds)), _stream(), symbol=f"{kernel}<{c_in // 32}, {c_out // 16}>")
+        return y
     if hidden_pre is not None:
         _dev(hidden_pre, "hidden_pre")
         _run(f"pw_mlp_train_fwd[{c_in}->{c_hid}->{c_out}]", nb + N * rows_per_sample * 2 * c_hid, nat.lib().pytc_pw_mlp_train_fwd,
@@ -662,6 +680,10 @@
     _run(f"pw_mlp_fwd[{c_in}->{c_hid}->{c_out}]", nb, nat.lib().pytc_pw_mlp_fwd, C.byref(a), _stream(),
          symbol=_mlp_symbol(a, f"pw_mlp_kernel<{c_in // 32}, {c_out // 16}>", 0))
     return y
+
+
+def pw_mlp_res_conv_supported(c_in: int, c_hid: int, c_out: int, res_mode: int, lds: bool = False) -> bool:
+    return bool(nat.lib().pytc_pw_mlp_res_conv_supported(int(c_in), int(c_hid), int(c_out), int(res_mode), int(bool(lds))))
 
 
 def pw_mlp_lds_supported(c_in: int, c_hid: int, c_out: int) -> bool:
diff --git a/pytorch_connectomics_amd/models/architectures/mednext.py b/pytorch_connectomics_amd/models/architectures/mednext.py
--- a/pytorch_connectomics_amd/models/architectures/mednext.py
+++ b/pytorch_connectomics_amd/models/architectures/mednext.py
@@ -412,6 +412,12 @@
                        res_mode=nat.RES_ADD if m.do_res else nat.RES_NONE, **kw)
     elif m.kind == "down":
         res = None
+        in_mixer = (m.resample_do_res and not kw.get("lds") and not kw.get("chunked") and x.is_contiguous()
+                    and ops.pw_mlp_res_conv_supported(C, c_hid, c_out, nat.RES_CONV_GATHER))
+        if in_mixer:
+            y = ops.pw_mlp(t, ab, w2, b2, w3, b3, res_mode=nat.RES_CONV_GATHER, res_x=x, res_w=self._pw_paired(m.res_conv),
+                           res_conv_bias=self._vec(m.res_conv, "bias", m.res_conv.bias), res_grid=(D, H, W), **kw)
+            return y.view(N, Do, Ho, Wo, c_out)
         if m.resample_do_res:
             paired = ops.pw_conv_paired_supported(c_in=C, c_out=c_out, in_dtype=dt, out_dtype=dt, gather=2)
             wres = self._pw_paired(m.res_conv) if paired else self._pw(m.res_conv, dt)
@@ -422,14 +428,19 @@
         if skip is None:
             skip = torch.zeros((N, Do, Ho, Wo, c_out), dtype=dt, device=x.device)
         res_low = res_bias = None
+        extra = {}
         if m.resample_do_res:
             res_bias = self._vec(m.res_conv, "bias", m.res_conv.bias)
-            paired = ops.pw_conv_paired_supported(c_in=C, c_out=c_out, in_dtype=dt, out_dtype=dt)
-            wres = self._pw_paired(m.res_conv, transposed=True) if paired else self._pw(m.res_conv, dt, transposed=True)
-            res_low = ops.pw_conv(x, wres, res_bias, N=N, rows_per_sample=D * H * W, c_in=C, c_out=c_out,
-                                  out_dtype=dt, w_paired=paired)
+            if (kw.get("lds") and x.is_contiguous() and m.res_conv.bias is not None
+                    and ops.pw_mlp_res_conv_supported(C, c_hid, c_out, nat.RES_UPSAMPLE, lds=True)):
+                extra = dict(res_x=x, res_w=self._pw_paired(m.res_conv, transposed=True), res_conv_bias=res_bias)
+            else:
+                paired = ops.pw_conv_paired_supported(c_in=C, c_out=c_out, in_dtype=dt, out_dtype=dt)
+                wres = self._pw_paired(m.res_conv, transposed=True) if paired else self._pw(m.res_conv, dt, transposed=True)
+                res_low = ops.pw_conv(x, wres, res_bias, N=N, rows_per_sample=D * H * W, c_in=C, c_out=c_out,
+                                      out_dtype=dt, w_paired=paired)
         y = ops.pw_mlp(t, ab, w2, b2, w3, b3, res=skip, res_mode=nat.RES_UPSAMPLE, grid=(Do, Ho, Wo),
-                       res_low=res_low, res_bias=res_bias, **kw)
+                       res_low=res_low, res_bias=res_bias, **extra, **kw)
     return y.view(N, Do, Ho, Wo, c_out)
 
 
```

Result: faster. 1.888 billion voxels/s (median of 6 runs) (+2.2%).
